# AIS-Bonn/lattice_net

Hardware: AMD Instinct MI355X
Metric: Mpoints/sec splat+conv+slice fwd+bwd on 120k-pt SemanticKITTI scan (higher is better)
Workload: dtype f32 (convolution products bf16x3-emulated)

## Files before the change

include/latticenet_hip.h:

```cpp
#ifndef LATTICENET_HIP_H
#define LATTICENET_HIP_H

#include <stddef.h>

#ifdef __cplusplus
extern "C" {
#endif

#define LN_OK 0
#define LN_ERR_ARG (-1)
#define LN_ERR_UNSUPPORTED (-2)
#define LN_ERR_LAUNCH (-3)
#define LN_ERR_WORKSPACE (-4)

#define LN_STATUS_TABLE_FULL 1
#define LN_STATUS_KEY_RANGE 2
#define LN_STATUS_BUCKET_OVERFLOW 4
#define LN_STATUS_CLOUD_BAND 8
#define LN_STATUS_CLOUD_STARTS 16

#define LN_MAX_POS_DIM 6
#define LN_SLOT_MAP_INTS 32
#define LN_KEYS_RAW 0
#define LN_KEYS_LATTICE 1
#define LN_NOT_VISITED (-2)

typedef struct LnTable {
    int capacity;
    int pos_dim;
    unsigned long long* slot_keys;
    unsigned int* slot_tok;
    int* slot_cnt;
    int* entries;
    int* keys;
    int* nr_filled;
    int* status;
    int* host_counters;
    int host_seq;
    int key_format;
    int row_limit;
    const int* slot_map;
    int bucket_slots_max;
    int batch_points;
    int batch_key_step;
    int* row_regions;
} LnTable;

#define LN_BATCH_POINT_STARTS (-1)
typedef struct LnTableClouds {
    LnTable table;
    const int* batch_point_starts;
    int batch_clouds;
} LnTableClouds;

#define LN_XCD_GROUPS 8
typedef struct LnCsr {
    int* grp_start;
    int* csr_tok;
    int* seg_desc;
    int* seg_count;
    long long seg_region;
    const int* planes;
    int dense;
} LnCsr;

const char* ln_last_error_string(void);
const char* ln_version(void);
const char* ln_abi_hash(void);

const char* ln_kernel_names(void);
int ln_profile_begin(const char* kernel_names, int max_samples);
int ln_profile_end(double* total_ms, int* launches);
int ln_profile_end_table(char* out, int out_bytes);

int ln_table_clear(const LnTable* t, float* values, long long values_elems, void* stream);

int ln_arena_init(int* arena, long long words, long long minus_begin, long long minus_end, void* stream);

int ln_table_bucket_count(int capacity);

size_t ln_build_workspace_bytes(long long tokens, int capacity);

#define LN_BUILD_WRITE_IDX 1
#define LN_BUILD_CLEAR_FIRST 2
#define LN_BUILD_ATOMIC_PATH 4
#define LN_BUILD_CANONICAL_ROWS 8
#define LN_BUILD_SORTED_CSR 16
#define LN_BUILD_OVERLAPPED 32
int ln_build_splat(const LnTable* t, const float* positions_raw, const float* sigmas_host, int n, int* idx, float* w,
                   int flags, const LnCsr* csr, void* workspace, size_t workspace_bytes, float* clear_values,
                   long long clear_values_elems, void* stream);

int ln_canonicalize(const LnTable* t, int* idx, long long tokens, const LnCsr* csr, void* workspace, size_t workspace_bytes, void* stream);

int ln_rehash(const LnTable* t, void* stream);

int ln_splat_accumulate(float* table_values, const float* vals, const int* idx, const float* w, int n, int pos_dim,
                        int val_dim, void* stream);

long long ln_csr_max_segments(long long tokens, int groups_upper);
size_t ln_csr_workspace_bytes(long long tokens, int groups_upper);
int ln_csr_build(const int* idx, long long tokens, int groups_upper, const LnCsr* csr, void* workspace, size_t workspace_bytes,
                 void* stream);
int ln_csr_reduce_rows(const LnCsr* csr, const int* grp_row, long long max_segments, const float* src, const float* w, int val_dim,
                       int src_div, int src_stride, float* dst, void* stream);
int ln_csr_sort(const LnCsr* csr, int groups_upper, void* workspace, size_t workspace_bytes, long long tokens, void* stream);

int ln_splat_accumulate_and_neighbours(const LnCsr* csr, const int* grp_row, long long max_segments, const float* src, const float* w,
                                       int val_dim, int src_div, int src_stride, float* dst, const LnTable* table, int query_rows_upper,
                                       int* nbr, void* stream);

int ln_csr_segment_max(const LnCsr* csr, const int* grp_row, long long max_segments, const float* src, int channels, int rows,
                       void* packed_ws, float* out_max, int* out_arg, void* stream);
int ln_csr_group_sizes(const LnCsr* csr, const int* grp_row, int groups_upper, int rows, int* counts, void* stream);

int ln_distribute(const LnTable* t, const float* positions_raw, const float* sigmas_host, const float* vals, int n,
                  int val_dim, int* idx, float* w, float* distributed, int flags, const LnCsr* csr, void* workspace,
                  size_t workspace_bytes, float* clear_values, long long clear_values_elems, void* stream);

int ln_coarsen(const LnTable* fine, int fine_rows_upper, const LnTable* coarse, const LnCsr* csr, void* workspace,
               size_t workspace_bytes, void* stream);

int ln_neighbours(const LnTable* query, int query_rows_upper, const LnTable* neigh, int lvl_query, int lvl_neigh,
                  int dilation, int flip, int* nbr, void* stream);

int ln_im2row(const int* nbr, const float* values_neigh, int m, int filter_extent, int val_dim, float* out, void* stream);
int ln_im2rowindices(const int* nbr, int m, int filter_extent, int val_dim, int* out, void* stream);
int ln_row2im(const int* nbr, const float* rowified, int m, int filter_extent, int val_dim, float* out, void* stream);

#define LN_CONV_FLIP_NEIGHBOURS 1
#define LN_CONV_TRANSPOSED_FILTER 2
#define LN_CONV_BANK_READY 4
int ln_conv_forward(const int* nbr, const float* values_neigh, const float* filter, int m, int filter_extent, int val_dim,
                    int nr_filters, int flags, float* out, void* stream);
size_t ln_conv_bank_workspace_bytes(int m, int filter_extent, int val_dim, int nr_filters);
size_t ln_conv_forward_workspace_bytes(int m, int filter_extent, int val_dim, int nr_filters);
int ln_conv_forward_ws(const int* nbr, const float* values_neigh, const float* filter, int m, int filter_extent, int val_dim,
                       int nr_filters, int flags, float* out, void* workspace, size_t workspace_bytes, const int* row_partition, void* stream);
size_t ln_conv_grad_filter_workspace_bytes(int m, int filter_extent, int val_dim, int nr_filters);
int ln_conv_grad_filter(const int* nbr, const float* values_neigh, const float* grad_out, int m, int filter_extent,
                        int val_dim, int nr_filters, float* grad_filter, void* workspace, size_t workspace_bytes,
                        void* stream);

int ln_slice_forward(const float* values, const int* idx, const float* w, int n, int pos_dim, int val_dim, float* out,
                     void* stream);
int ln_slice_forward_prepare_backward(const float* values, const int* idx, const float* w, int n, int pos_dim, int val_dim, float* out,
                                      float* grad_accumulator, long long grad_accumulator_elems, void* stream);
int ln_slice_forward_ordered(const LnTable* t, const LnCsr* csr, const float* values, const int* idx, const float* w, int n, int val_dim,
                             float* out, float* grad_accumulator, long long grad_accumulator_elems, void* stream);

int ln_slice_no_precomputation(const LnTable* t, const float* values, const float* positions_raw, const float* sigmas_host,
                               int n, int val_dim, float* out, int* idx, float* w, void* stream);
int ln_slice_backward(const float* grad_sliced, const int* idx, const float* w, int n, int pos_dim, int val_dim,
                      float* grad_values, void* stream);

int ln_gather_forward(const float* values, const int* idx, const float* w, int n, int pos_dim, int val_dim, float* out,
                      void* stream);
int ln_gather_backward(const float* grad_gathered, const int* idx, const float* w, int n, int pos_dim, int val_dim,
                       float* grad_values, void* stream);

int ln_slice_classify_forward(const float* values, const float* delta_w, const float* lin_w, const float* lin_b,
                              const int* idx, const float* w, int n, int pos_dim, int val_dim, int nr_classes,
                              float* logits, void* stream);
size_t ln_slice_classify_backward_workspace_bytes(int n, int pos_dim, int val_dim, int nr_classes);
int ln_slice_classify_backward(const float* grad_logits, const float* values, const float* delta_w, const float* lin_w,
                               const int* idx, const float* w, int n, int pos_dim, int val_dim, int nr_classes,
                               float* g_values, float* g_delta_w, float* g_lin_w, float* g_lin_b, float* grad_sliced,
                               float* w_eff, void* workspace, size_t workspace_bytes, void* stream);

size_t ln_conv_backward_workspace_bytes(int mq, int mn, int filter_extent, int val_dim, int nr_filters);
int ln_conv_backward(const int* nbr_q, const int* nbr_n, const float* values_neigh, const float* grad_out, const float* filter, int mq, int mn,
                     int filter_extent, int val_dim, int nr_filters, float* grad_values, float* grad_filter, void* workspace,
                     size_t workspace_bytes, const int* row_partition, void* stream);

int ln_csr_reduce_rows_f16(const LnCsr* csr, const int* grp_row, long long max_segments, const void* src_f16, const float* w, int val_dim,
                           int src_div, int src_stride, float* dst, void* stream);
int ln_splat_accumulate_and_neighbours_f16(const LnCsr* csr, const int* grp_row, long long max_segments, const void* src_f16, const float* w,
                                           int val_dim, int src_div, int src_stride, float* dst, const LnTable* table, int query_rows_upper,
                                           int* nbr, void* stream);
int ln_slice_forward_f16(const void* values_f16, const int* idx, const float* w, int n, int pos_dim, int val_dim, void* out_f16, void* stream);
int ln_slice_forward_f16_prepare_backward(const void* values_f16, const int* idx, const float* w, int n, int pos_dim, int val_dim, void* out_f16,
                                          float* grad_accumulator, long long grad_accumulator_elems, void* stream);

int ln_conv_forward_f16(const int* nbr, const void* values_neigh, const void* filter, int m, int filter_extent, int val_dim,
                        int nr_filters, int flags, void* out, void* stream);
size_t ln_conv_grad_filter_f16_workspace_bytes(int m, int filter_extent, int val_dim, int nr_filters);
int ln_conv_grad_filter_f16(const int* nbr, const void* values_neigh, const void* grad_out, int m, int filter_extent, int val_dim,
                            int nr_filters, float* grad_filter, void* workspace, size_t workspace_bytes, void* stream);

int ln_linear_act_forward(const float* x, const float* w, const float* b, long long rows, int cin, int cout, float slope, float* y,
                          void* stream);
size_t ln_linear_act_backward_workspace_bytes(int cin, int cout);
int ln_linear_act_backward(const float* x, const float* w, const float* y, const float* grad_y, long long rows, int cin, int cout,
                           float slope, float* grad_x, float* grad_w, float* grad_b, void* workspace, size_t workspace_bytes, void* stream);

size_t ln_group_norm_workspace_bytes(int channels);
int ln_group_norm_forward(const float* x, const float* gamma, const float* beta, int m, int channels, int groups, float eps, int relu,
                          float* y, float* mean_rstd, float* scale_shift, void* workspace, size_t workspace_bytes, void* next_workspace,
                          size_t next_workspace_bytes, void* stream);
int ln_group_norm_backward(const float* x, const float* grad_y, const float* gamma, const float* mean_rstd, const float* scale_shift, int m,
                           int channels, int groups, int relu, float* grad_x, float* grad_gamma, float* grad_beta, void* workspace,
                           size_t workspace_bytes, void* next_workspace, size_t next_workspace_bytes, void* stream);
int ln_group_norm_forward_rows(const float* x, const float* gamma, const float* beta, int m, int channels, int groups, float eps, int relu,
                               float* y, float* mean_rstd, float* scale_shift, void* workspace, size_t workspace_bytes, void* next_workspace,
                               size_t next_workspace_bytes, const int* rows_device, void* stream);
int ln_group_norm_backward_rows(const float* x, const float* grad_y, const float* gamma, const float* mean_rstd, const float* scale_shift, int m,
                                int channels, int groups, int relu, float* grad_x, float* grad_gamma, float* grad_beta, void* workspace,
                                size_t workspace_bytes, void* next_workspace, size_t next_workspace_bytes, const int* rows_device, void* stream);

int ln_cloud_row_starts(const LnTable* t, int rows_upper, int clouds, int* row_starts, int* order_flag, void* stream);
int ln_cloud_row_starts_many(const LnTable* t, int rows_upper, int clouds, int* row_starts, int* order_flag, void* stream);
size_t ln_group_norm_segments_workspace_bytes(int channels, int segments);
int ln_group_norm_forward_segments(const float* x, const float* gamma, const float* beta, int m, int channels, int groups, float eps, int relu,
                                   float* y, float* mean_rstd, float* scale_shift, void* workspace, size_t workspace_bytes, void* next_workspace,
                                   size_t next_workspace_bytes, const int* rows_device, const int* row_starts, int segments, void* stream);
int ln_group_norm_backward_segments(const float* x, const float* grad_y, const float* gamma, const float* mean_rstd, const float* scale_shift,
                                    int m, int channels, int groups, int relu, float* grad_x, float* grad_gamma, float* grad_beta, void* workspace,
                                    size_t workspace_bytes, void* next_workspace, size_t next_workspace_bytes, const int* rows_device,
                                    const int* row_starts, int segments, void* stream);
int ln_group_norm_forward_many_segments(const float* x, const float* gamma, const float* beta, int m, int channels, int groups, float eps,
                                        int relu, float* y, float* mean_rstd, float* scale_shift, void* workspace, size_t workspace_bytes,
                                        void* next_workspace, size_t next_workspace_bytes, const int* rows_device, const int* row_starts,
                                        int segments, void* stream);
int ln_group_norm_backward_many_segments(const float* x, const float* grad_y, const float* gamma, const float* mean_rstd,
                                         const float* scale_shift, int m, int channels, int groups, int relu, float* grad_x, float* grad_gamma,
                                         float* grad_beta, void* workspace, size_t workspace_bytes, void* next_workspace,
                                         size_t next_workspace_bytes, const int* rows_device, const int* row_starts, int segments, void* stream);

int ln_group_norm_forward_segments_f16(const void* x, const float* gamma, const float* beta, int m, int channels, int groups, float eps, int relu,
                                       void* y, float* mean_rstd, float* scale_shift, void* workspace, size_t workspace_bytes,
                                       void* next_workspace, size_t next_workspace_bytes, const int* rows_device, const int* row_starts,
                                       int segments, void* stream);
int ln_group_norm_backward_segments_f16(const void* x, const void* grad_y, const float* gamma, const float* mean_rstd, const float* scale_shift,
                                        int m, int channels, int groups, int relu, void* grad_x, float* grad_gamma, float* grad_beta,
                                        void* workspace, size_t workspace_bytes, void* next_workspace, size_t next_workspace_bytes,
                                        const int* rows_device, const int* row_starts, int segments, void* stream);

size_t ln_batch_norm_workspace_bytes(int channels);
int ln_batch_norm_forward(const float* x, const float* gamma, const float* beta, float* running_mean, float* running_var, int m, int channels,
                          float eps, double momentum, int training, int relu, float* y, float* mean_rstd, float* scale_shift, void* workspace,
                          size_t workspace_bytes, void* next_workspace, size_t next_workspace_bytes, const int* rows_device, void* stream);
int ln_batch_norm_backward(const float* x, const float* grad_y, const float* gamma, const float* mean_rstd, const float* scale_shift, int m,
                           int channels, int training, int relu, float* grad_x, float* grad_gamma, float* grad_beta, void* workspace,
                           size_t workspace_bytes, void* next_workspace, size_t next_workspace_bytes, const int* rows_device, void* stream);

int ln_max_centre_forward(const float* x, const float* gamma, const float* beta, long long n, int k, int c, float* out,
                          float* max_vals, unsigned char* arg_max, void* stream);
size_t ln_max_centre_backward_workspace_bytes(long long n, int k, int c);
int ln_max_centre_backward(const float* grad_out, const float* max_vals, const unsigned char* arg_max, const float* gamma,
                           long long n, int k, int c, float* grad_x, float* grad_gamma_beta, void* workspace,
                           size_t workspace_bytes, void* stream);

size_t ln_linear_backward_workspace_bytes(int rows, int cin, int cout);
int ln_linear_backward(const int* ident, const float* x, const float* grad_y, const float* w, int rows, int cin, int cout, float* grad_x,
                       float* grad_w, void* workspace, size_t workspace_bytes, void* stream);

int ln_weight_norm_forward(const float* v, const float* g, int rows, int cols, int g_dim, float* w, float* norm, void* stream);
int ln_weight_norm_backward(const float* v, const float* g, const float* grad_w, const float* norm, int rows, int cols, int g_dim,
                            float* grad_v, float* grad_g, void* stream);

int ln_distribute_centre(const float* distributed, const int* splat_idx, const float* position_sums, const int* counts, long long tokens,
                         int width, int pos_dim, float* out, void* stream);
int ln_distribute_centre_clouds(const float* distributed, const int* splat_idx, const float* position_sums, const int* counts,
                                long long tokens, int width, int pos_dim, long long tokens_per_cloud, const int* row_starts, int clouds,
                                float* out, void* stream);
int ln_distribute_centre_cloud_starts(const float* distributed, const int* splat_idx, const float* position_sums, const int* counts,
                                      long long tokens, int width, int pos_dim, int tokens_per_point, const int* point_starts,
                                      const int* row_starts, int clouds, float* out, void* stream);
int ln_distribute_centre_many_clouds(const float* distributed, const int* splat_idx, const float* position_sums, const int* counts,
                                     long long tokens, int width, int pos_dim, long long tokens_per_cloud, const int* row_starts, int clouds,
                                     float* out, void* stream);
int ln_distribute_centre_many_cloud_starts(const float* distributed, const int* splat_idx, const float* position_sums, const int* counts,
                                           long long tokens, int width, int pos_dim, int tokens_per_point, const int* point_starts,
                                           const int* row_starts, int clouds, float* out, void* stream);

size_t ln_pointnet_reduce_workspace_bytes(int rows, int channels);
int ln_pointnet_reduce_forward(const LnCsr* csr, const int* grp_row, long long max_segments, const float* src, int channels,
                               const float* bary, int bary_stride, int rows, int min_points, void* workspace, size_t workspace_bytes,
                               float* out, int* out_arg, void* stream);
int ln_pointnet_reduce_forward_clouds(const LnCsr* csr, const int* grp_row, long long max_segments, const float* src, int channels,
                                      const float* bary, int bary_stride, int rows, int min_points, void* workspace, size_t workspace_bytes,
                                      float* out, int* out_arg, const int* row_starts, int clouds, void* stream);
int ln_pointnet_reduce_forward_many_clouds(const LnCsr* csr, const int* grp_row, long long max_segments, const float* src, int channels,
                                           const float* bary, int bary_stride, int rows, int min_points, void* workspace,
                                           size_t workspace_bytes, float* out, int* out_arg, const int* row_starts, int clouds, void* stream);
int ln_pointnet_reduce_backward(const float* grad_out, int grad_stride, const int* out_arg, const int* splat_idx, long long tokens,
                                int channels, float* grad_src, void* stream);

size_t ln_nll_workspace_bytes(void);
int ln_nll_forward(const float* log_probs, const long long* target, long long n, int classes, long long ignore_index, void* workspace,
                   size_t workspace_bytes, float* loss_count, void* stream);
int ln_nll_backward(const long long* target, const float* grad_loss, const float* loss_count, long long n, int classes,
                    long long ignore_index, float* grad_log_probs, void* stream);

size_t ln_lovasz_workspace_bytes(long long n, int classes);
int ln_lovasz_forward(const float* log_probs, const long long* target, long long n, int classes, long long ignore_index, int reduction,
                      void* workspace, size_t workspace_bytes, float* loss, float* per_class, float* dloss_dlogp, void* stream);
int ln_lovasz_backward(const float* dloss_dlogp, const float* grad_loss, long long n, int classes, float* grad_log_probs, void* stream);

size_t ln_lovasz_clouds_workspace_bytes(long long n, long long points_per_cloud, int classes);
int ln_lovasz_forward_clouds(const float* log_probs, const long long* target, long long n, long long points_per_cloud, int classes,
                             long long ignore_index, int reduction, void* workspace, size_t workspace_bytes, float* loss, float* per_cloud,
                             float* per_class, float* dloss_dlogp, void* stream);

size_t ln_iou_counts_clouds_workspace_bytes(long long n, long long points_per_cloud, int classes);
int ln_iou_counts_clouds(const float* scores, const long long* target, long long n, long long points_per_cloud, int classes,
                         long long unlabeled_index, void* workspace, size_t workspace_bytes, long long* intersection, long long* union_,
                         void* stream);

size_t ln_dice_workspace_bytes(long long n, long long points_per_cloud, int classes);
int ln_dice_forward(const float* log_probs, const long long* target, long long n, long long points_per_cloud, int classes,
                    long long ignore_index, void* workspace, size_t workspace_bytes, float* loss, float* per_cloud, float* stats, float* coef,
                    void* stream);
int ln_dice_backward(const float* log_probs, const long long* target, const float* coef, const float* grad_loss, long long n,
                     long long points_per_cloud, int classes, float* grad_log_probs, void* stream);

size_t ln_nll_clouds_workspace_bytes(long long n, long long points_per_cloud);
int ln_nll_forward_clouds(const float* log_probs, const long long* target, long long n, long long points_per_cloud, int classes,
                          long long ignore_index, const float* class_weight, void* workspace, size_t workspace_bytes, float* loss,
                          float* per_cloud, float* weight_sum, void* stream);
int ln_nll_backward_clouds(const long long* target, const float* grad_loss, const float* weight_sum, long long n, long long points_per_cloud,
                           int classes, long long ignore_index, const float* class_weight, float* grad_log_probs, void* stream);

size_t ln_nll_ranges_workspace_bytes(long long n, int clouds, long long longest);
int ln_nll_forward_ranges(const float* log_probs, const long long* target, long long n, const int* point_starts, int clouds, long long longest,
                          int classes, long long ignore_index, const float* class_weight, void* workspace, size_t workspace_bytes, float* loss,
                          float* per_cloud, float* weight_sum, void* stream);
int ln_nll_backward_ranges(const long long* target, const float* grad_loss, const float* weight_sum, long long n, const int* point_starts,
                           int clouds, long long longest, int classes, long long ignore_index, const float* class_weight,
                           float* grad_log_probs, void* stream);
size_t ln_dice_ranges_workspace_bytes(long long n, int clouds, long long longest, int classes);
int ln_dice_forward_ranges(const float* log_probs, const long long* target, long long n, const int* point_starts, int clouds, long long longest,
                           int classes, long long ignore_index, void* workspace, size_t workspace_bytes, float* loss, float* per_cloud,
                           float* stats, float* coef, void* stream);
int ln_dice_backward_ranges(const float* log_probs, const long long* target, const float* coef, const float* grad_loss, long long n,
                            const int* point_starts, int clouds, long long longest, int classes, float* grad_log_probs, void* stream);
size_t ln_lovasz_ranges_workspace_bytes(long long n, int clouds, long long longest, int classes);
int ln_lovasz_forward_ranges(const float* log_probs, const long long* target, long long n, const int* point_starts, int clouds,
                             long long longest, int classes, long long ignore_index, int reduction, void* workspace, size_t workspace_bytes,
                             float* loss, float* per_cloud, float* per_class, float* dloss_dlogp, void* stream);

int ln_cloud_key_extents(const LnTable* t, const float* positions_raw, const float* sigmas_host, int n, int guard, int* extents,
                         int* first_bad, void* stream);
int ln_cloud_point_starts_check(const int* starts, int clouds, int n, int* status, void* stream);

#ifdef __cplusplus
}
#endif
#endif
```

lattice_net_amd/_lib.py:

```python
from __future__ import annotations

import ctypes as C
import os

import torch

_PKG = os.path.dirname(os.path.abspath(__file__))
LIB_PATH = os.environ.get("LATTICE_NET_LIB") or os.path.join(_PKG, "liblatticenet_hip.so")

LN_STATUS_TABLE_FULL = 1
LN_STATUS_KEY_RANGE = 2
LN_STATUS_BUCKET_OVERFLOW = 4
LN_STATUS_CLOUD_BAND = 8
LN_STATUS_CLOUD_STARTS = 16
LN_BUILD_WRITE_IDX = 1
LN_BUILD_CLEAR_FIRST = 2
LN_BUILD_ATOMIC_PATH = 4
LN_BUILD_CANONICAL_ROWS = 8
LN_BUILD_SORTED_CSR = 16
LN_BUILD_OVERLAPPED = 32
LN_NOT_VISITED = -2
LN_CONV_FLIP_NEIGHBOURS = 1
LN_CONV_TRANSPOSED_FILTER = 2
LN_CONV_BANK_READY = 4
LN_MAX_POS_DIM = 6
LN_KEYS_RAW = 0
LN_KEYS_LATTICE = 1
LN_XCD_GROUPS = 8
LN_SLOT_MAP_INTS = 32


class LnTable(C.Structure):

    _fields_ = [
        ("capacity", C.c_int),
        ("pos_dim", C.c_int),
        ("slot_keys", C.c_void_p),
        ("slot_tok", C.c_void_p),
        ("slot_cnt", C.c_void_p),
        ("entries", C.c_void_p),
        ("keys", C.c_void_p),
        ("nr_filled", C.c_void_p),
        ("status", C.c_void_p),
        ("host_counters", C.c_void_p),
        ("host_seq", C.c_int),
        ("key_format", C.c_int),
        ("row_limit", C.c_int),
        ("slot_map", C.c_void_p),
        ("bucket_slots_max", C.c_int),
        ("batch_points", C.c_int),
        ("batch_key_step", C.c_int),
        ("row_regions", C.c_void_p),
    ]


LN_BATCH_POINT_STARTS = -1


class LnTableClouds(C.Structure):

    _fields_ = [
        ("table", LnTable),
        ("batch_point_starts", C.c_void_p),
        ("batch_clouds", C.c_int),
    ]

    def __init__(self, table_fields=(), batch_point_starts=None, batch_clouds=0):
        super().__init__(LnTable(*table_fields), batch_point_starts, batch_clouds)
        self.table.batch_points = LN_BATCH_POINT_STARTS


class LnCsr(C.Structure):

    _fields_ = [
        ("grp_start", C.c_void_p),
        ("csr_tok", C.c_void_p),
        ("seg_desc", C.c_void_p),
        ("seg_count", C.c_void_p),
        ("seg_region", C.c_longlong),
        ("planes", C.c_void_p),
        ("dense", C.c_int),
    ]


class LatticeNetHipError(RuntimeError):
    pass


_vp, _i, _ll, _sz = C.c_void_p, C.c_int, C.c_longlong, C.c_size_t
_T = C.POINTER(LnTable)
_CSR = C.POINTER(LnCsr)

SIGNATURES = {
    "ln_last_error_string": (C.c_char_p, []),
    "ln_version": (C.c_char_p, []),
    "ln_abi_hash": (C.c_char_p, []),
    "ln_kernel_names": (C.c_char_p, []),
    "ln_profile_begin": (_i, [C.c_char_p, _i]),
    "ln_profile_end": (_i, [C.POINTER(C.c_double), C.POINTER(_i)]),
    "ln_profile_end_table": (_i, [C.c_char_p, _i]),
    "ln_table_clear": (_i, [_T, _vp, _ll, _vp]),
    "ln_build_workspace_bytes": (_sz, [_ll, _i]),
    "ln_table_bucket_count": (_i, [_i]),
    "ln_build_splat": (_i, [_T, _vp, _vp, _i, _vp, _vp, _i, _CSR, _vp, _sz, _vp, _ll, _vp]),
    "ln_rehash": (_i, [_T, _vp]),
    "ln_canonicalize": (_i, [_T, _vp, _ll, _CSR, _vp, _sz, _vp]),
    "ln_splat_accumulate": (_i, [_vp, _vp, _vp, _vp, _i, _i, _i, _vp]),
    "ln_csr_workspace_bytes": (_sz, [_ll, _i]),
    "ln_csr_max_segments": (_ll, [_ll, _i]),
    "ln_csr_build": (_i, [_vp, _ll, _i, _CSR, _vp, _sz, _vp]),
    "ln_csr_reduce_rows": (_i, [_CSR, _vp, _ll, _vp, _vp, _i, _i, _i, _vp, _vp]),
    "ln_csr_sort": (_i, [_CSR, _i, _vp, _sz, _ll, _vp]),
    "ln_splat_accumulate_and_neighbours": (_i, [_CSR, _vp, _ll, _vp, _vp, _i, _i, _i, _vp, _T, _i, _vp, _vp]),
    "ln_csr_segment_max": (_i, [_CSR, _vp, _ll, _vp, _i, _i, _vp, _vp, _vp, _vp]),
    "ln_csr_group_sizes": (_i, [_CSR, _vp, _i, _i, _vp, _vp]),
    "ln_distribute": (_i, [_T, _vp, _vp, _vp, _i, _i, _vp, _vp, _vp, _i, _CSR, _vp, _sz, _vp, _ll, _vp]),
    "ln_coarsen": (_i, [_T, _i, _T, _CSR, _vp, _sz, _vp]),
    "ln_neighbours": (_i, [_T, _i, _T, _i, _i, _i, _i, _vp, _vp]),
    "ln_im2row": (_i, [_vp, _vp, _i, _i, _i, _vp, _vp]),
    "ln_im2rowindices": (_i, [_vp, _i, _i, _i, _vp, _vp]),
    "ln_row2im": (_i, [_vp, _vp, _i, _i, _i, _vp, _vp]),
    "ln_conv_forward": (_i, [_vp, _vp, _vp, _i, _i, _i, _i, _i, _vp, _vp]),
    "ln_conv_forward_workspace_bytes": (_sz, [_i, _i, _i, _i]),
    "ln_conv_bank_workspace_bytes": (_sz, [_i, _i, _i, _i]),
    "ln_conv_forward_ws": (_i, [_vp, _vp, _vp, _i, _i, _i, _i, _i, _vp, _vp, _sz, _vp, _vp]),
    "ln_conv_grad_filter_workspace_bytes": (_sz, [_i, _i, _i, _i]),
    "ln_conv_grad_filter": (_i, [_vp, _vp, _vp, _i, _i, _i, _i, _vp, _vp, _sz, _vp]),
    "ln_slice_forward": (_i, [_vp, _vp, _vp, _i, _i, _i, _vp, _vp]),
    "ln_slice_forward_prepare_backward": (_i, [_vp, _vp, _vp, _i, _i, _i, _vp, _vp, _ll, _vp]),
    "ln_slice_forward_ordered": (_i, [_T, _CSR, _vp, _vp, _vp, _i, _i, _vp, _vp, _ll, _vp]),
    "ln_slice_no_precomputation": (_i, [_T, _vp, _vp, _vp, _i, _i, _vp, _vp, _vp, _vp]),
    "ln_slice_backward": (_i, [_vp, _vp, _vp, _i, _i, _i, _vp, _vp]),
    "ln_gather_forward": (_i, [_vp, _vp, _vp, _i, _i, _i, _vp, _vp]),
    "ln_gather_backward": (_i, [_vp, _vp, _vp, _i, _i, _i, _vp, _vp]),
    "ln_slice_classify_forward": (_i, [_vp, _vp, _vp, _vp, _vp, _vp, _i, _i, _i, _i, _vp, _vp]),
    "ln_csr_reduce_rows_f16": (_i, [_CSR, _vp, _ll, _vp, _vp, _i, _i, _i, _vp, _vp]),
    "ln_splat_accumulate_and_neighbours_f16": (_i, [_CSR, _vp, _ll, _vp, _vp, _i, _i, _i, _vp, _T, _i, _vp, _vp]),
    "ln_slice_forward_f16": (_i, [_vp, _vp, _vp, _i, _i, _i, _vp, _vp]),
    "ln_slice_forward_f16_prepare_backward": (_i, [_vp, _vp, _vp, _i, _i, _i, _vp, _vp, _ll, _vp]),
    "ln_conv_backward_workspace_bytes": (_sz, [_i, _i, _i, _i, _i]),
    "ln_conv_backward": (_i, [_vp, _vp, _vp, _vp, _vp, _i, _i, _i, _i, _i, _vp, _vp, _vp, _sz, _vp, _vp]),
    "ln_conv_forward_f16": (_i, [_vp, _vp, _vp, _i, _i, _i, _i, _i, _vp, _vp]),
    "ln_conv_grad_filter_f16_workspace_bytes": (_sz, [_i, _i, _i, _i]),
    "ln_conv_grad_filter_f16": (_i, [_vp, _vp, _vp, _i, _i, _i, _i, _vp, _vp, _sz, _vp]),
    "ln_linear_act_forward": (_i, [_vp, _vp, _vp, _ll, _i, _i, C.c_float, _vp, _vp]),
    "ln_linear_act_backward_workspace_bytes": (_sz, [_i, _i]),
    "ln_linear_act_backward": (_i, [_vp, _vp, _vp, _vp, _ll, _i, _i, C.c_float, _vp, _vp, _vp, _vp, _sz, _vp]),
    "ln_arena_init": (_i, [_vp, _ll, _ll, _ll, _vp]),
    "ln_weight_norm_forward": (_i, [_vp, _vp, _i, _i, _i, _vp, _vp, _vp]),
    "ln_weight_norm_backward": (_i, [_vp, _vp, _vp, _vp, _i, _i, _i, _vp, _vp, _vp]),
    "ln_distribute_centre": (_i, [_vp, _vp, _vp, _vp, _ll, _i, _i, _vp, _vp]),
    "ln_distribute_centre_clouds": (_i, [_vp, _vp, _vp, _vp, _ll, _i, _i, _ll, _vp, _i, _vp, _vp]),
    "ln_distribute_centre_many_clouds": (_i, [_vp, _vp, _vp, _vp, _ll, _i, _i, _ll, _vp, _i, _vp, _vp]),
    "ln_distribute_centre_cloud_starts": (_i, [_vp, _vp, _vp, _vp, _ll, _i, _i, _i, _vp, _vp, _i, _vp, _vp]),
    "ln_distribute_centre_many_cloud_starts": (_i, [_vp, _vp, _vp, _vp, _ll, _i, _i, _i, _vp, _vp, _i, _vp, _vp]),
    "ln_pointnet_reduce_workspace_bytes": (_sz, [_i, _i]),
    "ln_pointnet_reduce_forward": (_i, [_CSR, _vp, _ll, _vp, _i, _vp, _i, _i, _i, _vp, _sz, _vp, _vp, _vp]),
    "ln_pointnet_reduce_forward_clouds": (_i, [_CSR, _vp, _ll, _vp, _i, _vp, _i, _i, _i, _vp, _sz, _vp, _vp, _vp, _i, _vp]),
    "ln_pointnet_reduce_forward_many_clouds": (_i, [_CSR, _vp, _ll, _vp, _i, _vp, _i, _i, _i, _vp, _sz, _vp, _vp, _vp, _i, _vp]),
    "ln_pointnet_reduce_backward": (_i, [_vp, _i, _vp, _vp, _ll, _i, _vp, _vp]),
    "ln_linear_backward_workspace_bytes": (_sz, [_i, _i, _i]),
    "ln_linear_backward": (_i, [_vp, _vp, _vp, _vp, _i, _i, _i, _vp, _vp, _vp, _sz, _vp]),
    "ln_nll_workspace_bytes": (_sz, []),
    "ln_nll_forward": (_i, [_vp, _vp, _ll, _i, _ll, _vp, _sz, _vp, _vp]),
    "ln_nll_backward": (_i, [_vp, _vp, _vp, _ll, _i, _ll, _vp, _vp]),
    "ln_nll_clouds_workspace_bytes": (_sz, [_ll, _ll]),
    "ln_nll_forward_clouds": (_i, [_vp, _vp, _ll, _ll, _i, _ll, _vp, _vp, _sz, _vp, _vp, _vp, _vp]),
    "ln_nll_backward_clouds": (_i, [_vp, _vp, _vp, _ll, _ll, _i, _ll, _vp, _vp, _vp]),
    "ln_lovasz_workspace_bytes": (_sz, [_ll, _i]),
    "ln_lovasz_forward": (_i, [_vp, _vp, _ll, _i, _ll, _i, _vp, _sz, _vp, _vp, _vp, _vp]),
    "ln_lovasz_backward": (_i, [_vp, _vp, _ll, _i, _vp, _vp]),
    "ln_lovasz_clouds_workspace_bytes": (_sz, [_ll, _ll, _i]),
    "ln_lovasz_forward_clouds": (_i, [_vp, _vp, _ll, _ll, _i, _ll, _i, _vp, _sz, _vp, _vp, _vp, _vp, _vp]),
    "ln_iou_counts_clouds_workspace_bytes": (_sz, [_ll, _ll, _i]),
    "ln_iou_counts_clouds": (_i, [_vp, _vp, _ll, _ll, _i, _ll, _vp, _sz, _vp, _vp, _vp]),
    "ln_dice_workspace_bytes": (_sz, [_ll, _ll, _i]),
    "ln_dice_forward": (_i, [_vp, _vp, _ll, _ll, _i, _ll, _vp, _sz, _vp, _vp, _vp, _vp, _vp]),
    "ln_dice_backward": (_i, [_vp, _vp, _vp, _vp, _ll, _ll, _i, _vp, _vp]),
    "ln_nll_ranges_workspace_bytes": (_sz, [_ll, _i, _ll]),
    "ln_nll_forward_ranges": (_i, [_vp, _vp, _ll, _vp, _i, _ll, _i, _ll, _vp, _vp, _sz, _vp, _vp, _vp, _vp]),
    "ln_nll_backward_ranges": (_i, [_vp, _vp, _vp, _ll, _vp, _i, _ll, _i, _ll, _vp, _vp, _vp]),
    "ln_dice_ranges_workspace_bytes": (_sz, [_ll, _i, _ll, _i]),
    "ln_dice_forward_ranges": (_i, [_vp, _vp, _ll, _vp, _i, _ll, _i, _ll, _vp, _sz, _vp, _vp, _vp, _vp, _vp]),
    "ln_dice_backward_ranges": (_i, [_vp, _vp, _vp, _vp, _ll, _vp, _i, _ll, _i, _vp, _vp]),
    "ln_lovasz_ranges_workspace_bytes": (_sz, [_ll, _i, _ll, _i]),
    "ln_lovasz_forward_ranges": (_i, [_vp, _vp, _ll, _vp, _i, _ll, _i, _ll, _i, _vp, _sz, _vp, _vp, _vp, _vp, _vp]),
    "ln_max_centre_forward": (_i, [_vp, _vp, _vp, _ll, _i, _i, _vp, _vp, _vp, _vp]),
    "ln_max_centre_backward_workspace_bytes": (_sz, [_ll, _i, _i]),
    "ln_max_centre_backward": (_i, [_vp, _vp, _vp, _vp, _ll, _i, _i, _vp, _vp, _vp, _sz, _vp]),
    "ln_group_norm_workspace_bytes": (_sz, [_i]),
    "ln_group_norm_forward": (_i, [_vp, _vp, _vp, _i, _i, _i, C.c_float, _i, _vp, _vp, _vp, _vp, _sz, _vp, _sz, _vp]),
    "ln_group_norm_backward": (_i, [_vp, _vp, _vp, _vp, _vp, _i, _i, _i, _i, _vp, _vp, _vp, _vp, _sz, _vp, _sz, _vp]),
    "ln_group_norm_forward_rows": (_i, [_vp, _vp, _vp, _i, _i, _i, C.c_float, _i, _vp, _vp, _vp, _vp, _sz, _vp, _sz, _vp, _vp]),
    "ln_group_norm_backward_rows": (_i, [_vp, _vp, _vp, _vp, _vp, _i, _i, _i, _i, _vp, _vp, _vp, _vp, _sz, _vp, _sz, _vp, _vp]),
    "ln_cloud_row_starts": (_i, [_T, _i, _i, _vp, _vp, _vp]),
    "ln_cloud_row_starts_many": (_i, [_T, _i, _i, _vp, _vp, _vp]),
    "ln_group_norm_segments_workspace_bytes": (_sz, [_i, _i]),
    "ln_group_norm_forward_segments": (_i, [_vp, _vp, _vp, _i, _i, _i, C.c_float, _i, _vp, _vp, _vp, _vp, _sz, _vp, _sz, _vp, _vp, _i, _vp]),
    "ln_group_norm_forward_many_segments": (_i, [_vp, _vp, _vp, _i, _i, _i, C.c_float, _i, _vp, _vp, _vp, _vp, _sz, _vp, _sz, _vp, _vp, _i, _vp]),
    "ln_group_norm_backward_segments": (_i, [_vp, _vp, _vp, _vp, _vp, _i, _i, _i, _i, _vp, _vp, _vp, _vp, _sz, _vp, _sz, _vp, _vp, _i, _vp]),
    "ln_group_norm_backward_many_segments": (_i, [_vp, _vp, _vp, _vp, _vp, _i, _i, _i, _i, _vp, _vp, _vp, _vp, _sz, _vp, _sz, _vp, _vp, _i, _vp]),
    "ln_group_norm_forward_segments_f16": (_i, [_vp, _vp, _vp, _i, _i, _i, C.c_float, _i, _vp, _vp, _vp, _vp, _sz, _vp, _sz, _vp, _vp, _i, _vp]),
    "ln_group_norm_backward_segments_f16": (_i, [_vp, _vp, _vp, _vp, _vp, _i, _i, _i, _i, _vp, _vp, _vp, _vp, _sz, _vp, _sz, _vp, _vp, _i, _vp]),
    "ln_batch_norm_workspace_bytes": (_sz, [_i]),
    "ln_batch_norm_forward": (_i, [_vp, _vp, _vp, _vp, _vp, _i, _i, C.c_float, C.c_double, _i, _i, _vp, _vp, _vp, _vp, _sz, _vp, _sz, _vp, _vp]),
    "ln_batch_norm_backward": (_i, [_vp, _vp, _vp, _vp, _vp, _i, _i, _i, _i, _vp, _vp, _vp, _vp, _sz, _vp, _sz, _vp, _vp]),
    "ln_cloud_key_extents": (_i, [_T, _vp, _vp, _i, _i, _vp, _vp, _vp]),
    "ln_cloud_point_starts_check": (_i, [_vp, _i, _i, _vp, _vp]),
    "ln_slice_classify_backward_workspace_bytes": (_sz, [_i, _i, _i, _i]),
    "ln_slice_classify_backward": (_i, [_vp, _vp, _vp, _vp, _vp, _vp, _i, _i, _i, _i, _vp, _vp, _vp, _vp, _vp, _vp, _vp, _sz, _vp]),
}

_lib = None


def load():
    global _lib
    if _lib is not None:
        return _lib
    if not os.path.exists(LIB_PATH):
        raise LatticeNetHipError(
            f"{LIB_PATH} is missing: the HIP extension is not built. Run `python -c 'import __graft_entry__ as g; g.build()'` "
            "(or `python lattice_net_amd/build_ext.py`). There is no CPU fallback."
        )
    lib = C.CDLL(LIB_PATH)
    for name, (res, args) in SIGNATURES.items():
        fn = getattr(lib, name)
        fn.restype = res
        fn.argtypes = args
    from . import build_ext
    try:
        want = build_ext.abi_hash()
    except OSError:
        want = None
    have = lib.ln_abi_hash().decode()
    if want is not None and have != want:
        raise LatticeNetHipError(f"{LIB_PATH} was built from a different include/latticenet_hip.h (library {have}, header {want}): "
                                 "rebuild it with `python lattice_net_amd/build_ext.py`")
    _lib = lib
    return lib


def check(rc: int, what: str = ""):
    if rc != 0:
        msg = load().ln_last_error_string().decode("utf-8", "replace")
        raise LatticeNetHipError(f"{what or 'latticenet_hip'} failed (code {rc}): {msg}")


def ptr(t):
    return None if t is None else t.data_ptr()


def stream_ptr(device) -> int:
    cur = torch.cuda.current_device()
    idx = device.index if device.index is not None else cur
    if idx != cur:
        raise LatticeNetHipError(f"lattice tensors live on cuda:{idx} but the current device is cuda:{cur}; wrap the call in "
                                 f"`with torch.cuda.device({idx}):` (or torch.cuda.set_device) — one process drives one GPU")
    return torch._C._cuda_getCurrentRawStream(idx)


def host_floats(values):
    arr = (C.c_float * len(values))(*[float(v) for v in values])
    return arr
```

lattice_net_amd/csrc/ln_conv.hip:

```cpp
#include "ln_common.h"
#include <stdlib.h>

#include "ln_bf16x3.h"

#include "ln_conv_plan.h"
#include <type_traits>

#ifdef LN_STAMPS
__device__ unsigned long long* g_ln_stamps_conv = nullptr;
extern "C" int ln_debug_set_stamps_conv(void* buffer) {
    unsigned long long* p = static_cast<unsigned long long*>(buffer);
    return hipMemcpyToSymbol(HIP_SYMBOL(g_ln_stamps_conv), &p, sizeof(p)) == hipSuccess ? 0 : -1;
}
#define LN_CSTAMP(slot)                                                                                                  \
    do {                                                                                                                 \
        if (g_ln_stamps_conv && threadIdx.x == 0) g_ln_stamps_conv[(size_t)blockIdx.x * 8 + (slot)] = wall_clock64(); \
    } while (0)
#else
#define LN_CSTAMP(slot) do { } while (0)
#endif

template <int KQ>
__device__ __forceinline__ void ln_load_quarter(const float* __restrict__ src, float* a) {
    if constexpr (KQ % 4 == 0) {
// ... 784 lines not shown
        advance(it);
    };
    for (int it = 0; it < total; it += 2) {
        iteration(it, ap, ap_b);
        if (it + 1 < total) iteration(it + 1, ap_b, ap);
    }
    asm volatile("s_waitcnt vmcnt(0)" ::: "memory");
    __builtin_amdgcn_s_barrier();
    floatx4* park = reinterpret_cast<floatx4*>(s_pool) + (size_t)rt * NT * 4 * 64 + lane;
    if (kh == 1) {
#pragma unroll
        for (int nt = 0; nt < NT; ++nt)
#pragma unroll
            for (int qd = 0; qd < 4; ++qd)
                park[(nt * 4 + qd) * 64] = floatx4{acc[nt][4 * qd], acc[nt][4 * qd + 1], acc[nt][4 * qd + 2], acc[nt][4 * qd + 3]};
    }
    __syncthreads();
    if (kh == 0) {
#pragma unroll
        for (int nt = 0; nt < NT; ++nt) {
#pragma unroll
            for (int qd = 0; qd < 4; ++qd) {
                const floatx4 o = park[(nt * 4 + qd) * 64];
#pragma unroll
                for (int r4 = 0; r4 < 4; ++r4) {
                    const int row = m0 + 8 * qd + 4 * h + r4;
                    if (row < m) out[(size_t)row * f_total + f_off + nt * 32 + i] = acc[nt][4 * qd + r4] + o[r4];
                }
            }
        }
    }
}

template <int V, int NT, int E, bool FLIP, bool WT>
__global__ void __launch_bounds__(256)
    k_conv_mfma_full(const int* __restrict__ nbr, const float* __restrict__ values, const float* __restrict__ filter, int m,
                     float* __restrict__ out, int conv_blocks, const float* __restrict__ slab_partial, int nslabs, int slab_total,
                     float* __restrict__ slab_out) {
    if (slab_out != nullptr && (int)blockIdx.x >= conv_blocks) {
        ln_sum_slabs_body<false>(blockIdx.x - conv_blocks, slab_partial, nslabs, slab_total, slab_total, slab_out);
        return;
    }
    constexpr int F = 16 * NT;
    constexpr int KQ = V / 4;
    static_assert(E * V * F * 4 <= 64 * 1024, "filter bank must fit 64 KiB of LDS");
    __shared__ __attribute__((aligned(16))) float s_b[E * V * F];
    const int tid = threadIdx.x;
    const int lane = tid & 63;
    const int wave = tid >> 6;
    const int i = lane & 15;
    const int q = lane >> 4;
    const int m0 = blockIdx.x * 64 + wave * 16;
    const int my_row = m0 + i;

    LN_CSTAMP(0);
    constexpr int N4 = E * V * F / 4;
    constexpr int NST = (N4 + 255) / 256;
    float4 wv[NST];
#pragma unroll
    for (int s = 0; s < NST; ++s) {
        const int x4 = tid + s * 256;
        wv[s] = (x4 < N4) ? reinterpret_cast<const float4*>(filter)[x4] : make_float4(0.f, 0.f, 0.f, 0.f);
    }
    int nb[E];
#pragma unroll
    for (int e = 0; e < E; ++e) nb[e] = (my_row < m) ? nbr[(size_t)my_row * E + ((FLIP && e < E - 1) ? (e ^ 1) : e)] : -1;
    float a[E][KQ];
#pragma unroll
    for (int e = 0; e < E; ++e) ln_load_quarter<KQ>(values + (size_t)(nb[e] >= 0 ? nb[e] : 0) * V + q * KQ, a[e]);
#pragma unroll
    for (int s = 0; s < NST; ++s) {
        const int x4 = tid + s * 256;
        if (x4 < N4) {
            const int x = x4 * 4;
            if constexpr (!WT) {
                const int ek = x / F;
                const int f = x - ek * F;
                const int e = ek / V;
                const int k = ek - e * V;
                const int qq = k / KQ;
                const int kk = k - qq * KQ;
                float* dst = s_b + (((e * KQ + kk) * NT + (f >> 4)) * 64 + qq * 16 + (f & 15));
                *reinterpret_cast<float4*>(dst) = wv[s];
            } else {
                const int ef = x / V;
                const int k0 = x - ef * V;
                const int e = ef / F;
                const int f = ef - e * F;
                const float vals4[4] = {wv[s].x, wv[s].y, wv[s].z, wv[s].w};
#pragma unroll
                for (int j = 0; j < 4; ++j) {
                    const int k = k0 + j;
                    const int qq = k / KQ;
                    const int kk = k - qq * KQ;
                    s_b[((e * KQ + kk) * NT + (f >> 4)) * 64 + qq * 16 + (f & 15)] = vals4[j];
                }
            }
        }
    }
    __syncthreads();
    LN_CSTAMP(1);
    floatx4 acc[NT];
#pragma unroll
    for (int nt = 0; nt < NT; ++nt) acc[nt] = floatx4{0.f, 0.f, 0.f, 0.f};
#pragma unroll
    for (int e = 0; e < E; ++e) {
#pragma unroll
        for (int kk = 0; kk < KQ; ++kk) {
            const float av = nb[e] >= 0 ? a[e][kk] : 0.f;
#pragma unroll
            for (int nt = 0; nt < NT; ++nt) {
                const float b = s_b[((e * KQ + kk) * NT + nt) * 64 + lane];
                acc[nt] = __builtin_amdgcn_mfma_f32_16x16x4f32(av, b, acc[nt], 0, 0, 0);
            }
        }
    }
    LN_CSTAMP(2);
#pragma unroll
    for (int nt = 0; nt < NT; ++nt) {
#pragma unroll
        for (int r = 0; r < 4; ++r) {
            const int row = m0 + q * 4 + r;
            if (row < m) out[(size_t)row * F + nt * 16 + i] = acc[nt][r];
        }
    }
    LN_CSTAMP(3);
}

__global__ void __launch_bounds__(256)
    k_conv_generic(const int* __restrict__ nbr, const float* __restrict__ values, const float* __restrict__ filter, long long work,
                   int E, int V, int F, int flip, int wt, float* __restrict__ out) {
    const long long g = (long long)blockIdx.x * blockDim.x + threadIdx.x;
    if (g >= work) return;
    const long long mrow = g / F;
    const int f = int(g - mrow * F);
    float acc = 0.0f;
    for (int e = 0; e < E; ++e) {
        const int nb = nbr[mrow * E + ((flip && e < E - 1) ? (e ^ 1) : e)];
        if (nb < 0) continue;
        const float* vr = values + (size_t)nb * V;
        if (wt) {
            const float* wr = filter + ((size_t)e * F + f) * V;
            for (int v = 0; v < V; ++v) acc = fmaf(vr[v], wr[v], acc);
        } else {
            const float* wr = filter + (size_t)e * V * F + f;
            for (int v = 0; v < V; ++v) acc = fmaf(vr[v], wr[(size_t)v * F], acc);
        }
    }
    out[g] = acc;
}

__global__ void __launch_bounds__(256) ln_k_sum_partials(const float* __restrict__ partial, int nslabs, long long total4, float* __restrict__ out) {
    const long long i = (long long)blockIdx.x * 256 + threadIdx.x;
    if (i >= total4) return;
    float4 acc = reinterpret_cast<const float4*>(partial)[i];
    for (int sl = 1; sl < nslabs; ++sl) {
        const float4 v = reinterpret_cast<const float4*>(partial)[(long long)sl * total4 + i];
        acc.x += v.x; acc.y += v.y; acc.z += v.z; acc.w += v.w;
    }
    reinterpret_cast<float4*>(out)[i] = acc;
}

static bool ln_conv_b3_enabled() {
    static int v = -1;
    if (v < 0) {
        const char* e = getenv("LN_CONV_EXACT_F32");
        v = (e && e[0] == '1') ? 0 : 1;
    }
    return v == 1;
}
static bool ln_aligned16(const void* p) { return (reinterpret_cast<uintptr_t>(p) & 15) == 0; }

extern "C" size_t ln_conv_bank_workspace_bytes(int m, int filter_extent, int val_dim, int nr_filters) {
    return ln_conv_bank_query(m, filter_extent, val_dim, nr_filters, ln_conv_b3_enabled());
}

extern "C" size_t ln_conv_forward_workspace_bytes(int m, int filter_extent, int val_dim, int nr_filters) {
    return ln_conv_forward_query(m, filter_extent, val_dim, nr_filters, ln_conv_b3_enabled());
}

template <int T>
__global__ void __launch_bounds__(256 * T) __attribute__((amdgpu_waves_per_eu(T, T)))
    k_conv_forward_b3(const int* __restrict__ nbr, const float* __restrict__ values, const float* __restrict__ filter, int m,
                      float* __restrict__ out, const int* __restrict__ row_part) {
    constexpr int V = 32, F = 32, E = 9, KQ = 8, NT = 2;
    constexpr int THREADS = 256 * T;
    constexpr int FRAG16 = E * NT * 3 * 64;
    __shared__ __attribute__((aligned(16))) unsigned char s_raw[FRAG16 * 16];
    const u32x4* s_frag = reinterpret_cast<const u32x4*>(s_raw);
    __shared__ __attribute__((aligned(16))) floatx4 s_x[4 * T][16 * 8];
    __shared__ int s_nbr[64 * T * E];
    const int tid = threadIdx.x;
    const int lane = tid & 63;
    const int i = lane & 15;
    const int q = lane >> 4;
    const int bx = ln_partition_tile(blockIdx.x, gridDim.x, row_part, 64 * T);
    const int m0 = bx * (64 * T) + (tid >> 6) * 16;
    const int my_row = m0 + i;
    constexpr int ITEMS = E * (V / 8) * F;
    constexpr int NIT = (ITEMS + THREADS - 1) / THREADS;
    float wv[NIT][8];
#pragma unroll
    for (int s = 0; s < NIT; ++s) {
        const int x = min(tid + s * THREADS, ITEMS - 1);
        const int f = x % F;
        const int ev8 = x / F;
#pragma unroll
        for (int j = 0; j < 8; ++j) wv[s][j] = filter[(ev8 * 8 + j) * F + f];
    }
    {
        const size_t g0 = (size_t)bx * (64 * T) * E, g_end = (size_t)m * E;
        for (int x = tid; x < 64 * T * E; x += THREADS) s_nbr[x] = (g0 + x < g_end) ? nbr[g0 + x] : -1;
    }
    {
        bool any = false;
        for (int x = tid; x < 64 * T * E; x += THREADS) any |= s_nbr[x] >= 0;
        if (!__syncthreads_or(any)) {
            for (int x = tid; x < 64 * T * (F / 4); x += THREADS) {
                const int row = bx * (64 * T) + x / (F / 4);
                if (row < m) *reinterpret_cast<float4*>(out + (size_t)row * F + (x % (F / 4)) * 4) = make_float4(0.f, 0.f, 0.f, 0.f);
            }
            return;
        }
    }
    const int wv_ = tid >> 6;
    const int lr = lane >> 3;
    int nb[2][E];
#pragma unroll
    for (int j = 0; j < 2; ++j)
#pragma unroll
        for (int e = 0; e < E; ++e) nb[j][e] = s_nbr[(wv_ * 16 + 8 * j + lr) * E + e];
    auto fsw = [](int r) -> int { return ((r >> 1) & 7) ^ (((r >> 2) & 1) << 1); };
    floatx4* xw[2];
#pragma unroll
    for (int j = 0; j < 2; ++j) xw[j] = &s_x[wv_][(8 * j + lr) * 8 + ((lane & 7) ^ fsw(8 * j + lr))];
    const floatx4* xr0 = &s_x[wv_][i * 8 + ((2 * q) ^ fsw(i))];
    const floatx4* xr1 = &s_x[wv_][i * 8 + ((2 * q + 1) ^ fsw(i))];
#ifndef LN_FWD_DEPTH
#define LN_FWD_DEPTH 4
#endif
    constexpr int DEPTH = LN_FWD_DEPTH;
    floatx4 a[DEPTH][2];
    auto gather = [&](int e, floatx4 (&dst)[2]) {
#pragma unroll
        for (int j = 0; j < 2; ++j)
            dst[j] = *reinterpret_cast<const floatx4*>(values + (size_t)(nb[j][e] >= 0 ? nb[j][e] : 0) * V + (lane & 7) * 4);
    };
#pragma unroll
    for (int k = 0; k < DEPTH - 1 && k < E; ++k) gather(k, a[k]);
    u32x4* s_frag_w = reinterpret_cast<u32x4*>(s_raw);
#pragma unroll
    for (int s = 0; s < NIT; ++s) {
        const int x = tid + s * THREADS;
        if (x < ITEMS) {
            const int f = x % F;
            const int ev8 = x / F;
            const int e = ev8 / (V / 8);
            const int vo = ev8 - e * (V / 8);
            unsigned int h[8], md[8], lo[8];
#pragma unroll
            for (int j = 0; j < 8; ++j) ln_split3_bits(wv[s][j], h[j], md[j], lo[j]);
            const int unit = ((e * NT + (f >> 4)) * 3) * 64 + vo * 16 + (f & 15);
            s_frag_w[unit] = u32x4{ln_pack_hi(h[0], h[1]), ln_pack_hi(h[2], h[3]), ln_pack_hi(h[4], h[5]), ln_pack_hi(h[6], h[7])};
            s_frag_w[unit + 64] = u32x4{ln_pack_hi(md[0], md[1]), ln_pack_hi(md[2], md[3]), ln_pack_hi(md[4], md[5]), ln_pack_hi(md[6], md[7])};
            s_frag_w[unit + 128] = u32x4{ln_pack_hi(lo[0], lo[1]), ln_pack_hi(lo[2], lo[3]), ln_pack_hi(lo[4], lo[5]), ln_pack_hi(lo[6], lo[7])};
        }
    }
    floatx4 acc[NT];
#pragma unroll
    for (int nt = 0; nt < NT; ++nt) acc[nt] = floatx4{0.f, 0.f, 0.f, 0.f};
    __syncthreads();
#pragma unroll
    for (int e = 0; e < E; ++e) {
        if (e + DEPTH - 1 < E) gather(e + DEPTH - 1, a[(e + DEPTH - 1) % DEPTH]);
#pragma unroll
        for (int j = 0; j < 2; ++j) *xw[j] = (nb[j][e] >= 0) ? a[e % DEPTH][j] : floatx4{0.f, 0.f, 0.f, 0.f};
        __builtin_amdgcn_fence(__ATOMIC_RELEASE, "wavefront");
        __builtin_amdgcn_wave_barrier();
        __builtin_amdgcn_fence(__ATOMIC_ACQUIRE, "wavefront");
        const floatx4 lo4 = *xr0, hi4 = *xr1;
        __builtin_amdgcn_fence(__ATOMIC_RELEASE, "wavefront");
        __builtin_amdgcn_wave_barrier();
        __builtin_amdgcn_fence(__ATOMIC_ACQUIRE, "wavefront");
        const float ae[KQ] = {lo4[0], lo4[1], lo4[2], lo4[3], hi4[0], hi4[1], hi4[2], hi4[3]};
        u32x4 p[3];
        ln_split3_pack8(ae, 0, p);
        const bf16x8 ap[3] = {__builtin_bit_cast(bf16x8, p[0]), __builtin_bit_cast(bf16x8, p[1]), __builtin_bit_cast(bf16x8, p[2])};
#pragma unroll
        for (int nt = 0; nt < NT; ++nt) {
            const u32x4* pb = s_frag + ((e * NT + nt) * 3) * 64 + lane;
            const bf16x8 bp[3] = {__builtin_bit_cast(bf16x8, pb[0]), __builtin_bit_cast(bf16x8, pb[64]), __builtin_bit_cast(bf16x8, pb[128])};
            ln_b3_mfma16(ap, bp, acc[nt]);
        }
    }
#pragma unroll
    for (int nt = 0; nt < NT; ++nt)
#pragma unroll
        for (int r = 0; r < 4; ++r) {
            const int row = m0 + q * 4 + r;
            if (row < m) out[(size_t)row * F + nt * 16 + i] = acc[nt][r];
        }
}

template <bool FLIP, bool WT>
struct LnConvCall {
    const int* nbr;
    const float *values, *filter;
    int m, E, V, F;
    float* out;
    unsigned short* bank;
    float* dst;
    int e_per;
    LnSlabSum sum;
    const int* row_partition;
    hipStream_t st;
};

template <bool FLIP, bool WT>
static void ln_conv_launch_full(int V, int NT, dim3 grid, hipStream_t st, const int* nbr, const float* values, const float* filter, int m,
                                float* out, int conv_blocks, const float* partial, int chunks, int total, float* grad_filter) {
    auto go = [&](auto v, auto nt) {
        constexpr int VV = decltype(v)::value, NN = decltype(nt)::value;
        static_assert(ln_conv_full_shape(VV, 16 * NN), "not a small-filter shape");
        LN_LAUNCH("k_conv_mfma", (k_conv_mfma_full<VV, NN, 9, FLIP, WT>), grid, dim3(256), 0, st, nbr, values, filter, m, out, conv_blocks, partial,
                  chunks, total, grad_filter);
    };
    using std::integral_constant;
    switch (V * 16 + NT) {
        case 32 * 16 + 2: go(integral_constant<int, 32>{}, integral_constant<int, 2>{}); break;
        case 32 * 16 + 1: go(integral_constant<int, 32>{}, integral_constant<int, 1>{}); break;
        case 16 * 16 + 1: go(integral_constant<int, 16>{}, integral_constant<int, 1>{}); break;
        case 16 * 16 + 2: go(integral_constant<int, 16>{}, integral_constant<int, 2>{}); break;
        case 16 * 16 + 4: go(integral_constant<int, 16>{}, integral_constant<int, 4>{}); break;
        case 8 * 16 + 1: go(integral_constant<int, 8>{}, integral_constant<int, 1>{}); break;
        case 8 * 16 + 2: go(integral_constant<int, 8>{}, integral_constant<int, 2>{}); break;
        case 8 * 16 + 4: go(integral_constant<int, 8>{}, integral_constant<int, 4>{}); break;
        case 8 * 16 + 8: go(integral_constant<int, 8>{}, integral_constant<int, 8>{}); break;
        default: break;
    }
}

template <bool FLIP, bool WT>
struct LnConvEntry {
    const LnConvLaunch& l;
    const LnConvCall<FLIP, WT>& c;
    dim3 grid() const { return dim3(l.grid[0], l.grid[1], l.grid[2]); }
    unsigned short* bank() const { return c.bank + l.bank_off; }
    const u32x4* frags() const { return reinterpret_cast<const u32x4*>(bank()); }
    LnSlabSum ride() const { return l.carries_sum ? c.sum : LnSlabSum{nullptr, 0, 0, nullptr}; }
};
template <int V, int NT, bool FLIP, bool WT>
static void ln_conv_run_wide(const LnConvEntry<FLIP, WT>& e) {
    const LnConvLaunch& l = e.l;
    const LnConvCall<FLIP, WT>& c = e.c;
    if constexpr (ln_conv_wide_built(V, NT)) {
        if (l.kernel == LN_K_SPLIT_BANK32) {
            LN_LAUNCH("k_conv_split_bank", (k_conv_split_bank32<V, NT, WT>), e.grid(), dim3(l.block), 0, c.st, c.filter, c.F, l.f_off, e.bank(), l.split_x,
                      e.ride());
            return;
        }
        if constexpr (NT == 3) {
            if (l.kernel == LN_K_ROWS32SK) {
                LN_LAUNCH("k_conv_mfma", (k_conv_rows32sk_b3<V, NT, LN_CONV_R32SK_RT, FLIP>), e.grid(), dim3(l.block), 0, c.st, c.nbr, c.values, e.frags(),
                          c.m, c.E, c.dst, c.F, l.f_off, c.e_per);
                return;
            }
        }
        LN_LAUNCH("k_conv_mfma", (k_conv_rows32_b3<V, ln_conv_r32_ntw(NT), ln_conv_r32_ch(NT), ln_conv_r32_rt(NT), FLIP>), e.grid(), dim3(l.block), 0, c.st,
                  c.nbr, c.values, e.frags(), c.m, c.E, c.dst, c.F, l.f_off, c.e_per);
    }
}
template <int V, int NT, bool FLIP, bool WT>
static void ln_conv_run_chunk(const LnConvEntry<FLIP, WT>& e) {
    const LnConvLaunch& l = e.l;
    const LnConvCall<FLIP, WT>& c = e.c;
    if constexpr (ln_conv_chunk_fits(V, NT)) {
        if constexpr (ln_conv_chunk_b3(V, NT)) {
            if (l.kernel == LN_K_SPLIT_BANK) {
                LN_LAUNCH("k_conv_split_bank", (k_conv_split_bank<V, NT, WT>), e.grid(), dim3(l.block), 0, c.st, c.filter, c.F, l.f_off, e.bank(), l.split_x,
                          e.ride());
                return;
            }
            if (l.kernel == LN_K_MFMA_B3) {
                if (l.t == 3) {
                    if constexpr (ln_conv_b3_three_subtiles(V))
                        LN_LAUNCH("k_conv_mfma", (k_conv_mfma_b3<V, NT, FLIP, 3>), e.grid(), dim3(l.block), 0, c.st, c.nbr, c.values, e.frags(), c.m, c.E,
                                  c.dst, c.F, l.f_off, c.e_per);
                } else {
                    LN_LAUNCH("k_conv_mfma", (k_conv_mfma_b3<V, NT, FLIP, 1>), e.grid(), dim3(l.block), 0, c.st, c.nbr, c.values, e.frags(), c.m, c.E, c.dst,
                              c.F, l.f_off, c.e_per);
                }
                return;
            }
        }
        LN_LAUNCH("k_conv_mfma", (k_conv_mfma<V, NT, FLIP, WT>), e.grid(), dim3(l.block), 0, c.st, c.nbr, c.values, c.filter, c.m, c.E, c.dst, c.F, l.f_off,
                  c.e_per);
    }
}

template <int V, bool FLIP, bool WT>
static void ln_conv_run_v(const LnConvLaunch& l, const LnConvCall<FLIP, WT>& c) {
    const LnConvEntry<FLIP, WT> e = {l, c};
    if (l.kernel == LN_K_SPLIT_BANK32 || l.kernel == LN_K_ROWS32 || l.kernel == LN_K_ROWS32SK) {
        switch (l.nt) {
            case 4: ln_conv_run_wide<V, 4>(e); break;
            case 3: ln_conv_run_wide<V, 3>(e); break;
            case 2: ln_conv_run_wide<V, 2>(e); break;
            case 1: ln_conv_run_wide<V, 1>(e); break;
            default: break;
        }
    } else {
        switch (l.nt) {
            case 8: ln_conv_run_chunk<V, 8>(e); break;
            case 4: ln_conv_run_chunk<V, 4>(e); break;
            case 2: ln_conv_run_chunk<V, 2>(e); break;
            case 1: ln_conv_run_chunk<V, 1>(e); break;
            default: break;
        }
    }
}

template <bool FLIP, bool WT>
static void ln_conv_run(const LnConvPlan& p, const LnConvCall<FLIP, WT>& c) {
    for (int k = 0; k < p.n; ++k) {
        const LnConvLaunch& l = p.launch[k];
        const dim3 grid(l.grid[0], l.grid[1], l.grid[2]), block(l.block);
        switch (l.kernel) {
            case LN_K_FORWARD_B3:
                if constexpr (!FLIP && !WT) {
                    if (l.t == 1) LN_LAUNCH("k_conv_mfma", (k_conv_forward_b3<1>), grid, block, 0, c.st, c.nbr, c.values, c.filter, c.m, c.out, c.row_partition);
                    else if (l.t == 2) LN_LAUNCH("k_conv_mfma", (k_conv_forward_b3<2>), grid, block, 0, c.st, c.nbr, c.values, c.filter, c.m, c.out, c.row_partition);
                    else LN_LAUNCH("k_conv_mfma", (k_conv_forward_b3<3>), grid, block, 0, c.st, c.nbr, c.values, c.filter, c.m, c.out, c.row_partition);
                }
                break;
            case LN_K_FULL:
                ln_conv_launch_full<FLIP, WT>(c.V, l.nt, grid, c.st, c.nbr, c.values, c.filter, c.m, c.out, l.grid[0], nullptr, 0, 0, nullptr);
                break;
            case LN_K_SUM_PARTIALS:
                LN_LAUNCH("k_conv_sum_partials", ln_k_sum_partials, grid, block, 0, c.st, (const float*)c.dst, p.nsplit, (long long)c.m * c.F / 4, c.out);
                break;
            case LN_K_GENERIC:
                LN_LAUNCH("k_conv_generic", k_conv_generic, grid, block, 0, c.st, c.nbr, c.values, c.filter, (long long)c.m * c.F, c.E, c.V, c.F,
                          FLIP ? 1 : 0, WT ? 1 : 0, c.out);
                break;
            default:
                switch (c.V) {
                    case 8: ln_conv_run_v<8>(l, c); break;
                    case 16: ln_conv_run_v<16>(l, c); break;
                    case 32: ln_conv_run_v<32>(l, c); break;
                    case 48: ln_conv_run_v<48>(l, c); break;
                    case 64: ln_conv_run_v<64>(l, c); break;
                    case 96: ln_conv_run_v<96>(l, c); break;
                    case 128: ln_conv_run_v<128>(l, c); break;
                    case 192: ln_conv_run_v<192>(l, c); break;
                    case 256: ln_conv_run_v<256>(l, c); break;
                    default: break;
                }
        }
    }
}

template <bool FLIP, bool WT>
static void ln_conv_plan_and_run(LnConvPlanIn in, const int* nbr, const float* values, const float* filter, float* out, void* ws,
                                 const LnSlabSum& sum, bool* sum_left, const int* row_partition, hipStream_t st) {
    in.flip = FLIP;
    in.wt = WT;
    const LnConvPlan p = ln_conv_plan(in);
    char* slabs = static_cast<char*>(ws) + p.bank_bytes;
    ln_conv_run<FLIP, WT>(p, LnConvCall<FLIP, WT>{nbr, values, filter, in.m, in.E, in.V, in.F, out, static_cast<unsigned short*>(ws),
                                                 p.nsplit > 1 ? reinterpret_cast<float*>(slabs) : out, p.e_per, sum, row_partition, st});
    *sum_left = p.sum_left;
}

static int ln_conv_forward_riding(const int* nbr, const float* values_neigh, const float* filter, int m, int filter_extent, int val_dim,
                                  int nr_filters, int flags, float* out, void* workspace, size_t workspace_bytes, const int* row_partition,
                                  void* stream, const LnSlabSum& sum) {
    hipStream_t st = (hipStream_t)stream;
    bool sum_left = sum.partial != nullptr;
    const int rc = [&]() -> int {
        LN_REQUIRE(m >= 0 && filter_extent >= 1 && val_dim >= 1 && nr_filters >= 1, LN_ERR_ARG, "ln_conv_forward: bad sizes");
        LN_REQUIRE(m == 0 || (nbr && values_neigh && filter && out), LN_ERR_ARG, "ln_conv_forward: null buffer");
        LN_REQUIRE((flags & ~7) == 0, LN_ERR_ARG, "ln_conv_forward: unknown flags %d", flags);
        if (m == 0) return LN_OK;
        LnConvPlanIn in = {};
        in.m = m, in.E = filter_extent, in.V = val_dim, in.F = nr_filters;
        in.b3_enabled = ln_conv_b3_enabled();
        in.values_aligned = ln_aligned16(values_neigh);
        in.filter_aligned = ln_aligned16(filter);
        in.ws_aligned = workspace && (reinterpret_cast<uintptr_t>(workspace) & 255) == 0;
        in.ws_bytes = workspace_bytes;
        in.bank_ready = (flags & LN_CONV_BANK_READY) != 0 && workspace != nullptr;
        in.riding_total = sum.partial ? sum.total : 0;
        switch (flags & 3) {
            case 0: ln_conv_plan_and_run<false, false>(in, nbr, values_neigh, filter, out, workspace, sum, &sum_left, row_partition, st); break;
            case LN_CONV_FLIP_NEIGHBOURS: ln_conv_plan_and_run<true, false>(in, nbr, values_neigh, filter, out, workspace, sum, &sum_left, row_partition, st); break;
            case LN_CONV_TRANSPOSED_FILTER: ln_conv_plan_and_run<false, true>(in, nbr, values_neigh, filter, out, workspace, sum, &sum_left, row_partition, st); break;
            default: ln_conv_plan_and_run<true, true>(in, nbr, values_neigh, filter, out, workspace, sum, &sum_left, row_partition, st); break;
        }
        return ln_check_launch("ln_conv_forward");
    }();
    if (sum_left) (void)ln_reduce_slabs_async(sum.partial, sum.nslabs, sum.total, sum.out, st);
    return rc;
}

extern "C" int ln_conv_forward_ws(const int* nbr, const float* values_neigh, const float* filter, int m, int filter_extent, int val_dim,
                                  int nr_filters, int flags, float* out, void* workspace, size_t workspace_bytes, const int* row_partition,
                                  void* stream) {
    return ln_conv_forward_riding(nbr, values_neigh, filter, m, filter_extent, val_dim, nr_filters, flags, out, workspace, workspace_bytes,
                                  row_partition, stream, LnSlabSum{nullptr, 0, 0, nullptr});
}

extern "C" int ln_conv_forward(const int* nbr, const float* values_neigh, const float* filter, int m, int filter_extent,
                               int val_dim, int nr_filters, int flags, float* out, void* stream) {
    return ln_conv_forward_ws(nbr, values_neigh, filter, m, filter_extent, val_dim, nr_filters, flags, out, nullptr, 0, nullptr, stream);
}

#define LN_GF_SUB 64

template <int VT, int FT>
__global__ void __launch_bounds__(256)
    k_grad_filter_mfma(const int* __restrict__ nbr, const float* __restrict__ values, const float* __restrict__ grad_out, int m,
                       int E, float* __restrict__ partial, int v_total, int v_off, int f_total, int f_off) {
    if (gridDim.z > 1) {
        const int col_tiles = f_total / (16 * FT);
        v_off = (blockIdx.z / col_tiles) * 16 * VT;
        f_off = (blockIdx.z % col_tiles) * 16 * FT;
    }
    constexpr int V = VT * 16;
    constexpr int F = FT * 16;
    constexpr int SA = V + 16;
    constexpr int SG = F + 16;
    constexpr int TILES = VT * FT;
    constexpr int TPW = (TILES + 3) / 4;
    constexpr int A4 = LN_GF_SUB * V / 4 / 256;
    constexpr int G4 = LN_GF_SUB * F / 4 / 256;
    static_assert(A4 >= 1 && G4 >= 1, "tile too small for 256 staging threads");
    __shared__ __attribute__((aligned(16))) float s_a[LN_GF_SUB * SA];
    __shared__ __attribute__((aligned(16))) float s_g[LN_GF_SUB * SG];
    const int tid = threadIdx.x;
    const int lane = tid & 63;
    const int wave = tid >> 6;
    const int i = lane & 15;
    const int q = lane >> 4;
    const int e = blockIdx.y;
    const int chunk_begin = blockIdx.x * LN_GF_ROWS;
    const int chunk_end = min(chunk_begin + LN_GF_ROWS, m);

    floatx4 acc[TPW][2];
#pragma unroll
    for (int t = 0; t < TPW; ++t) {
        acc[t][0] = floatx4{0.f, 0.f, 0.f, 0.f};
        acc[t][1] = floatx4{0.f, 0.f, 0.f, 0.f};
    }
    float4 ra[A4], rg[G4];
    auto issue_loads = [&](int sub_begin) {
#pragma unroll
        for (int s = 0; s < A4; ++s) {
            const int x4 = tid + s * 256;
            const int r = x4 / (V / 4);
            const int c = x4 - r * (V / 4);
            const int row = sub_begin + r;
            const int nb = (row < chunk_end) ? nbr[(size_t)row * E + e] : -1;
            ra[s] = *reinterpret_cast<const float4*>(values + (size_t)(nb >= 0 ? nb : 0) * v_total + v_off + c * 4);
            if (nb < 0) ra[s] = make_float4(0.f, 0.f, 0.f, 0.f);
        }
#pragma unroll
        for (int s = 0; s < G4; ++s) {
            const int x4 = tid + s * 256;
            const int r = x4 / (F / 4);
            const int c = x4 - r * (F / 4);
            const int row = sub_begin + r;
            rg[s] = (row < chunk_end) ? *reinterpret_cast<const float4*>(grad_out + (size_t)row * f_total + f_off + c * 4)
                                      : make_float4(0.f, 0.f, 0.f, 0.f);
        }
    };
    if (chunk_begin < chunk_end) issue_loads(chunk_begin);
    for (int sub = chunk_begin; sub < chunk_end; sub += LN_GF_SUB) {
        __syncthreads();
#pragma unroll
        for (int s = 0; s < A4; ++s) {
            const int x4 = tid + s * 256;
            const int r = x4 / (V / 4);
            const int c = x4 - r * (V / 4);
            *reinterpret_cast<float4*>(s_a + r * SA + c * 4) = ra[s];
        }
#pragma unroll
        for (int s = 0; s < G4; ++s) {
            const int x4 = tid + s * 256;
            const int r = x4 / (F / 4);
            const int c = x4 - r * (F / 4);
            *reinterpret_cast<float4*>(s_g + r * SG + c * 4) = rg[s];
        }
        __syncthreads();
        if (sub + LN_GF_SUB < chunk_end) issue_loads(sub + LN_GF_SUB);
#pragma unroll
        for (int t = 0; t < TPW; ++t) {
            const int tile = wave + 4 * t;
            if (tile < TILES) {
                const int vt = tile / FT;
                const int ft = tile - vt * FT;
                const float* pa = s_a + q * SA + vt * 16 + i;
                const float* pg = s_g + q * SG + ft * 16 + i;
#pragma unroll 8
                for (int k = 0; k < LN_GF_SUB / 4; k += 2) {
                    acc[t][0] = __builtin_amdgcn_mfma_f32_16x16x4f32(pa[(k * 4) * SA], pg[(k * 4) * SG], acc[t][0], 0, 0, 0);
                    acc[t][1] = __builtin_amdgcn_mfma_f32_16x16x4f32(pa[(k * 4 + 4) * SA], pg[(k * 4 + 4) * SG], acc[t][1], 0, 0, 0);
                }
            }
        }
    }
    float* dst = partial + ((size_t)blockIdx.x * E + e) * ((size_t)v_total * f_total) + (size_t)v_off * f_total + f_off;
#pragma unroll
    for (int t = 0; t < TPW; ++t) {
        const int tile = wave + 4 * t;
        if (tile < TILES) {
            const int vt = tile / FT;
            const int ft = tile - vt * FT;
#pragma unroll
            for (int r = 0; r < 4; ++r) dst[(size_t)(vt * 16 + q * 4 + r) * f_total + ft * 16 + i] = acc[t][0][r] + acc[t][1][r];
        }
    }
}

__global__ void __launch_bounds__(256)
    k_grad_filter_generic(const int* __restrict__ nbr, const float* __restrict__ values, const float* __restrict__ grad_out, int m,
                          int E, int V, int F, float* __restrict__ grad_filter) {
    const int g = blockIdx.x * blockDim.x + threadIdx.x;
    if (g >= E * V * F) return;
    const int f = g % F;
    const int ev = g / F;
    const int v = ev % V;
    const int e = ev / V;
    float acc = 0.0f;
    for (int row = 0; row < m; ++row) {
        const int nb = nbr[(size_t)row * E + e];
        if (nb >= 0) acc = fmaf(values[(size_t)nb * V + v], grad_out[(size_t)row * F + f], acc);
    }
    grad_filter[g] = acc;
}

__global__ void __launch_bounds__(256) k_reduce_slabs4(const float* __restrict__ partial, int nslabs, int total, float* __restrict__ out) {
    ln_reduce_slabs4_block(blockIdx.x, partial, nslabs, total, out);
}

int ln_reduce_slabs_async(const float* partial, int nslabs, int total, float* out, hipStream_t st) {
    if (total % 64 == 0 && ((reinterpret_cast<uintptr_t>(out) | reinterpret_cast<uintptr_t>(partial)) & 15) == 0)
        LN_LAUNCH("k_reduce_slabs", k_reduce_slabs4, dim3(total / 64), dim3(256), 0, st, partial, nslabs, total, out);
    else
        LN_LAUNCH("k_reduce_slabs", ln_k_sum_slabs<false>, dim3(ln_div_up(total, 16)), dim3(256), 0, st, partial, nslabs, (long long)total, total, out);
    return LN_OK;
}

typedef short gf_short4 __attribute__((ext_vector_type(4)));
#ifndef LN_GFB_WAVES
#define LN_GFB_WAVES 2
#endif
template <int VT, int FT, int E, int WV, int WF>
__global__ void __launch_bounds__(64 * WV * WF, (WV * WF) > 8 ? 1 : LN_GFB_WAVES)
    k_grad_filter_b3(const int* __restrict__ nbr, const float* __restrict__ values, const float* __restrict__ grad_out, int m, int rows_per_wg,
                     float* __restrict__ partial, int v_total, int f_total) {
    constexpr int V = VT * 16, F = FT * 16;
    constexpr int EG = LN_GFB_EG;
    static_assert(E % EG == 0, "slot groups");
    constexpr int TPV = VT / WV, TPF = FT / WF;
    constexpr int THREADS = 64 * WV * WF;
    constexpr int RSA = V + 16, RSG = F + 16;
    constexpr int PA = LN_GFB_SUB * RSA, PG = LN_GFB_SUB * RSG;
    constexpr int A4 = LN_GFB_SUB * V / 4 / THREADS, G4 = LN_GFB_SUB * F / 4 / THREADS;
    static_assert(A4 >= 1 && G4 >= 1 && VT % WV == 0 && FT % WF == 0 && (LN_GFB_SUB * V / 4) % THREADS == 0 && (LN_GFB_SUB * F / 4) % THREADS == 0,
                  "block shape");
    extern __shared__ __attribute__((aligned(16))) unsigned short s_gfb[];
    unsigned short* s_a = s_gfb;
    unsigned short* s_g = s_gfb + 3 * PA;
    const int tid = threadIdx.x, lane = tid & 63, wave = tid >> 6;
    const int i = lane & 15, q = lane >> 4;
    const int col_blocks = f_total / F;
    const int v_off = (blockIdx.z / col_blocks) * V, f_off = (blockIdx.z % col_blocks) * F;
    const int e0 = blockIdx.y * EG;
    const int chunk_begin = blockIdx.x * rows_per_wg;
    const int chunk_end = min(chunk_begin + rows_per_wg, m);
    const int wv = wave / WF, wf = wave % WF;

    floatx4 acc[EG][TPV][TPF];
#pragma unroll
    for (int e = 0; e < EG; ++e)
#pragma unroll
        for (int a = 0; a < TPV; ++a)
#pragma unroll
            for (int b = 0; b < TPF; ++b) acc[e][a][b] = floatx4{0.f, 0.f, 0.f, 0.f};
    float4 ra[A4], rg[G4];
    int ids[EG][A4];
    auto fetch_ids = [&](int sub) {
#pragma unroll
        for (int e = 0; e < EG; ++e)
#pragma unroll
            for (int k = 0; k < A4; ++k) {
                const int row = sub + (tid + THREADS * k) / (V / 4);
                ids[e][k] = row < chunk_end ? nbr[(size_t)row * E + e0 + e] : -1;
            }
    };
    auto fetch_a = [&](const int (&nb)[A4]) {
#pragma unroll
        for (int k = 0; k < A4; ++k) {
            const int x4 = tid + THREADS * k;
            const int c4 = x4 % (V / 4);
            ra[k] = make_float4(0.f, 0.f, 0.f, 0.f);
            if (nb[k] >= 0) ra[k] = *reinterpret_cast<const float4*>(values + (size_t)nb[k] * v_total + v_off + c4 * 4);
        }
    };
    auto fetch_g = [&](int sub) {
#pragma unroll
        for (int k = 0; k < G4; ++k) {
            const int x4 = tid + THREADS * k;
            const int r = x4 / (F / 4), c4 = x4 - r * (F / 4);
            const int row = sub + r;
            rg[k] = make_float4(0.f, 0.f, 0.f, 0.f);
            if (row < chunk_end) rg[k] = *reinterpret_cast<const float4*>(grad_out + (size_t)row * f_total + f_off + c4 * 4);
        }
    };
    auto stage = [&](const float4& x, unsigned short* dst, int plane) {
        unsigned int h[4], md[4], lo[4];
        ln_split3_bits(x.x, h[0], md[0], lo[0]);
        ln_split3_bits(x.y, h[1], md[1], lo[1]);
        ln_split3_bits(x.z, h[2], md[2], lo[2]);
        ln_split3_bits(x.w, h[3], md[3], lo[3]);
        *reinterpret_cast<uint2*>(dst) = make_uint2(ln_pack_hi(h[0], h[1]), ln_pack_hi(h[2], h[3]));
        *reinterpret_cast<uint2*>(dst + plane) = make_uint2(ln_pack_hi(md[0], md[1]), ln_pack_hi(md[2], md[3]));
        *reinterpret_cast<uint2*>(dst + 2 * plane) = make_uint2(ln_pack_hi(lo[0], lo[1]), ln_pack_hi(lo[2], lo[3]));
    };
    auto frag = [&](const unsigned short* base, int rs) {
        const gf_short4 lo4 = __builtin_amdgcn_ds_read_tr16_b64_v4i16((gf_short4 __attribute__((address_space(3)))*)(base));
        const gf_short4 hi4 = __builtin_amdgcn_ds_read_tr16_b64_v4i16((gf_short4 __attribute__((address_space(3)))*)(base + 16 * rs));
        u32x4 p;
        p[0] = (unsigned int)(unsigned short)lo4[0] | ((unsigned int)(unsigned short)lo4[1] << 16);
        p[1] = (unsigned int)(unsigned short)lo4[2] | ((unsigned int)(unsigned short)lo4[3] << 16);
        p[2] = (unsigned int)(unsigned short)hi4[0] | ((unsigned int)(unsigned short)hi4[1] << 16);
        p[3] = (unsigned int)(unsigned short)hi4[2] | ((unsigned int)(unsigned short)hi4[3] << 16);
        return __builtin_bit_cast(bf16x8, p);
    };
    if (chunk_begin < chunk_end) {
        fetch_ids(chunk_begin);
        fetch_g(chunk_begin);
        fetch_a(ids[0]);
    }
    for (int sub = chunk_begin; sub < chunk_end; sub += LN_GFB_SUB) {
        int nxt[A4];
#pragma unroll
        for (int k = 0; k < A4; ++k) {
            const int row = sub + LN_GFB_SUB + (tid + THREADS * k) / (V / 4);
            nxt[k] = row < chunk_end ? nbr[(size_t)row * E + e0] : -1;
        }
#pragma unroll
        for (int e = 0; e < EG; ++e) {
            __syncthreads();
            if (e == 0) {
#pragma unroll
                for (int k = 0; k < G4; ++k) {
                    const int x4 = tid + THREADS * k;
                    const int r = x4 / (F / 4), c4 = x4 - r * (F / 4);
                    stage(rg[k], s_g + r * RSG + c4 * 4, PG);
                }
            }
#pragma unroll
            for (int k = 0; k < A4; ++k) {
                const int x4 = tid + THREADS * k;
                const int r = x4 / (V / 4), c4 = x4 - r * (V / 4);
                stage(ra[k], s_a + r * RSA + c4 * 4, PA);
            }
            __syncthreads();
            if (e + 1 < EG) {
                fetch_a(ids[e + 1]);
            } else if (sub + LN_GFB_SUB < chunk_end) {
                fetch_g(sub + LN_GFB_SUB);
                fetch_a(nxt);
                fetch_ids(sub + LN_GFB_SUB);
            }
#pragma unroll
            for (int st = 0; st < LN_GFB_SUB / 32; ++st) {
                const int row0 = 32 * st + 4 * q + (i >> 2);
                bf16x8 fa[TPV][3], fb[TPF][3];
#pragma unroll
                for (int a = 0; a < TPV; ++a)
#pragma unroll
                    for (int part = 0; part < 3; ++part) fa[a][part] = frag(s_a + part * PA + row0 * RSA + (wv * TPV + a) * 16 + (i & 3) * 4, RSA);
#pragma unroll
                for (int b = 0; b < TPF; ++b)
#pragma unroll
                    for (int part = 0; part < 3; ++part) fb[b][part] = frag(s_g + part * PG + row0 * RSG + (wf * TPF + b) * 16 + (i & 3) * 4, RSG);
#pragma unroll
                for (int a = 0; a < TPV; ++a)
#pragma unroll
                    for (int b = 0; b < TPF; ++b) ln_b3_mfma16(fa[a], fb[b], acc[e][a][b]);
            }
        }
    }
// ... 146 lines not shown
        const int x4 = tid + s * THREADS;
        if (x4 < N4) {
            const int x = x4 * 4;
            const int ev = x / F;
            const int k0 = x - ev * F;
            const int e = ev / V;
            const int v = ev - e * V;
            const float vals4[4] = {wv[s].x, wv[s].y, wv[s].z, wv[s].w};
#pragma unroll
            for (int j = 0; j < 4; ++j) {
                const int k = k0 + j;
                const int qq = k / KQ;
                const int kk = k - qq * KQ;
                s_b[((e * KQ + kk) * NT + (v >> 4)) * 64 + qq * 16 + (v & 15)] = vals4[j];
            }
        }
    }
    floatx4 acc_v[NT];
#pragma unroll
    for (int nt = 0; nt < NT; ++nt) acc_v[nt] = floatx4{0.f, 0.f, 0.f, 0.f};
    floatx4 acc_w[E];
#pragma unroll
    for (int e = 0; e < E; ++e) acc_w[e] = floatx4{0.f, 0.f, 0.f, 0.f};
#pragma unroll
    for (int k = 0; k < E; ++k) {
        const int e = slot_of(k);
        float* sg = s_all + BANK + sub * STAGE + (k & 1) * (64 * SG);
        float (&ae)[KQ] = a[k % (DEPTH + 1)];
        if (k + DEPTH < E)
            ln_load_quarter<KQ>(grad_out + (size_t)(nb[slot_of(k + DEPTH)] >= 0 ? nb[slot_of(k + DEPTH)] : 0) * F + q * KQ, a[(k + DEPTH) % (DEPTH + 1)]);
        {
            float* dst = sg + (wave * 16 + i) * SG + q * KQ;
#pragma unroll
            for (int c = 0; c < KQ; c += 4)
                *reinterpret_cast<float4*>(dst + c) = nb[e] >= 0 ? make_float4(ae[c], ae[c + 1], ae[c + 2], ae[c + 3]) : make_float4(0.f, 0.f, 0.f, 0.f);
        }
        __syncthreads();
        if (k == 0) LN_CSTAMP(1);
        if (k == 1) LN_CSTAMP(4);
        if (k == 8) LN_CSTAMP(5);
#pragma unroll
        for (int kk = 0; kk < KQ; ++kk) {
            const float av = nb[e] >= 0 ? ae[kk] : 0.f;
#pragma unroll
            for (int nt = 0; nt < NT; ++nt)
                acc_v[nt] = __builtin_amdgcn_mfma_f32_16x16x4f32(av, s_b[((e * KQ + kk) * NT + nt) * 64 + lane], acc_v[nt], 0, 0, 0);
        }
        const float* pg = sg + q * SG + ft * 16 + i;
        floatx4 w0 = floatx4{0.f, 0.f, 0.f, 0.f}, w1 = floatx4{0.f, 0.f, 0.f, 0.f};
#pragma unroll
        for (int st = 0; st < 16; st += 2) {
            w0 = __builtin_amdgcn_mfma_f32_16x16x4f32(vT[st], pg[(4 * st) * SG], w0, 0, 0, 0);
            w1 = __builtin_amdgcn_mfma_f32_16x16x4f32(vT[st + 1], pg[(4 * st + 4) * SG], w1, 0, 0, 0);
        }
        acc_w[e] = w0 + w1;
    }
    LN_CSTAMP(2);
#pragma unroll
    for (int nt = 0; nt < NT; ++nt) {
#pragma unroll
        for (int r = 0; r < 4; ++r) {
            const int row = m0 + q * 4 + r;
            if (row < m) grad_values[(size_t)row * V + nt * 16 + i] = acc_v[nt][r];
        }
    }
    __syncthreads();
    if (sub > 0) {
        float* park = s_all + (size_t)(sub - 1) * BANK;
#pragma unroll
        for (int e = 0; e < E; ++e)
#pragma unroll
            for (int r = 0; r < 4; ++r) park[(e * V + vt * 16 + q * 4 + r) * F + ft * 16 + i] = acc_w[e][r];
    }
    if constexpr (T > 1) __syncthreads();
    if (sub == 0) {
        float* dst = slabs + (size_t)blockIdx.x * BANK;
#pragma unroll
        for (int e = 0; e < E; ++e)
#pragma unroll
            for (int r = 0; r < 4; ++r) {
                const int o = (e * V + vt * 16 + q * 4 + r) * F + ft * 16 + i;
                float sum = acc_w[e][r];
#pragma unroll
                for (int k = 1; k < T; ++k) sum += s_all[(size_t)(k - 1) * BANK + o];
                dst[o] = sum;
            }
    }
    LN_CSTAMP(3);
}

typedef short short4v __attribute__((ext_vector_type(4)));
template <int T>
__global__ void __launch_bounds__(256 * T) __attribute__((amdgpu_waves_per_eu(T, T)))
    k_conv_backward_fused_b3(const int* __restrict__ nbr, const float* __restrict__ values, const float* __restrict__ grad_out,
                             const float* __restrict__ filter, int m, float* __restrict__ grad_values, float* __restrict__ slabs,
                             const int* __restrict__ row_part) {
    constexpr int V = 32, F = 32, E = 9, KQ = 8, NT = 2, FT = 2;
    constexpr int THREADS = 256 * T;
    constexpr int BANK = E * V * F;
    constexpr int FRAG16 = E * NT * 3 * 64;
    constexpr int RS = 32;
    auto swz = [](int r) { return (0x78 >> (2 * ((r >> 2) & 3))) & 3; };
    constexpr int PART = 64 * RS;
    constexpr int STAGE = 2 * 3 * PART;
    constexpr int LDS_BYTES_A = FRAG16 * 16 + T * STAGE * 2;
    constexpr int LDS_BYTES_B = (T - 1) * BANK * 4;
    constexpr int LDS_BYTES = LDS_BYTES_A > LDS_BYTES_B ? LDS_BYTES_A : LDS_BYTES_B;
    __shared__ __attribute__((aligned(16))) unsigned char s_raw[LDS_BYTES];
    u32x4* s_frag = reinterpret_cast<u32x4*>(s_raw);
    unsigned short* s_fh = reinterpret_cast<unsigned short*>(s_raw);
    unsigned short* s_stage = reinterpret_cast<unsigned short*>(s_raw + FRAG16 * 16);
    const int tid = threadIdx.x;
    const int sub = tid >> 8;
    const int t256 = tid & 255;
    const int lane = tid & 63;
    const int wave = t256 >> 6;
    const int i = lane & 15;
    const int q = lane >> 4;
    const int bx = ln_partition_tile(blockIdx.x, gridDim.x, row_part, 64 * T);
    const int sub0 = bx * (64 * T) + sub * 64;
    const int m0 = sub0 + wave * 16;
    const int my_row = m0 + i;

    constexpr int N4 = E * V * F / 4;
    constexpr int NST = (N4 + THREADS - 1) / THREADS;
    float4 wv[NST];
#pragma unroll
    for (int s = 0; s < NST; ++s) {
        const int x4 = tid + s * THREADS;
        wv[s] = (N4 % THREADS == 0 || x4 < N4) ? reinterpret_cast<const float4*>(filter)[x4] : make_float4(0.f, 0.f, 0.f, 0.f);
    }
    const int vt = wave / FT, ft = wave % FT;
    u32x4 va[2][3];
#pragma unroll
    for (int st = 0; st < 2; ++st) {
        float x[8];
#pragma unroll
        for (int j = 0; j < 8; ++j) {
            const int row = sub0 + 32 * st + 8 * q + j;
            const float xv = values[(size_t)min(row, m - 1) * V + vt * 16 + i];
            x[j] = (row < m) ? xv : 0.f;
        }
#pragma unroll
        for (int j = 0; j < 4; ++j) {
            unsigned int h0, m0_, l0, h1, m1_, l1;
            ln_split3_bits(x[2 * j], h0, m0_, l0);
            ln_split3_bits(x[2 * j + 1], h1, m1_, l1);
            va[st][0][j] = ln_pack_hi(h0, h1);
            va[st][1][j] = ln_pack_hi(m0_, m1_);
            va[st][2][j] = ln_pack_hi(l0, l1);
        }
    }
#ifndef LN_BWD_DEPTH
#define LN_BWD_DEPTH 2
#endif
    constexpr int DEPTH = LN_BWD_DEPTH;
    auto slot_of = [](int k) { return k == 0 ? E - 1 : k - 1; };
    const int lr = lane >> 3, c8 = lane & 7;
    int nb2[2][E];
#pragma unroll
    for (int j = 0; j < 2; ++j)
#pragma unroll
        for (int e = 0; e < E; ++e) {
            const int id = nbr[(size_t)min(m0 + 8 * j + lr, m - 1) * E + (e < E - 1 ? (e ^ 1) : e)];
            nb2[j][e] = (m0 + 8 * j + lr < m) ? id : -1;
        }
    floatx4 a[DEPTH + 1][2];
    auto gather = [&](int e, floatx4 (&dst)[2]) {
#pragma unroll
        for (int j = 0; j < 2; ++j) dst[j] = *reinterpret_cast<const floatx4*>(grad_out + (size_t)(nb2[j][e] >= 0 ? nb2[j][e] : 0) * F + c8 * 4);
    };
#pragma unroll
    for (int j = 0; j < 2; ++j)
        a[0][j] = *reinterpret_cast<const floatx4*>(grad_out + (size_t)(m0 + 8 * j + lr < m ? m0 + 8 * j + lr : 0) * F + c8 * 4);
#pragma unroll
    for (int k = 1; k < DEPTH && k < E; ++k) gather(slot_of(k), a[k % (DEPTH + 1)]);
#pragma unroll
    for (int s = 0; s < NST; ++s) {
        const int x4 = tid + s * THREADS;
        if (N4 % THREADS == 0 || x4 < N4) {
            const int x = x4 * 4;
            const int ev = x / F;
            const int f0 = x - ev * F;
            const int e = ev / V;
            const int v = ev - e * V;
            const float v4[4] = {wv[s].x, wv[s].y, wv[s].z, wv[s].w};
            unsigned int h[4], md[4], lo[4];
#pragma unroll
            for (int j = 0; j < 4; ++j) ln_split3_bits(v4[j], h[j], md[j], lo[j]);
            const int fr = (((e * NT + (v >> 4)) * 3) * 64 + (f0 >> 3) * 16 + ((v & 15) ^ (2 * (f0 >> 3)))) * 8 + (f0 & 7);
            *reinterpret_cast<uint2*>(s_fh + fr) = make_uint2(ln_pack_hi(h[0], h[1]), ln_pack_hi(h[2], h[3]));
            *reinterpret_cast<uint2*>(s_fh + fr + 64 * 8) = make_uint2(ln_pack_hi(md[0], md[1]), ln_pack_hi(md[2], md[3]));
            *reinterpret_cast<uint2*>(s_fh + fr + 2 * 64 * 8) = make_uint2(ln_pack_hi(lo[0], lo[1]), ln_pack_hi(lo[2], lo[3]));
        }
    }
    floatx4 acc_v[NT];
#pragma unroll
    for (int nt = 0; nt < NT; ++nt) acc_v[nt] = floatx4{0.f, 0.f, 0.f, 0.f};
    floatx4 acc_w[E];
#pragma unroll
    for (int e = 0; e < E; ++e) acc_w[e] = floatx4{0.f, 0.f, 0.f, 0.f};
#pragma unroll
    for (int k = 0; k < E; ++k) {
        const int e = slot_of(k);
        unsigned short* sg = s_stage + (size_t)sub * STAGE + (k & 1) * (3 * PART);
        if (k + DEPTH < E) gather(slot_of(k + DEPTH), a[(k + DEPTH) % (DEPTH + 1)]);
#pragma unroll
        for (int j = 0; j < 2; ++j) {
            const floatx4 x = a[k % (DEPTH + 1)][j];
            const bool there = nb2[j][e] >= 0;
            unsigned int h[4], md[4], lo[4];
#pragma unroll
            for (int c = 0; c < 4; ++c) ln_split3_bits(there ? x[c] : 0.f, h[c], md[c], lo[c]);
            const int row = wave * 16 + 8 * j + lr;
            unsigned short* dst = sg + row * RS + (((c8 >> 1) ^ swz(row)) * 8 + (c8 & 1) * 4);
            *reinterpret_cast<uint2*>(dst) = make_uint2(ln_pack_hi(h[0], h[1]), ln_pack_hi(h[2], h[3]));
            *reinterpret_cast<uint2*>(dst + PART) = make_uint2(ln_pack_hi(md[0], md[1]), ln_pack_hi(md[2], md[3]));
            *reinterpret_cast<uint2*>(dst + 2 * PART) = make_uint2(ln_pack_hi(lo[0], lo[1]), ln_pack_hi(lo[2], lo[3]));
        }
        __syncthreads();
        u32x4 p1, p2, p3;
        {
            const unsigned short* src = sg + (wave * 16 + i) * RS + ((q ^ swz(wave * 16 + i)) * KQ);
            p1 = *reinterpret_cast<const u32x4*>(src);
            p2 = *reinterpret_cast<const u32x4*>(src + PART);
            p3 = *reinterpret_cast<const u32x4*>(src + 2 * PART);
        }
        const bf16x8 a1 = __builtin_bit_cast(bf16x8, p1), a2 = __builtin_bit_cast(bf16x8, p2), a3 = __builtin_bit_cast(bf16x8, p3);
#pragma unroll
        for (int nt = 0; nt < NT; ++nt) {
            const u32x4* pb = s_frag + ((e * NT + nt) * 3) * 64 + q * 16 + (i ^ (2 * q));
            const bf16x8 b1 = __builtin_bit_cast(bf16x8, pb[0]), b2 = __builtin_bit_cast(bf16x8, pb[64]), b3 = __builtin_bit_cast(bf16x8, pb[128]);
            acc_v[nt] = __builtin_amdgcn_mfma_f32_16x16x32_bf16(a3, b1, acc_v[nt], 0, 0, 0);
            acc_v[nt] = __builtin_amdgcn_mfma_f32_16x16x32_bf16(a1, b3, acc_v[nt], 0, 0, 0);
            acc_v[nt] = __builtin_amdgcn_mfma_f32_16x16x32_bf16(a2, b2, acc_v[nt], 0, 0, 0);
            acc_v[nt] = __builtin_amdgcn_mfma_f32_16x16x32_bf16(a2, b1, acc_v[nt], 0, 0, 0);
            acc_v[nt] = __builtin_amdgcn_mfma_f32_16x16x32_bf16(a1, b2, acc_v[nt], 0, 0, 0);
            acc_v[nt] = __builtin_amdgcn_mfma_f32_16x16x32_bf16(a1, b1, acc_v[nt], 0, 0, 0);
        }
        floatx4 w0 = floatx4{0.f, 0.f, 0.f, 0.f}, w1 = floatx4{0.f, 0.f, 0.f, 0.f};
#pragma unroll
        for (int st = 0; st < 2; ++st) {
            bf16x8 b[3];
#pragma unroll
            for (int part = 0; part < 3; ++part) {
                const int r_lo = 32 * st + 8 * q + (i >> 2), r_hi = r_lo + 4;
                const int piece = ft * 2 + ((i & 3) >> 1), inner = (i & 1) * 4;
                const unsigned short* base = sg + part * PART + r_lo * RS + (piece ^ swz(r_lo)) * 8 + inner;
                const unsigned short* base_hi = sg + part * PART + r_hi * RS + (piece ^ swz(r_hi)) * 8 + inner;
                const short4v lo4 = __builtin_amdgcn_ds_read_tr16_b64_v4i16((short4v __attribute__((address_space(3)))*)(base));
                const short4v hi4 = __builtin_amdgcn_ds_read_tr16_b64_v4i16((short4v __attribute__((address_space(3)))*)(base_hi));
                u32x4 packed;
                packed[0] = (unsigned int)(unsigned short)lo4[0] | ((unsigned int)(unsigned short)lo4[1] << 16);
                packed[1] = (unsigned int)(unsigned short)lo4[2] | ((unsigned int)(unsigned short)lo4[3] << 16);
                packed[2] = (unsigned int)(unsigned short)hi4[0] | ((unsigned int)(unsigned short)hi4[1] << 16);
                packed[3] = (unsigned int)(unsigned short)hi4[2] | ((unsigned int)(unsigned short)hi4[3] << 16);
                b[part] = __builtin_bit_cast(bf16x8, packed);
            }
            const bf16x8 v1 = __builtin_bit_cast(bf16x8, va[st][0]), v2 = __builtin_bit_cast(bf16x8, va[st][1]), v3 = __builtin_bit_cast(bf16x8, va[st][2]);
            floatx4& acc = st ? w1 : w0;
            acc = __builtin_amdgcn_mfma_f32_16x16x32_bf16(v3, b[0], acc, 0, 0, 0);
            acc = __builtin_amdgcn_mfma_f32_16x16x32_bf16(v1, b[2], acc, 0, 0, 0);
            acc = __builtin_amdgcn_mfma_f32_16x16x32_bf16(v2, b[1], acc, 0, 0, 0);
            acc = __builtin_amdgcn_mfma_f32_16x16x32_bf16(v2, b[0], acc, 0, 0, 0);
            acc = __builtin_amdgcn_mfma_f32_16x16x32_bf16(v1, b[1], acc, 0, 0, 0);
            acc = __builtin_amdgcn_mfma_f32_16x16x32_bf16(v1, b[0], acc, 0, 0, 0);
        }
        acc_w[e] = w0 + w1;
    }
#pragma unroll
    for (int nt = 0; nt < NT; ++nt) {
#pragma unroll
        for (int r = 0; r < 4; ++r) {
            const int row = m0 + q * 4 + r;
            if (row < m) grad_values[(size_t)row * V + nt * 16 + i] = acc_v[nt][r];
        }
    }
    __syncthreads();
    float* park_all = reinterpret_cast<float*>(s_raw);
    const int colp = (ft * 16 + i) ^ ((q & 1) << 4);
    if (sub > 0) {
        float* park = park_all + (size_t)(sub - 1) * BANK;
#pragma unroll
        for (int e = 0; e < E; ++e)
#pragma unroll
            for (int r = 0; r < 4; ++r) park[(e * V + vt * 16 + q * 4 + r) * F + colp] = acc_w[e][r];
    }
    if constexpr (T > 1) __syncthreads();
    if (sub == 0) {
        float* dst = slabs + (size_t)blockIdx.x * BANK;
#pragma unroll
        for (int e = 0; e < E; ++e)
#pragma unroll
            for (int r = 0; r < 4; ++r) {
                const int o = (e * V + vt * 16 + q * 4 + r) * F + ft * 16 + i;
                float sum = acc_w[e][r];
#pragma unroll
                for (int k2 = 1; k2 < T; ++k2) sum += park_all[(k2 - 1) * BANK + (e * V + vt * 16 + q * 4 + r) * F + colp];
                dst[o] = sum;
            }
    }
}

template <int T>
static void ln_bwd_launch_fused(const LnBwdPlan& p, const int* nbr, const float* values, const float* grad_out, const float* filter, int m,
                                float* grad_values, float* partial, const int* row_partition, hipStream_t st) {
    if constexpr (T <= LN_BWD_B3_MAX_T) {
        if (p.form == LN_BWD_FUSED_B3) {
            LN_LAUNCH("k_conv_backward_fused", (k_conv_backward_fused_b3<T>), dim3(p.grid), dim3(p.block), 0, st, nbr, values, grad_out, filter, m,
                      grad_values, partial, row_partition);
            return;
        }
    }
    LN_LAUNCH("k_conv_backward_fused", (k_conv_backward_fused<32, 32, 9, T>), dim3(p.grid), dim3(p.block), 0, st, nbr, values, grad_out, filter, m,
              grad_values, partial);
}

extern "C" size_t ln_conv_backward_workspace_bytes(int mq, int mn, int filter_extent, int val_dim, int nr_filters) {
    return ln_conv_backward_query(mq, mn, filter_extent, val_dim, nr_filters, ln_conv_b3_enabled());
}

extern "C" int ln_conv_backward(const int* nbr_q, const int* nbr_n, const float* values_neigh, const float* grad_out, const float* filter, int mq,
                                int mn, int filter_extent, int val_dim, int nr_filters, float* grad_values, float* grad_filter,
                                void* workspace, size_t workspace_bytes, const int* row_partition, void* stream) {
    hipStream_t st = (hipStream_t)stream;
    const LnBwdPlan p = ln_conv_backward_plan(LnBwdPlanIn{
        mq, mn, filter_extent, val_dim, nr_filters, nbr_q == nbr_n,
        nbr_q && nbr_n && values_neigh && grad_out && filter && grad_values && grad_filter, workspace ? workspace_bytes : 0,
        ln_aligned16(values_neigh) && ln_aligned16(grad_out) && ln_aligned16(filter), ln_conv_b3_enabled()});
    float* partial = static_cast<float*>(workspace);
    const int total = filter_extent * val_dim * nr_filters;
    if (p.form == LN_BWD_FUSED_B3 || p.form == LN_BWD_FUSED_F32) {
        switch (p.t) {
            case 1: ln_bwd_launch_fused<1>(p, nbr_n, values_neigh, grad_out, filter, mn, grad_values, partial, row_partition, st); break;
            case 2: ln_bwd_launch_fused<2>(p, nbr_n, values_neigh, grad_out, filter, mn, grad_values, partial, row_partition, st); break;
            case 3: ln_bwd_launch_fused<3>(p, nbr_n, values_neigh, grad_out, filter, mn, grad_values, partial, row_partition, st); break;
            default: ln_bwd_launch_fused<4>(p, nbr_n, values_neigh, grad_out, filter, mn, grad_values, partial, row_partition, st); break;
        }
        (void)ln_reduce_slabs_async(partial, p.grid, total, grad_filter, st);
        return ln_check_launch("ln_conv_backward");
    }
    if (p.form == LN_BWD_FULL_SUM) {
        const LnGfPlan gf = ln_gf_plan(mq, filter_extent, val_dim, nr_filters, ln_conv_b3_enabled());
        ln_gf_launch_partials(gf, nbr_q, values_neigh, grad_out, mq, filter_extent, val_dim, nr_filters, partial, st);
        ln_conv_launch_full<true, true>(nr_filters, val_dim / 16, dim3(p.grid), st, nbr_n, grad_out, filter, mn, grad_values, p.conv_blocks,
                                        (const float*)partial, gf.chunks, total, grad_filter);
        return ln_check_launch("ln_conv_backward");
    }
    LnSlabSum sum = {nullptr, 0, 0, nullptr};
    int rc = ln_conv_grad_filter_impl(nbr_q, values_neigh, grad_out, mq, filter_extent, val_dim, nr_filters, grad_filter, workspace, workspace_bytes,
                                      stream, &sum);
    if (rc) return rc;
    const size_t gf_bytes = ln_bwd_gf_bytes(mq, filter_extent, val_dim, nr_filters, ln_conv_b3_enabled());
    char* conv_ws = (workspace && workspace_bytes > gf_bytes) ? static_cast<char*>(workspace) + gf_bytes : nullptr;
    rc = ln_conv_forward_riding(nbr_n, grad_out, filter, mn, filter_extent, nr_filters, val_dim, LN_CONV_FLIP_NEIGHBOURS | LN_CONV_TRANSPOSED_FILTER,
                                grad_values, conv_ws, conv_ws ? workspace_bytes - gf_bytes : 0, row_partition, stream, sum);
    return rc ? rc : ln_check_launch("ln_conv_backward");
}

extern "C" size_t ln_linear_backward_workspace_bytes(int rows, int cin, int cout) {
    return ln_linear_backward_query(rows, cin, cout, ln_conv_b3_enabled());
}

extern "C" int ln_linear_backward(const int* ident, const float* x, const float* grad_y, const float* w, int rows, int cin, int cout,
                                  float* grad_x, float* grad_w, void* workspace, size_t workspace_bytes, void* stream) {
    LN_REQUIRE(rows >= 0 && cin >= 1 && cout >= 1 && grad_w, LN_ERR_ARG, "ln_linear_backward: bad sizes / null output");
    LN_REQUIRE(workspace && workspace_bytes >= ln_linear_backward_workspace_bytes(rows, cin, cout), LN_ERR_WORKSPACE,
               "ln_linear_backward: workspace too small");
    const size_t gf_bytes = ln_bwd_gf_bytes(rows, 1, cout, cin, ln_conv_b3_enabled());
    const bool conv = grad_x && rows > 0;
    LnSlabSum sum = {nullptr, 0, 0, nullptr};
    int rc = ln_conv_grad_filter_impl(ident, grad_y, x, rows, 1, cout, cin, grad_w, workspace, gf_bytes, stream, conv ? &sum : nullptr);
    if (rc) return rc;
    if (conv)
        rc = ln_conv_forward_riding(ident, grad_y, w, rows, 1, cout, cin, 0, grad_x, static_cast<char*>(workspace) + gf_bytes,
                                    workspace_bytes - gf_bytes, nullptr, stream, sum);
    return rc ? rc : ln_check_launch("ln_linear_backward");
}
```

lattice_net_amd/csrc/ln_conv_plan.h:

```cpp
#pragma once
#include <stddef.h>
#include <stdint.h>

#define LN_BWD_MAX_SUBTILES 4
#define LN_BWD_CUS 256
#ifndef LN_BWD_B3_MAX_T
#define LN_BWD_B3_MAX_T 3
#endif
#ifndef LN_CONV_LDS_E
#define LN_CONV_LDS_E 16
#endif
#define LN_CONV_B3_WAVES(V) ((V) <= 128 ? 3 : 2)
#ifndef LN_CONV_SPLIT_TILES
#define LN_CONV_SPLIT_TILES 512
#endif
#ifndef LN_CONV_WIDE_SPLIT_MIN_V
#define LN_CONV_WIDE_SPLIT_MIN_V 128
#endif
#ifndef LN_CONV_B3_MIN_ROWS
#define LN_CONV_B3_MIN_ROWS 4096
#endif
#ifndef LN_GF_ROWS
#define LN_GF_ROWS 320
#endif
#ifndef LN_GFB_SUB
#define LN_GFB_SUB 64
#endif
#ifndef LN_GFB_EG
#define LN_GFB_EG 3
#endif
#ifndef LN_GFB_W128F
#define LN_GFB_W128F 2
#endif
#define LN_GFB_SLAB_BYTES (24ll << 20)

constexpr int ln_cdiv(long long a, long long b) { return int((a + b - 1) / b); }

constexpr bool ln_conv_per_slot_v(int V) {
    return V == 8 || V == 16 || V == 32 || V == 48 || V == 64 || V == 96 || V == 128 || V == 192 || V == 256;
}
constexpr int ln_conv_nt_max(int V) { return (V * 16 * 8 * 4 <= 32 * 1024) ? 8 : ((V * 16 * 4 * 4 <= 48 * 1024) ? 4 : 2); }
constexpr bool ln_conv_chunk_fits(int V, int NT) { return (NT == 8 || NT == 4 || NT == 2 || NT == 1) && NT <= ln_conv_nt_max(V); }
constexpr bool ln_conv_chunk_b3_spills(int V, int NT) { return V >= 256 && NT > 1; }
constexpr bool ln_conv_chunk_b3(int V, int NT) { return V % 32 == 0 && V * 16 * NT * 6 <= 64 * 1024 && !ln_conv_chunk_b3_spills(V, NT); }
constexpr bool ln_conv_b3_three_subtiles(int V) { return LN_CONV_B3_WAVES(V) == 3; }
constexpr int ln_conv_b3_subtiles(int V, int m, int chunks) {
    return ln_conv_b3_three_subtiles(V) && (long long)ln_cdiv(m, 192) * chunks >= LN_BWD_CUS * 3 / 4 ? 3 : 1;
}
constexpr bool ln_conv_wide_built(int V, int NT) { return V % 32 == 0 && NT >= 1 && NT <= 4; }
constexpr bool ln_conv_wide_shape(int V, int F) { return V % 32 == 0 && V >= 96 && F % 32 == 0; }
constexpr int ln_conv_r32_ntw(int NT) { return NT == 4 ? 2 : (NT == 3 ? 3 : 1); }
constexpr int ln_conv_r32_ch(int NT) { return NT % 2 == 0 ? 2 : 1; }
constexpr int ln_conv_r32_rt(int NT) { return NT % 2 == 0 ? 6 : 4; }
constexpr int LN_CONV_R32SK_RT = 6;
constexpr bool ln_conv_full_shape(int V, int F) {
    return (V == 8 || V == 16 || V == 32) && (F == 16 || F == 32 || F == 64 || F == 128) && V * F <= 1024;
}
constexpr bool ln_conv_small_filter(int E, int V, int F) { return E == 9 && (size_t)E * V * F * 4 <= 64 * 1024 && V <= 32; }
constexpr bool ln_bwd_fused_shape(int E, int V, int F) { return E == 9 && V == 32 && F == 32; }

constexpr int ln_bwd_subtiles(int m, bool b3_enabled) {
    const int max_t = b3_enabled ? LN_BWD_B3_MAX_T : LN_BWD_MAX_SUBTILES;
    const int s = (m + 63) / 64;
    int best = 1, best_cost = 1 << 30;
    for (int t = 1; t <= max_t; ++t) {
        const int wgs = (s + t - 1) / t;
        const int cost = ((wgs + LN_BWD_CUS - 1) / LN_BWD_CUS) * (t + 1);
        if (cost <= best_cost) {
            best = t;
            best_cost = cost;
        }
    }
    return best;
}
constexpr int ln_bwd_workgroups(int m, bool b3_enabled) { return ln_cdiv(m, 64 * ln_bwd_subtiles(m, b3_enabled)); }

constexpr size_t ln_conv_bank_bytes(int m, int E, int V, int F, bool b3_enabled) {
    if (V % 32 != 0 || F % 16 != 0 || m < LN_CONV_B3_MIN_ROWS || E > LN_CONV_LDS_E || !b3_enabled) return 0;
    return (((size_t)E * V * F * 3 * sizeof(unsigned short)) + 255) & ~size_t(255);
}
constexpr int ln_conv_slots_per_split(int V, int m, int E, int F) {
    if (!ln_conv_per_slot_v(V)) return E;
    const long long tiles = (long long)ln_cdiv(m, 64) * ln_cdiv(F, 16 * ln_conv_nt_max(V));
    if (tiles * 2 > LN_CONV_SPLIT_TILES || E < 2) return E;
    int nsplit = int((LN_CONV_SPLIT_TILES + tiles - 1) / tiles);
    if (nsplit > E) nsplit = E;
    return (E + nsplit - 1) / nsplit;
}
constexpr bool ln_conv_wide_fills_chip(int m, int F) { return (long long)ln_cdiv(m, 192) * ln_cdiv(F, 128) >= LN_BWD_CUS / 2; }
constexpr int ln_conv_wide_split(int V, int m, int E, int F, bool have_bank) {
    if (!have_bank || !ln_conv_per_slot_v(V) || V % 32 != 0 || V < LN_CONV_WIDE_SPLIT_MIN_V || F % 32 != 0 || E < 3 || m < LN_CONV_B3_MIN_ROWS)
        return 0;
    if (ln_conv_wide_fills_chip(m, F)) return 0;
    const long long wgs = (long long)ln_cdiv(m, 192) * (F >= 128 ? F / 128 : 1);
    int best = 1;
    long long best_cost = 1ll << 60;
    for (int n = 2; n <= E; ++n) {
        const long long cost = ((wgs * n + LN_BWD_CUS - 1) / LN_BWD_CUS) * ((E + n - 1) / n);
        if (cost < best_cost) {
            best = n;
            best_cost = cost;
        }
    }
    return best;
}
struct LnConvLayout {
    size_t bank_bytes;
    int wide_split;
    int nsplit, e_per;
};
constexpr LnConvLayout ln_conv_layout(int m, int E, int V, int F, bool b3_enabled, bool have_bank) {
    LnConvLayout l = {ln_conv_bank_bytes(m, E, V, F, b3_enabled), 0, 1, ln_conv_slots_per_split(V, m, E, F)};
    l.wide_split = ln_conv_wide_split(V, m, E, F, l.bank_bytes > 0 && have_bank);
    if (l.wide_split > 1) l.e_per = (E + l.wide_split - 1) / l.wide_split;
    l.nsplit = (E + l.e_per - 1) / l.e_per;
    return l;
}
constexpr size_t ln_conv_slab_bytes(int nsplit, int m, int F) { return nsplit > 1 ? (size_t)nsplit * m * F * sizeof(float) : 0; }
constexpr size_t ln_conv_bank_query(int m, int E, int V, int F, bool b3_enabled) {
    if (m <= 0 || F % 16 != 0 || ln_conv_small_filter(E, V, F)) return 0;
    return ln_conv_bank_bytes(m, E, V, F, b3_enabled);
}
constexpr size_t ln_conv_forward_query(int m, int E, int V, int F, bool b3_enabled) {
    if (m <= 0 || F % 16 != 0) return 256;
    return ln_conv_bank_query(m, E, V, F, b3_enabled) + ln_conv_slab_bytes(ln_conv_layout(m, E, V, F, b3_enabled, true).nsplit, m, F) + 256;
}

enum LnConvKernel : uint8_t {
    LN_K_FORWARD_B3,
    LN_K_FULL,
    LN_K_SPLIT_BANK32,
    LN_K_ROWS32,
    LN_K_ROWS32SK,
    LN_K_SPLIT_BANK,
    LN_K_MFMA_B3,
    LN_K_MFMA,
    LN_K_SUM_PARTIALS,
    LN_K_GENERIC,
};
struct LnConvLaunch {
    uint8_t kernel;
    uint8_t nt, t;
    bool carries_sum;
    int grid[3], block;
    int f_off, cols;
    int split_x;
    size_t bank_off;
    size_t bank_elems;
};
#define LN_CONV_MAX_LAUNCHES 10
struct LnConvPlanIn {
    int m, E, V, F;
    bool flip, wt;
    bool b3_enabled;
    bool values_aligned, filter_aligned;
    bool ws_aligned;
    size_t ws_bytes;
    bool bank_ready;
    int riding_total;
};
struct LnConvPlan {
    size_t bank_bytes, slab_bytes;
    int nsplit, e_per;
    bool sum_left;
    int n;
    LnConvLaunch launch[LN_CONV_MAX_LAUNCHES];
};

inline LnConvLaunch* ln_plan_add(LnConvPlan& p, LnConvKernel k, int nt, int t, int gx, int gy, int gz, int block, int f_off, int cols) {
    LnConvLaunch& l = p.launch[p.n++];
    l = LnConvLaunch{uint8_t(k), uint8_t(nt), uint8_t(t), false, {gx, gy, gz}, block, f_off, cols, 0, 0, 0};
    return &l;
}

inline LnConvPlan ln_conv_plan(const LnConvPlanIn& in) {
    const int m = in.m, E = in.E, V = in.V, F = in.F;
    LnConvPlan p = {};
    p.nsplit = 1;
    p.e_per = E;
    p.sum_left = in.riding_total > 0;
    if (E == 9 && in.filter_aligned) {
        if (!in.flip && !in.wt && V == 32 && F == 32 && m >= LN_CONV_B3_MIN_ROWS && in.b3_enabled && in.values_aligned) {
            const int bt = ln_bwd_subtiles(m, true), t = bt < 3 ? bt : 3;
            ln_plan_add(p, LN_K_FORWARD_B3, 2, t, ln_cdiv(m, 64 * t), 1, 1, 256 * t, 0, F);
            return p;
        }
        if (ln_conv_full_shape(V, F)) {
            ln_plan_add(p, LN_K_FULL, F / 16, 1, ln_cdiv(m, 64), 1, 1, 256, 0, F);
            return p;
        }
    }
    if (!(F % 16 == 0 && in.values_aligned && in.filter_aligned && ln_conv_per_slot_v(V))) {
        ln_plan_add(p, LN_K_GENERIC, 0, 0, ln_cdiv((long long)m * F, 256), 1, 1, 256, 0, F);
        return p;
    }
    const size_t bank_bytes = ln_conv_bank_bytes(m, E, V, F, in.b3_enabled);
    const bool b3 = bank_bytes > 0 && in.ws_aligned && in.ws_bytes >= bank_bytes;
    const LnConvLayout lay = ln_conv_layout(m, E, V, F, in.b3_enabled, b3);
    p.bank_bytes = b3 ? bank_bytes : 0;
    p.nsplit = lay.nsplit;
    p.e_per = lay.e_per;
    if (p.nsplit > 1 && (!in.ws_aligned || in.ws_bytes - p.bank_bytes < ln_conv_slab_bytes(p.nsplit, m, F))) {
        p.e_per = E;
        p.nsplit = 1;
    }
    p.slab_bytes = ln_conv_slab_bytes(p.nsplit, m, F);
    const int nsplit = p.nsplit;
    int f_off = 0;
    size_t bank_off = 0;
    auto split = [&](LnConvKernel k, int nt, int cnt, int cols_per_chunk) {
        if (in.bank_ready) return;
        const int sx = ln_cdiv(V * cols_per_chunk, 256);
        LnConvLaunch* l = ln_plan_add(p, k, nt, 1, sx, E, cnt, 256, f_off, cnt * cols_per_chunk);
        l->split_x = sx;
        l->bank_off = bank_off;
        l->bank_elems = (size_t)E * cnt * V * cols_per_chunk * 3;
        if (p.sum_left) {
            l->carries_sum = true;
            l->grid[0] += ln_cdiv(in.riding_total / 64, E * cnt);
            p.sum_left = false;
        }
    };
    auto conv = [&](LnConvKernel k, int nt, int t, int rows, int block, int cnt, int cols_per_chunk, bool banked) {
        LnConvLaunch* l = ln_plan_add(p, k, nt, t, ln_cdiv(m, rows), cnt, nsplit, block, f_off, cnt * cols_per_chunk);
        if (banked) {
            l->bank_off = bank_off;
            l->bank_elems = (size_t)E * cnt * V * cols_per_chunk * 3;
            bank_off += l->bank_elems;
        }
        f_off += cnt * cols_per_chunk;
    };
    if (b3 && ln_conv_wide_shape(V, F) && ((lay.wide_split > 1 && nsplit > 1) || (nsplit == 1 && ln_conv_wide_fills_chip(m, F)))) {
        const bool rest_sk = F % 128 == 96;
        for (int nt = 4; nt >= 1; --nt) {
            const int cnt = (F - f_off) / (32 * nt);
            if (cnt == 0) continue;
            const bool sk = rest_sk && nt == 3;
            const int rt = sk ? LN_CONV_R32SK_RT : ln_conv_r32_rt(nt);
            split(LN_K_SPLIT_BANK32, nt, cnt, 32 * nt);
            conv(sk ? LN_K_ROWS32SK : LN_K_ROWS32, nt, 1, 32 * rt, sk ? 128 * rt : 64 * rt * ln_conv_r32_ch(nt), cnt, 32 * nt, true);
        }
    }
    for (int nt = 8; nt >= 1; nt >>= 1) {
        if (!ln_conv_chunk_fits(V, nt) || (b3 && ln_conv_chunk_b3_spills(V, nt))) continue;
        const int cnt = (F - f_off) / (16 * nt);
        if (cnt == 0) continue;
        if (b3 && ln_conv_chunk_b3(V, nt)) {
            split(LN_K_SPLIT_BANK, nt, cnt, 16 * nt);
            const int t = ln_conv_b3_subtiles(V, m, cnt * nsplit);
            conv(LN_K_MFMA_B3, nt, t, 64 * t, 256 * t, cnt, 16 * nt, true);
        } else {
            conv(LN_K_MFMA, nt, 1, 64, 256, cnt, 16 * nt, false);
        }
    }
    if (nsplit > 1) ln_plan_add(p, LN_K_SUM_PARTIALS, 0, 0, ln_cdiv((long long)m * F / 4, 256), 1, 1, 256, 0, F);
    return p;
}

constexpr bool ln_gf_mfma_supported(int V, int F) { return V % 16 == 0 && F % 16 == 0; }
struct LnGfBlock {
    int vs, fs;
};
constexpr LnGfBlock ln_gfb_block(int V, int F) {
    constexpr int cand[7][2] = {{128, 128}, {64, 64}, {32, 96}, {96, 32}, {64, 32}, {32, 64}, {32, 32}};
    for (int k = 0; k < 7; ++k)
        if (V % cand[k][0] == 0 && F % cand[k][1] == 0) return LnGfBlock{cand[k][0], cand[k][1]};
    return LnGfBlock{0, 0};
}
constexpr int ln_gfb_wv(int vs, int fs) { return vs == 128 && fs == 128 ? 4 : 2; }
constexpr int ln_gfb_wf(int vs, int fs) { return vs == 128 && fs == 128 ? LN_GFB_W128F : 2; }
constexpr int ln_gfb_rows(int m, int E, int V, int F) {
    const LnGfBlock b = ln_gfb_block(V, F);
    if (E != 9 || b.vs == 0) return 0;
    const long long z = (long long)(V / b.vs) * (F / b.fs) * (E / LN_GFB_EG);
    const long long slab = (long long)E * V * F * 4;
    const bool one_per_cu = b.vs * b.fs > 64 * 96;
    long long chunks = ((one_per_cu ? 256 : 512) + z - 1) / z;
    const long long budget = one_per_cu ? 2 * LN_GFB_SLAB_BYTES : LN_GFB_SLAB_BYTES;
    const long long cap = budget / slab > 0 ? budget / slab : 1;
    if (chunks > cap) chunks = cap;
    long long rows = ((m + chunks - 1) / chunks + LN_GFB_SUB - 1) / LN_GFB_SUB * LN_GFB_SUB;
    if (rows < LN_GFB_SUB) rows = LN_GFB_SUB;
    return int(rows);
}
constexpr size_t ln_gf_query(int m, int E, int V, int F, bool b3_enabled) {
    if (!ln_gf_mfma_supported(V, F) || m <= 0) return 256;
    int chunks = ln_cdiv(m, LN_GF_ROWS);
    if (ln_bwd_fused_shape(E, V, F) && ln_bwd_workgroups(m, b3_enabled) > chunks) chunks = ln_bwd_workgroups(m, b3_enabled);
    const int rows_b3 = ln_gfb_rows(m, E, V, F);
    if (rows_b3 > 0 && ln_cdiv(m, rows_b3) > chunks) chunks = ln_cdiv(m, rows_b3);
    return (size_t)chunks * E * V * F * sizeof(float) + 256;
}
constexpr size_t ln_round256(size_t b) { return (b + 255) & ~size_t(255); }
constexpr size_t ln_bwd_gf_bytes(int m, int E, int V, int F, bool b3_enabled) { return ln_round256(ln_gf_query(m, E, V, F, b3_enabled)); }
constexpr size_t ln_linear_backward_query(int rows, int cin, int cout, bool b3_enabled) {
    return ln_bwd_gf_bytes(rows, 1, cout, cin, b3_enabled) + ln_conv_forward_query(rows, 1, cout, cin, b3_enabled) + 256;
}
constexpr size_t ln_conv_backward_query(int mq, int mn, int E, int V, int F, bool b3_enabled) {
    const size_t conv = ln_conv_forward_query(mn, E, F, V, b3_enabled);
    return conv > 256 ? ln_bwd_gf_bytes(mq, E, V, F, b3_enabled) + conv : ln_gf_query(mq, E, V, F, b3_enabled);
}

enum LnGfForm : uint8_t {
    LN_GF_GENERIC,
    LN_GF_B3,
    LN_GF_F32,
};
struct LnGfPlan {
    uint8_t form;
    int vs, fs, wv, wf;
    int tile;
    int rows, chunks;
    int grid[3], block;
    size_t lds;
};
constexpr LnGfPlan ln_gf_plan(int m, int E, int V, int F, bool b3_enabled) {
    LnGfPlan p = {};
    p.block = 256;
    if (!ln_gf_mfma_supported(V, F)) {
        p.form = LN_GF_GENERIC;
        p.grid[0] = ln_cdiv((long long)E * V * F, 256);
        p.grid[1] = p.grid[2] = 1;
        return p;
    }
    const LnGfBlock b = ln_gfb_block(V, F);
    if (E == 9 && m >= LN_CONV_B3_MIN_ROWS && b3_enabled && b.vs > 0) {
        p.form = LN_GF_B3;
        p.vs = b.vs, p.fs = b.fs, p.wv = ln_gfb_wv(b.vs, b.fs), p.wf = ln_gfb_wf(b.vs, b.fs);
        p.rows = ln_gfb_rows(m, E, V, F);
        p.chunks = ln_cdiv(m, p.rows);
        p.grid[0] = p.chunks, p.grid[1] = E / LN_GFB_EG, p.grid[2] = (V / b.vs) * (F / b.fs);
        p.block = 64 * p.wv * p.wf;
        p.lds = (size_t)3 * LN_GFB_SUB * ((b.vs + 16) + (b.fs + 16)) * sizeof(unsigned short);
        return p;
    }
    p.form = LN_GF_F32;
    p.tile = (V % 64 == 0 && F % 64 == 0) ? 4 : ((V % 32 == 0 && F % 32 == 0) ? 2 : 1);
    p.rows = LN_GF_ROWS;
    p.chunks = ln_cdiv(m, LN_GF_ROWS);
    p.grid[0] = p.chunks, p.grid[1] = E, p.grid[2] = (V / (16 * p.tile)) * (F / (16 * p.tile));
    return p;
}

enum LnBwdForm : uint8_t {
    LN_BWD_FUSED_B3,
    LN_BWD_FUSED_F32,
    LN_BWD_FULL_SUM,
    LN_BWD_TWO_CALLS,
};
struct LnBwdPlanIn {
    int mq, mn, E, val_dim, nr_filters;
    bool same_list;
    bool buffers;
    size_t ws_bytes;
    bool aligned;
    bool b3_enabled;
};
struct LnBwdPlan {
    uint8_t form;
    int t;
    int grid, block;
    int conv_blocks;
};
constexpr LnBwdPlan ln_conv_backward_plan(const LnBwdPlanIn& in) {
    LnBwdPlan p = {LN_BWD_TWO_CALLS, 0, 0, 256, 0};
    if (!(in.E == 9 && in.mq > 0 && in.mn > 0 && ln_gf_mfma_supported(in.val_dim, in.nr_filters) && in.buffers && in.ws_bytes > 0 &&
          in.ws_bytes >= ln_gf_query(in.mq, in.E, in.val_dim, in.nr_filters, in.b3_enabled) && in.aligned))
        return p;
    if (in.same_list && in.mq == in.mn && ln_bwd_fused_shape(in.E, in.val_dim, in.nr_filters)) {
        p.t = ln_bwd_subtiles(in.mn, in.b3_enabled);
        p.form = in.b3_enabled && p.t <= LN_BWD_B3_MAX_T ? LN_BWD_FUSED_B3 : LN_BWD_FUSED_F32;
        p.grid = ln_cdiv(in.mn, 64 * p.t);
        p.block = 256 * p.t;
    } else if (ln_conv_full_shape(in.nr_filters, in.val_dim)) {
        p.form = LN_BWD_FULL_SUM;
        p.conv_blocks = ln_cdiv(in.mn, 64);
        p.grid = p.conv_blocks + ln_cdiv((long long)in.E * in.val_dim * in.nr_filters, 16);
    }
    return p;
}
```

lattice_net_amd/lattice.py:

```python
from __future__ import annotations

import ctypes as C
import itertools
import os
import re
import weakref
from typing import Optional, Sequence

import torch
import torch.utils.weak

from . import _lib

__all__ = ["Lattice", "HashTable", "set_row_order", "get_row_order", "set_hash_capacity_policy", "set_slot_order", "set_bank_cache", "set_deterministic"]


_SIZE_CACHE = {}
_FORCE_ATOMIC_BUILD = os.environ.get("LATTICE_BUILD_PATH", "") == "atomic"

_ROW_ORDER = [os.environ.get("LATTICE_ROW_ORDER", "slot")]


_HASH_POLICY = [os.environ.get("LATTICE_HASH_CAPACITY", "tokens")]
_STATIC_SLOTS_PER_ROW = float(os.environ.get("LATTICE_STATIC_SLOTS_PER_ROW", "2.3"))
# ... 764 lines not shown
        _lib.check(_lib.load().ln_cloud_key_extents(C.byref(t), _lib.ptr(positions_raw), self._sigmas_host(), n, band.guard, buf.data_ptr(),
                                                    buf.data_ptr() + 8 * clouds, stream), "ln_cloud_key_extents")
        ht._band_last = (buf, clouds)
        ht._band_pending = True
        _BAND_REPORTS[ht._pinned.data_ptr()] = (buf, clouds, band.guard, step, d)

    def cloud_key_extents(self) -> torch.Tensor:
        last = self.m_hash_table._band_last
        if last is None:
            raise _lib.LatticeNetHipError("cloud_key_extents: no checked build has happened on this lattice (set_cloud_batch(check_band=True))")
        buf, clouds = last
        return buf[: 2 * clouds].view(clouds, 2)

    @staticmethod
    def band_violation_message(report) -> str:
        info = _BAND_REPORTS.get(int(report.ctypes.data)) if report is not None else None
        if info is None:
            return "a cloud of the batch leaves its key band (Lattice.set_cloud_batch)"
        buf, clouds, guard, step, d = info
        vals = buf.tolist()
        half, bad = step >> 1, vals[2 * clouds]
        where = (f"cloud {bad} has first key coordinates [{vals[2 * bad]}, {vals[2 * bad + 1]}]" if 0 <= bad < clouds
                 else "no cloud of the LAST checked build on this stream offends (the extents buffer was reused since)")
        return (f"a cloud of the batch leaves its key band: {where}, the band is [{-half + guard}, {half - guard}) "
                f"(half a key step of {step} = quotient_step {step // (d + 1)} x {d + 1}, less a guard of {guard}); its vertices merge with "
                "the next cloud's and per-cloud results are wrong.  Raise quotient_step (lattice_net_amd.suggest_quotient_step), use larger "
                "sigmas or centre the clouds")

    def canonicalize_rows(self, idx: torch.Tensor):
        ht = self.m_hash_table
        st = ht._storage
        lib = _lib.load()
        tokens = int(idx.numel())
        hit = st.csr_cache.get((idx.data_ptr(), idx._version, idx.numel()))
        ws = self._workspace(_build_sizes(tokens, st.hashed())[0])
        t = ht.c_table()
        _lib.check(lib.ln_canonicalize(C.byref(t), _lib.ptr(idx), tokens, C.byref(hit[1]) if hit is not None else None, _lib.ptr(ws), ws.numel(),
                                       self._stream()), "ln_canonicalize")
        keep = {k: v for k, v in st.csr_cache.items() if hit is not None and v is hit}
        st.touch()
        st.csr_cache.update(keep)

    def _csr(self, idx: torch.Tensor):
        st = self.m_hash_table._storage
        key = (idx.data_ptr(), idx._version, idx.numel())
        hit = st.csr_cache.get(key)
        if hit is not None:
            return hit
        lib = _lib.load()
        tokens = idx.numel()
        rows_upper = self.m_hash_table.capacity()
        csr_buf, csr, max_seg = self._alloc_csr(tokens, rows_upper)
        ws = self._workspace(_build_sizes(tokens, rows_upper)[1])
        _lib.check(lib.ln_csr_build(_lib.ptr(idx), tokens, rows_upper, C.byref(csr), _lib.ptr(ws), ws.numel(), self._stream()), "ln_csr_build")
        if _DETERMINISTIC[0]:
            _lib.check(lib.ln_csr_sort(C.byref(csr), rows_upper, _lib.ptr(ws), ws.numel(), tokens, self._stream()), "ln_csr_sort")
        if len(st.csr_cache) >= 4:
            st.csr_cache.pop(next(iter(st.csr_cache)))
        entry = (csr_buf, csr, max_seg, None, idx)
        st.csr_cache[key] = entry
        return entry

    def _dense_hint(self, tokens: int) -> int:
        ht = self.m_hash_table
        m = ht._static_rows if ht._static_rows is not None else ht.m_nr_filled
        return (1 if (m is not None and m > 0 and tokens >= _DENSE_TOKENS_PER_VERTEX * m) else 0) | (2 if _DETERMINISTIC[0] else 0)

    def _scatter_rows(self, src: torch.Tensor, idx: torch.Tensor, w: torch.Tensor, dst: torch.Tensor, val_dim: int, src_div: int,
                      src_stride: int):
        if idx.numel() == 0:
            return
        _, csr, max_seg, grp_row, _ = self._csr(idx)
        csr.dense = self._dense_hint(idx.numel())
        lib = _lib.load()
        fn, what = (lib.ln_csr_reduce_rows_f16, "ln_csr_reduce_rows_f16") if src.dtype == torch.float16 else \
            (lib.ln_csr_reduce_rows, "ln_csr_reduce_rows")
        _lib.check(fn(C.byref(csr), _lib.ptr(grp_row), max_seg, _lib.ptr(src), _lib.ptr(w), val_dim, src_div, src_stride, _lib.ptr(dst),
                      self._stream()), what)

    def scatter_max(self, src: torch.Tensor, idx: torch.Tensor):
        if src.dim() != 2 or src.dtype != torch.float32 or not src.is_contiguous() or src.shape[0] != idx.numel():
            raise ValueError("src must be a contiguous float [nr_tokens, C] tensor matching the splat indices")
        _require_cuda(src, "src")
        m = self.nr_lattice_vertices()
        c = int(src.shape[1])
        _, csr, max_seg, grp_row, _ = self._csr(idx)
        dev = self._dev()
        out_max = torch.empty((m, c), dtype=torch.float32, device=dev)
        out_arg = torch.empty((m, c), dtype=torch.int32, device=dev)
        packed = torch.empty((m * c,), dtype=torch.int64, device=dev)
        lib = _lib.load()
        _lib.check(lib.ln_csr_segment_max(C.byref(csr), _lib.ptr(grp_row), max_seg, _lib.ptr(src), c, m, _lib.ptr(packed), _lib.ptr(out_max),
                                          _lib.ptr(out_arg), self._stream()), "ln_csr_segment_max")
        return out_max, out_arg

    def vertex_point_counts(self, idx: torch.Tensor) -> torch.Tensor:
        m = self.nr_lattice_vertices()
        _, csr, _, grp_row, _ = self._csr(idx)
        counts = torch.empty((m,), dtype=torch.int32, device=self._dev())
        lib = _lib.load()
        groups_upper = self.m_hash_table._storage.hashed() if grp_row is not None else self.m_hash_table.capacity()
        _lib.check(lib.ln_csr_group_sizes(C.byref(csr), _lib.ptr(grp_row), groups_upper, m, _lib.ptr(counts), self._stream()),
                   "ln_csr_group_sizes")
        return counts

    def begin_splat(self, reset_hashmap: bool = True):
        if reset_hashmap:
            self.m_hash_table.clear(lazy=True)
        else:
            self.m_hash_table.clear_only_values()
        self.m_hash_table.m_nr_filled_is_dirty = True

    def splat_standalone(self, positions_raw: torch.Tensor, values: torch.Tensor):
        self._check_positions_and_values(positions_raw, values)
        n, d = positions_raw.shape
        v = values.shape[1]
        self.m_positions = positions_raw
        ht = self.m_hash_table
        if not ht.is_initialized():
            ht.init(d, v, self._dev(positions_raw))
        tv = ht.m_values_tensor
        cap = ht._static_rows if ht._static_rows is not None else ht.capacity()
        if tv is None or tuple(tv.shape) != (cap, v) or tv.requires_grad or tv._base is not None or not tv.is_contiguous():
            pending = getattr(ht, "_clear_pending", False)
            ht._clear_pending = False
            if pending:
                self._choose_hash_capacity(n * (d + 1), fresh=True)
                reach = min(cap, ht._storage.hashed())
                ht.m_values_tensor = torch.empty((cap, v), dtype=torch.float32, device=self._dev(positions_raw))
                if reach < cap:
                    ht.m_values_tensor[reach:].zero_()
                ht._zero_beyond = (weakref.ref(ht.m_values_tensor), reach)
            else:
                ht.m_values_tensor = torch.zeros((cap, v), dtype=torch.float32, device=self._dev(positions_raw))
                ht._zero_beyond = (weakref.ref(ht.m_values_tensor), 0)
            ht._clear_pending = pending
        idx, w = self._build(positions_raw, True)
        tv = ht.m_values_tensor
        self._after_build(lambda: self._accumulate_and_prefetch(values, idx, w, tv, v, d + 1, n * (d + 1)))
        self._trace_level()
        return idx, w

    def just_create_verts(self, positions_raw: torch.Tensor, return_indices_and_weights: bool):
        self._check_positions(positions_raw)
        d = positions_raw.shape[1]
        self._ensure_table(d, 1, positions_raw)
        idx, w = self._build(positions_raw, bool(return_indices_and_weights))
        self._trace_level()
        return idx, w

    def distribute(self, positions_raw: torch.Tensor, values: torch.Tensor, reset_hashmap: bool = True):
        self._check_positions_and_values(positions_raw, values)
        n, d = positions_raw.shape
        v = values.shape[1]
        dev = self._dev(positions_raw)
        self.m_positions = positions_raw
        oh = self.m_hash_table
        if not oh.is_initialized():
            if reset_hashmap:
                oh._pos_dim_hint, oh._val_dim_hint = d, v
            else:
                oh.init(d, v, dev)
        distributed = torch.empty((n * (d + 1), d + v + 1), dtype=torch.float32, device=dev)
        new = Lattice._clone_of(self)
        new.m_name = "distributed_lattice"
        nh = new.m_hash_table
        if reset_hashmap:
            nh._storage = _TableStorage(oh.capacity(), d, dev)
            nh.m_values_tensor = torch.zeros((oh.capacity(), oh.val_dim() or v), dtype=torch.float32, device=dev)
            nh._zero_beyond = (weakref.ref(nh.m_values_tensor), 0)
            nh._counters = nh._storage.fresh_counters
            nh.clear(lazy=True)
        else:
            nh._storage = oh._storage.clone()
            nh.m_values_tensor = torch.zeros_like(oh.m_values_tensor)
            nh._counters = oh._counters.clone()
        idx, w = new._build(positions_raw, True, vals=values, distributed=distributed)
        new._after_build(lambda: new._prefetch_neighbours(n * (d + 1)))
        new._trace_level()
        return new, distributed, idx, w

    def expand(self, positions_raw: torch.Tensor, point_multiplier: int, noise_stddev: float, expand_values: bool):
        self._check_positions(positions_raw)
        d = positions_raw.shape[1]
        self._ensure_table(d, 1, positions_raw)
        pos = positions_raw.repeat(point_multiplier, 1)
        pos = pos + torch.randn_like(pos) * noise_stddev
        new = Lattice._clone_of(self)
        new.m_name = "expanded_lattice"
        oh, nh = self.m_hash_table, new.m_hash_table
        nh._storage = oh._storage.clone()
        nh.m_values_tensor = torch.zeros((1, self.val_dim()), dtype=torch.float32, device=self._dev())
        nh._counters = oh._counters.clone()
        new.just_create_verts(pos.contiguous(), False)
        if expand_values:
            diff = new.nr_lattice_vertices() - self.nr_lattice_vertices()
            if diff < 0:
                raise _lib.LatticeNetHipError("expand produced fewer vertices than the source lattice")
            new.set_values(torch.nn.functional.pad(self.values()[: self.nr_lattice_vertices()], (0, 0, 0, diff)))
        return new

    def _accumulate_and_prefetch(self, values, idx, w, dst, val_dim, src_div, tokens):
        ht = self.m_hash_table
        st = ht._storage
        rows_upper = min(ht.capacity(), tokens)
        _, csr, max_seg, grp_row, _ = self._csr(idx)
        if rows_upper <= 0 or max_seg <= 0 or not self.prefetch_neighbours:
            return self._scatter_rows(values, idx, w, dst, val_dim, src_div, val_dim)
        lib = _lib.load()
        nbr = torch.empty((rows_upper, self.get_filter_extent(1)), dtype=torch.int32, device=self._dev())
        t = ht.c_table()
        fn, what = (lib.ln_splat_accumulate_and_neighbours_f16, "ln_splat_accumulate_and_neighbours_f16") if values.dtype == torch.float16 \
            else (lib.ln_splat_accumulate_and_neighbours, "ln_splat_accumulate_and_neighbours")
        csr.dense = self._dense_hint(tokens)
        _lib.check(fn(C.byref(csr), _lib.ptr(grp_row), max_seg, _lib.ptr(values), _lib.ptr(w), val_dim, src_div, val_dim, _lib.ptr(dst),
                      C.byref(t), rows_upper, _lib.ptr(nbr), self._stream()), what)
        st.nbr_cache[("prefetch", st.uid, st.version, self.m_lvl)] = (nbr,)

    def _prefetch_neighbours(self, tokens: int):
        ht = self.m_hash_table
        st = ht._storage
        rows_upper = min(ht.capacity(), tokens)
        if rows_upper <= 0:
            return
        lib = _lib.load()
        E = self.get_filter_extent(1)
        nbr = torch.empty((rows_upper, E), dtype=torch.int32, device=self._dev())
        t = ht.c_table()
        _lib.check(lib.ln_neighbours(C.byref(t), rows_upper, C.byref(t), self.m_lvl, self.m_lvl, 1, 0, _lib.ptr(nbr), self._stream()),
                   "ln_neighbours")
        st.nbr_cache[("prefetch", st.uid, st.version, self.m_lvl)] = (nbr,)


    def neighbours(self, lattice_neighbours: Optional["Lattice"], dilation: int, flip_neighbours: bool) -> torch.Tensor:
        nb = lattice_neighbours if lattice_neighbours is not None else self
        if abs(self.m_lvl - nb.m_lvl) > 1:
            raise ValueError(f"query lvl {self.m_lvl} and neighbours lvl {nb.m_lvl} must differ by at most 1")
        m = self.nr_lattice_vertices()
        if m == 0:
            raise _lib.LatticeNetHipError("this lattice has zero vertices")
        sq, sn = self.m_hash_table._storage, nb.m_hash_table._storage
        key = (sn.uid, sn.version, self.m_lvl, nb.m_lvl, int(dilation), bool(flip_neighbours), m)
        hit = sq.nbr_cache.get(key)
        if hit is not None:
            return hit[0]
        E = self.get_filter_extent(1)
        pre = sq.nbr_cache.get(("prefetch", sn.uid, sn.version, self.m_lvl)) if (sn is sq and not flip_neighbours and dilation == 1 and
                                                                                  nb.m_lvl == self.m_lvl) else None
        if pre is not None and pre[0].shape[0] >= m:
            nbr = pre[0][:m]
            sq.nbr_cache[key] = (nbr,)
            return nbr
        if flip_neighbours:
            base = self.neighbours(nb, dilation, False)
            perm = [e ^ 1 for e in range(E - 1)] + [E - 1]
            nbr = base[:, perm].contiguous()
        else:
            lib = _lib.load()
            nbr = torch.empty((m, E), dtype=torch.int32, device=self._dev())
            tq, tn = self.m_hash_table.c_table(), nb.m_hash_table.c_table()
            _lib.check(lib.ln_neighbours(C.byref(tq), m, C.byref(tn), self.m_lvl, nb.m_lvl, int(dilation), 0, _lib.ptr(nbr),
                                         self._stream()), "ln_neighbours")
        sq.nbr_cache[key] = (nbr,)
        return nbr

    def _row_partition(self):
        st = self.m_hash_table._storage
        if st is None or not st.rows_follow_space or st.row_regions is None:
            return None
        return st.row_regions.data_ptr()

    def _check_filter_extent(self, filter_extent: int):
        if filter_extent != self.get_filter_extent(1):
            raise ValueError(f"filter extent should be {self.get_filter_extent(1)} (1-hop neighbourhood + centre), got {filter_extent}")

    def convolve_im2row_standalone(self, filter_bank: torch.Tensor, dilation: int, lattice_neighbours: Optional["Lattice"],
                                   flip_neighbours: bool, filter_is_transposed: bool = False) -> "Lattice":
        nb = lattice_neighbours if lattice_neighbours is not None else self
        if filter_bank is None or filter_bank.dim() != 2:
            raise ValueError("filter bank should be 2-D: (filter_extent * val_dim) x nr_filters")
        filter_bank = filter_bank.contiguous()
        v = nb.val_dim()
        E = self.get_filter_extent(1)
        if filter_is_transposed:
            if filter_bank.shape[1] != v or filter_bank.shape[0] % E != 0:
                raise ValueError(f"transposed filter bank should be (filter_extent * nr_filters) x val_dim={v}, got {tuple(filter_bank.shape)}")
            nr_filters = int(filter_bank.shape[0]) // E
            filter_extent = E
        else:
            nr_filters = int(filter_bank.shape[1])
            filter_extent = filter_bank.shape[0] // v
            self._check_filter_extent(filter_extent)
            if filter_bank.shape[0] != filter_extent * v:
                raise ValueError("filter bank rows must be filter_extent * val_dim")
        nbr = self.neighbours(nb, dilation, False)
        m = nbr.shape[0]
        vals = nb.values()
        half = vals.dtype == torch.float16
        if filter_bank.dtype != vals.dtype:
            raise ValueError(f"filter bank is {filter_bank.dtype}, lattice values are {vals.dtype}")
        out = torch.empty((m, nr_filters), dtype=vals.dtype, device=self._dev())
        flags = (_lib.LN_CONV_FLIP_NEIGHBOURS if flip_neighbours else 0) | (_lib.LN_CONV_TRANSPOSED_FILTER if filter_is_transposed else 0)
        lib = _lib.load()
        if half:
            _lib.check(lib.ln_conv_forward_f16(_lib.ptr(nbr), _lib.ptr(vals), _lib.ptr(filter_bank), m, filter_extent, v, nr_filters, flags,
                                               _lib.ptr(out), self._stream()), "ln_conv_forward_f16")
        else:
            wsb = int(lib.ln_conv_forward_workspace_bytes(m, filter_extent, v, nr_filters))
            ws = None
            key = None
            bank_b = int(lib.ln_conv_bank_workspace_bytes(m, filter_extent, v, nr_filters))
            if bank_b > 0 and wsb == bank_b + 256 and _BANK_CACHE[0] and not filter_bank.requires_grad and \
                    not torch.cuda.is_current_stream_capturing():
                key = (filter_bank.data_ptr(), filter_bank._version, m, filter_extent, v, nr_filters, flags, self._stream())
                hit = _BANK_ENTRIES.get(filter_bank)
                if hit is not None and hit[0] == key:
                    ws, flags = hit[1], flags | _lib.LN_CONV_BANK_READY
            if ws is None and wsb > 256:
                ws = torch.empty((wsb,), dtype=torch.uint8, device=self._dev())
            _lib.check(lib.ln_conv_forward_ws(_lib.ptr(nbr), _lib.ptr(vals), _lib.ptr(filter_bank), m, filter_extent, v, nr_filters, flags,
                                              _lib.ptr(out), _lib.ptr(ws), 0 if ws is None else ws.numel(), self._row_partition(),
                                              self._stream()), "ln_conv_forward")
            if key is not None and not (flags & _lib.LN_CONV_BANK_READY):
                try:
                    _BANK_ENTRIES[filter_bank] = (key, ws)
                except TypeError:
                    pass
        conv = Lattice._clone_of(self)
        conv.m_name = "convolved_lattice"
        conv.m_hash_table.set_values(out)
        return conv

    def convolve_im2row_backward(self, grad_out: torch.Tensor, filter_bank: torch.Tensor, dilation: int,
                                 query: Optional["Lattice"], neighbours: Optional["Lattice"], filter_grad_fp32: bool = False):
        q = query if query is not None else self
        nb = neighbours if neighbours is not None else self
        lib = _lib.load()
        main = self._stream()
        E = q.get_filter_extent(1)
        grad_out = grad_out.contiguous()
        filter_bank = filter_bank.contiguous()
        v = nb.val_dim()
        f = int(filter_bank.shape[1])
        if filter_bank.shape[0] != E * v or grad_out.shape[1] != f:
            raise ValueError("filter bank / gradient shapes do not match the forward convolution")
        nbr_q = q.neighbours(nb, dilation, False)
        mq = nbr_q.shape[0]
        if grad_out.shape[0] != mq:
            raise ValueError(f"grad_out has {grad_out.shape[0]} rows, the query lattice has {mq} vertices")
        dev = self._dev()
        half = grad_out.dtype == torch.float16
        if filter_bank.dtype != grad_out.dtype or nb.values().dtype != grad_out.dtype:
            raise ValueError("grad_out, filter bank and lattice values must share one dtype (float32 or float16)")
        gf = torch.empty((E * v, f), dtype=torch.float32, device=dev)
        ws_bytes = int(lib.ln_conv_grad_filter_f16_workspace_bytes(mq, E, v, f) if half else
                       lib.ln_conv_backward_workspace_bytes(mq, int(nb.nr_lattice_vertices()), E, v, f))
        ws = torch.empty((max(ws_bytes, 256),), dtype=torch.uint8, device=dev)
        nbr_n = nb.neighbours(q, dilation, False)
        mn = nbr_n.shape[0]
        gvals = torch.empty((mn, v), dtype=grad_out.dtype, device=dev)
        if half:
            _lib.check(lib.ln_conv_grad_filter_f16(_lib.ptr(nbr_q), _lib.ptr(nb.values()), _lib.ptr(grad_out), mq, E, v, f, _lib.ptr(gf),
                                                   _lib.ptr(ws), ws.numel(), main), "ln_conv_grad_filter_f16")
            flags = _lib.LN_CONV_FLIP_NEIGHBOURS | _lib.LN_CONV_TRANSPOSED_FILTER
            _lib.check(lib.ln_conv_forward_f16(_lib.ptr(nbr_n), _lib.ptr(grad_out), _lib.ptr(filter_bank), mn, E, f, v, flags, _lib.ptr(gvals),
                                               main), "ln_conv_forward_f16")
            return gvals, (gf if filter_grad_fp32 else gf.to(torch.float16))
        part = nb._row_partition() if q.m_hash_table._storage is nb.m_hash_table._storage else None
        _lib.check(lib.ln_conv_backward(_lib.ptr(nbr_q), _lib.ptr(nbr_n), _lib.ptr(nb.values()), _lib.ptr(grad_out), _lib.ptr(filter_bank), mq,
                                        mn, E, v, f, _lib.ptr(gvals), _lib.ptr(gf), _lib.ptr(ws), ws.numel(), part, main), "ln_conv_backward")
        return gvals, gf

    def convolve_im2row_grad_filter(self, grad_out: torch.Tensor, dilation: int, lattice_neighbours: Optional["Lattice"],
                                    filter_extent: int) -> torch.Tensor:
        nb = lattice_neighbours if lattice_neighbours is not None else self
        self._check_filter_extent(filter_extent)
        grad_out = grad_out.contiguous()
        nbr = self.neighbours(nb, dilation, False)
        m = nbr.shape[0]
        v = nb.val_dim()
        f = int(grad_out.shape[1])
        if grad_out.shape[0] != m:
            raise ValueError(f"grad_out has {grad_out.shape[0]} rows, lattice has {m} vertices")
        lib = _lib.load()
        gf = torch.empty((filter_extent * v, f), dtype=torch.float32, device=self._dev())
        ws = self._workspace(lib.ln_conv_grad_filter_workspace_bytes(m, filter_extent, v, f))
        _lib.check(lib.ln_conv_grad_filter(_lib.ptr(nbr), _lib.ptr(nb.values()), _lib.ptr(grad_out), m, filter_extent, v, f,
                                           _lib.ptr(gf), _lib.ptr(ws), ws.numel(), self._stream()), "ln_conv_grad_filter")
        return gf

    def im2row(self, lattice_neighbours: Optional["Lattice"], filter_extent: int, dilation: int, flip_neighbours: bool):
        nb = lattice_neighbours if lattice_neighbours is not None else self
        self._check_filter_extent(filter_extent)
        nbr = self.neighbours(nb, dilation, flip_neighbours)
        m = nbr.shape[0]
        v = nb.val_dim()
        out = torch.empty((m, filter_extent * v), dtype=torch.float32, device=self._dev())
        lib = _lib.load()
        _lib.check(lib.ln_im2row(_lib.ptr(nbr), _lib.ptr(nb.values()), m, filter_extent, v, _lib.ptr(out), self._stream()), "ln_im2row")
        return out

    def im2rowindices(self, lattice_neighbours: Optional["Lattice"], filter_extent: int, dilation: int, flip_neighbours: bool):
        nb = lattice_neighbours if lattice_neighbours is not None else self
        self._check_filter_extent(filter_extent)
        nbr = self.neighbours(nb, dilation, flip_neighbours)
        m = nbr.shape[0]
        v = nb.val_dim()
        out = torch.empty((m, filter_extent * v), dtype=torch.int32, device=self._dev())
        lib = _lib.load()
        _lib.check(lib.ln_im2rowindices(_lib.ptr(nbr), m, filter_extent, v, _lib.ptr(out), self._stream()), "ln_im2rowindices")
        return out

    def row2im(self, lattice_rowified: torch.Tensor, dilation: int, filter_extent: int, nr_filters: int,
               lattice_neighbours: Optional["Lattice"]):
        nb = lattice_neighbours if lattice_neighbours is not None else self
        if not lattice_rowified.is_contiguous():
            raise ValueError("lattice rowified is not contiguous, call .contiguous() on it")
        v = lattice_rowified.shape[1] // filter_extent
        if v != self.val_dim():
            raise ValueError(f"each rowified row should be val_dim*filter_extent long: row {lattice_rowified.shape[1]}, val_dim {self.val_dim()}")
        nbr = self.neighbours(nb, dilation, False)
        m = nbr.shape[0]
        out = torch.empty((m, v), dtype=torch.float32, device=self._dev())
        lib = _lib.load()
        _lib.check(lib.ln_row2im(_lib.ptr(nbr), _lib.ptr(lattice_rowified), m, filter_extent, v, _lib.ptr(out), self._stream()), "ln_row2im")
        self.m_hash_table.m_values_tensor = out
        return out

    def _new_coarse(self) -> "Lattice":
        capacity = self.m_hash_table.capacity()
        d = self.pos_dim()
        dev = self._dev()
        coarse = Lattice._clone_of(self)
        coarse.m_name = "coarse_lattice"
        coarse.m_lvl = self.m_lvl + 1
        coarse.m_sigmas = [s * 2.0 for s in self.m_sigmas]
        coarse._sigmas_tensor = None
        ht = HashTable(capacity)
        bp, step = self.m_hash_table._batch
        ht._batch = (bp, (step // (2 * (d + 1))) * (d + 1)) if bp else (0, 0)
        ht._cloud_lengths, ht._cloud_starts = self.m_hash_table._cloud_lengths, self.m_hash_table._cloud_starts
        ht._per_cloud_norm = self.m_hash_table._per_cloud_norm
        ht._per_cloud_invalid_vertex = self.m_hash_table._per_cloud_invalid_vertex
        ht._many_clouds = self.m_hash_table._many_clouds
        ht._band = self.m_hash_table._band
        ht._storage = _TableStorage(capacity, d, dev, spare_row_width=self.val_dim())
        ht.m_values_tensor = ht._storage.fresh_row if ht._storage.fresh_row is not None else torch.zeros((1, self.val_dim()), dtype=torch.float32, device=dev)
        ht._counters = ht._storage.fresh_counters
        levels = getattr(self.m_hash_table, "_static_levels", None)
        if self.m_hash_table._static_rows is not None:
            if not levels or coarse.m_lvl not in levels:
                raise _lib.LatticeNetHipError(f"static-rows mode: no row bound for lattice level {coarse.m_lvl} "
                                              "(set_static_rows(bound, coarse_bounds=[...]))")
            ht._static_rows = min(int(levels[coarse.m_lvl]), capacity)
        ht._static_levels = levels
        coarse.m_hash_table = ht
        ht.clear(lazy=True)
        return coarse

    def create_coarse_verts(self) -> "Lattice":
        coarse = self._new_coarse()
        coarse.m_hash_table._storage.key_format = _lib.LN_KEYS_RAW
        lib = _lib.load()
        m = self.nr_lattice_vertices()
        tokens = m * (2 * (self.pos_dim() + 1) + 1)
        coarse._choose_hash_capacity(tokens, fresh=True)
        cap = coarse.m_hash_table._storage.hashed()
        ws = self._workspace(_build_sizes(tokens, cap)[0])
        csr_buf, csr, _ = self._alloc_csr(tokens, cap)
        tf, tc = self.m_hash_table.c_table(), coarse.m_hash_table.c_table()
        _lib.check(lib.ln_coarsen(C.byref(tf), m, C.byref(tc), C.byref(csr), _lib.ptr(ws), ws.numel(), self._stream()), "ln_coarsen")
        coarse.m_hash_table._storage.touch()
        coarse.m_hash_table.m_nr_filled_is_dirty = True
        nr = coarse.nr_lattice_vertices()
        coarse.m_hash_table.m_values_tensor = torch.zeros((nr, self.val_dim()), dtype=torch.float32, device=self._dev())
        coarse._trace_level()
        return coarse

    def create_coarse_verts_naive(self, positions_raw: torch.Tensor) -> "Lattice":
        self._check_positions(positions_raw)
        coarse = self._new_coarse()
        coarse.just_create_verts(positions_raw, False)
        coarse._trace_level()
        return coarse

    def _check_slice_inputs(self, positions_raw, idx, w):
        self._check_positions(positions_raw)
        if self.val_dim() <= 0:
            raise ValueError("val_dim is 0: splat something first")
        if positions_raw.shape[1] != self.pos_dim():
            raise ValueError("position dimension does not match the lattice")
        n = positions_raw.shape[0]
        expect = n * (self.pos_dim() + 1)
        if idx is None or w is None or idx.numel() != expect or w.numel() != expect:
            raise ValueError(f"indices / weights must have {expect} elements")
        return n

    def slice_standalone_with_precomputation(self, positions_raw, splatting_indices_tensor, splatting_weights_tensor,
                                             grad_accumulator: Optional[torch.Tensor] = None):
        idx, w = splatting_indices_tensor.contiguous(), splatting_weights_tensor.contiguous()
        n = self._check_slice_inputs(positions_raw, idx, w)
        vals = self.values()
        lib = _lib.load()
        if vals.dtype == torch.float16:
            out = torch.empty((n, self.val_dim()), dtype=torch.float16, device=self._dev())
            if grad_accumulator is None:
                _lib.check(lib.ln_slice_forward_f16(_lib.ptr(vals), _lib.ptr(idx), _lib.ptr(w), n, self.pos_dim(), self.val_dim(), _lib.ptr(out),
                                                    self._stream()), "ln_slice_forward_f16")
            else:
                _lib.check(lib.ln_slice_forward_f16_prepare_backward(_lib.ptr(vals), _lib.ptr(idx), _lib.ptr(w), n, self.pos_dim(), self.val_dim(),
                                                                     _lib.ptr(out), _lib.ptr(grad_accumulator), grad_accumulator.numel(),
                                                                     self._stream()), "ln_slice_forward_f16_prepare_backward")
            return out
        out = torch.empty((n, self.val_dim()), dtype=torch.float32, device=self._dev())
        st = self.m_hash_table._storage
        hit = st.csr_cache.get((idx.data_ptr(), idx._version, idx.numel())) if (st is not None and st.rows_follow_space and _ORDERED_SLICE[0]) else None
        if hit is not None and hit[3] is not None:
            t = self.m_hash_table.c_table()
            _lib.check(lib.ln_slice_forward_ordered(C.byref(t), C.byref(hit[1]), _lib.ptr(vals), _lib.ptr(idx), _lib.ptr(w), n, self.val_dim(),
                                                    _lib.ptr(out), _lib.ptr(grad_accumulator),
                                                    0 if grad_accumulator is None else grad_accumulator.numel(), self._stream()),
                       "ln_slice_forward_ordered")
            return out
        if grad_accumulator is None:
            _lib.check(lib.ln_slice_forward(_lib.ptr(vals), _lib.ptr(idx), _lib.ptr(w), n, self.pos_dim(), self.val_dim(), _lib.ptr(out),
                                            self._stream()), "ln_slice_forward")
        else:
            _lib.check(lib.ln_slice_forward_prepare_backward(_lib.ptr(vals), _lib.ptr(idx), _lib.ptr(w), n, self.pos_dim(), self.val_dim(),
                                                             _lib.ptr(out), _lib.ptr(grad_accumulator), grad_accumulator.numel(),
                                                             self._stream()), "ln_slice_forward_prepare_backward")
        return out

    def slice_standalone_no_precomputation(self, positions_raw):
        self._check_positions(positions_raw)
        if positions_raw.shape[1] != self.pos_dim():
            raise ValueError("position dimension does not match the lattice")
        n, d = positions_raw.shape
        dev = self._dev()
        out = torch.empty((n, self.val_dim()), dtype=torch.float32, device=dev)
        idx = torch.empty((n * (d + 1),), dtype=torch.int32, device=dev)
        w = torch.empty((n * (d + 1),), dtype=torch.float32, device=dev)
        lib = _lib.load()
        t = self.m_hash_table.c_table()
        _lib.check(lib.ln_slice_no_precomputation(C.byref(t), _lib.ptr(self.values()), _lib.ptr(positions_raw), self._sigmas_host(), n,
                                                  self.val_dim(), _lib.ptr(out), _lib.ptr(idx), _lib.ptr(w), self._stream()),
                   "ln_slice_no_precomputation")
        return out, idx, w

    def gather_standalone_with_precomputation(self, positions_raw, splatting_indices_tensor, splatting_weights_tensor):
        idx, w = splatting_indices_tensor.contiguous(), splatting_weights_tensor.contiguous()
        n = self._check_slice_inputs(positions_raw, idx, w)
        d, v = self.pos_dim(), self.val_dim()
        out = torch.empty((n, (d + 1) * (v + 1)), dtype=torch.float32, device=self._dev())
        lib = _lib.load()
        _lib.check(lib.ln_gather_forward(_lib.ptr(self.values()), _lib.ptr(idx), _lib.ptr(w), n, d, v, _lib.ptr(out), self._stream()),
                   "ln_gather_forward")
        return out

    def gather_standalone_no_precomputation(self, positions_raw):
        raise NotImplementedError("gather_no_precomputation is dead code in the reference (LatticeGPU.cuh:2875 names an undeclared symbol)")

    def slice_classify_no_precomputation(self, *args, **kwargs):
        raise NotImplementedError("slice_classify_no_precomputation is dead code in the reference (LatticeGPU.cuh:3356)")

    def slice_backwards_standalone_with_precomputation(self, *args, **kwargs):
        raise NotImplementedError("the homogeneous slice backward kernel is commented out in the reference (LatticeGPU.cuh:3467-3536)")

    def slice_classify_with_precomputation(self, positions_raw, delta_weights, linear_clasify_weight, linear_clasify_bias, nr_classes,
                                           splatting_indices_tensor, splatting_weights_tensor):
        idx, w = splatting_indices_tensor.contiguous(), splatting_weights_tensor.contiguous()
        n = self._check_slice_inputs(positions_raw, idx, w)
        dw, lw, lb = delta_weights.contiguous(), linear_clasify_weight.contiguous(), linear_clasify_bias.contiguous()
        logits = torch.empty((n, nr_classes), dtype=torch.float32, device=self._dev())
        lib = _lib.load()
        _lib.check(lib.ln_slice_classify_forward(_lib.ptr(self.values()), _lib.ptr(dw), _lib.ptr(lw), _lib.ptr(lb), _lib.ptr(idx),
                                                 _lib.ptr(w), n, self.pos_dim(), self.val_dim(), int(nr_classes), _lib.ptr(logits),
                                                 self._stream()), "ln_slice_classify_forward")
        return logits

    def slice_backwards_standalone_with_precomputation_no_homogeneous(self, positions_raw, grad_sliced_values, splatting_indices_tensor,
                                                                      splatting_weights_tensor, zeroed_accumulator=None):
        idx, w = splatting_indices_tensor.contiguous(), splatting_weights_tensor.contiguous()
        n = self._check_slice_inputs(positions_raw, idx, w)
        if grad_sliced_values.dim() != 2 or not grad_sliced_values.is_contiguous():
            raise ValueError("grad_sliced_values should be contiguous nr_positions x val_dim")
        v = int(grad_sliced_values.shape[1])
        m = self.nr_lattice_vertices()
        gv = zeroed_accumulator
        if gv is None or tuple(gv.shape) != (m, v) or gv.dtype != torch.float32 or not gv.is_contiguous():
            gv = torch.zeros((m, v), dtype=torch.float32, device=self._dev())
        self._scatter_rows(grad_sliced_values, idx, w, gv, v, self.pos_dim() + 1, v)
        if grad_sliced_values.dtype == torch.float16:
            gv = gv.half()
        self.m_hash_table.m_values_tensor = gv

    def slice_classify_backwards_with_precomputation(self, grad_class_logits, positions_raw, initial_values, delta_weights,
                                                     linear_clasify_weight, linear_clasify_bias, nr_classes, grad_lattice_values,
                                                     grad_delta_weights, grad_linear_clasify_weight, grad_linear_clasify_bias,
                                                     splatting_indices_tensor, splatting_weights_tensor):
        idx, w = splatting_indices_tensor.contiguous(), splatting_weights_tensor.contiguous()
        n = self._check_slice_inputs(positions_raw, idx, w)
        if grad_class_logits.dim() != 2 or not grad_class_logits.is_contiguous():
            raise ValueError("grad_class_logits should be contiguous nr_positions x nr_classes")
        for name, g in (("grad_lattice_values", grad_lattice_values), ("grad_delta_weights", grad_delta_weights),
                        ("grad_linear_clasify_weight", grad_linear_clasify_weight), ("grad_linear_clasify_bias", grad_linear_clasify_bias)):
            if not g.is_contiguous():
                raise ValueError(f"{name} must be contiguous (it is filled in place)")
        iv, dw, lw = initial_values.contiguous(), delta_weights.contiguous(), linear_clasify_weight.contiguous()
        lib = _lib.load()
        v, c, d = int(iv.shape[1]), int(nr_classes), self.pos_dim()
        dev = self._dev()
        grad_sliced = torch.empty((n, v), dtype=torch.float32, device=dev)
        w_eff = torch.empty((n * (d + 1),), dtype=torch.float32, device=dev)
        ws = self._workspace(lib.ln_slice_classify_backward_workspace_bytes(n, d, v, c))
        _lib.check(lib.ln_slice_classify_backward(_lib.ptr(grad_class_logits), _lib.ptr(iv), _lib.ptr(dw), _lib.ptr(lw), _lib.ptr(idx),
                                                  _lib.ptr(w), n, d, v, c, None, _lib.ptr(grad_delta_weights),
                                                  _lib.ptr(grad_linear_clasify_weight), _lib.ptr(grad_linear_clasify_bias),
                                                  _lib.ptr(grad_sliced), _lib.ptr(w_eff), _lib.ptr(ws), ws.numel(), self._stream()),
                   "ln_slice_classify_backward")
        self._scatter_rows(grad_sliced, idx, w_eff, grad_lattice_values, v, d + 1, v)

    def gather_backwards_standalone_with_precomputation(self, positions_raw, grad_sliced_values, splatting_indices_tensor,
                                                        splatting_weights_tensor):
        idx, w = splatting_indices_tensor.contiguous(), splatting_weights_tensor.contiguous()
        n = self._check_slice_inputs(positions_raw, idx, w)
        if grad_sliced_values.dim() != 2 or not grad_sliced_values.is_contiguous():
            raise ValueError("grad_sliced_values should be contiguous nr_positions x ((val_dim+1)*(pos_dim+1))")
        d = self.pos_dim()
        v = grad_sliced_values.shape[1] // (d + 1) - 1
        m = self.nr_lattice_vertices()
        gv = torch.zeros((m, v), dtype=torch.float32, device=self._dev())
        self._scatter_rows(grad_sliced_values, idx, w, gv, v, 1, v + 1)
        self.m_hash_table.m_values_tensor = gv

    def clone_lattice(self) -> "Lattice":
        return Lattice._clone_of(self)

    def increase_sigmas(self, stepsize: float):
        self.m_sigmas = [s + stepsize for s in self.m_sigmas]
        self._sigmas_tensor = None

    def set_sigma(self, sigma: float):
        if len(self.m_sigmas_val_and_extent) != 1:
            raise ValueError("set_sigma assumes exactly one sigma group")
        self.m_sigmas = [float(sigma)] * len(self.m_sigmas)
        self._sigmas_tensor = None

    def val_dim(self) -> int:
        return self.m_hash_table.val_dim()

    def pos_dim(self) -> int:
        d = self.m_hash_table.pos_dim()
        return d if d >= 0 else len(self.m_sigmas)

    def capacity(self) -> int:
        return self.m_hash_table.capacity()

    def name(self) -> str:
        return self.m_name

    def set_name(self, name: str):
        self.m_name = name

    def lvl(self) -> int:
        return self.m_lvl

    def rows_device(self):
        ht = self.m_hash_table
        return ht._counters[0:1] if (ht._static_rows is not None and ht._counters is not None) else None

    _level_trace = None
    _level_trace_segments = 1
    _static_build_log = None
# ... 321 lines not shown
```

Before: 1487.

## Add narrow multi-chunk conv kernels when several scans run concurrently

Adds an OVERLAPPED flag that the Python layer sets when more than one scan is in flight. With the flag set, the bf16x3 forward and fused-backward conv kernels run with a fixed narrow workgroup (T=2) that loops over C=2 row chunks. The filter fragments are staged into LDS once per workgroup and reused across both chunks. The goal is to use fewer, persistent workgroups so concurrent scans share the GPU better and filter splitting is amortised, at the cost of less parallelism per kernel and extra plan and workspace complexity.

```diff
diff --git a/include/latticenet_hip.h b/include/latticenet_hip.h
--- a/include/latticenet_hip.h
+++ b/include/latticenet_hip.h
@@ -131,6 +131,7 @@
 #define LN_CONV_FLIP_NEIGHBOURS 1
 #define LN_CONV_TRANSPOSED_FILTER 2
 #define LN_CONV_BANK_READY 4
+#define LN_CONV_OVERLAPPED 8
 int ln_conv_forward(const int* nbr, const float* values_neigh, const float* filter, int m, int filter_extent, int val_dim,
                     int nr_filters, int flags, float* out, void* stream);
 size_t ln_conv_bank_workspace_bytes(int m, int filter_extent, int val_dim, int nr_filters);
@@ -172,6 +173,9 @@
 int ln_conv_backward(const int* nbr_q, const int* nbr_n, const float* values_neigh, const float* grad_out, const float* filter, int mq, int mn,
                      int filter_extent, int val_dim, int nr_filters, float* grad_values, float* grad_filter, void* workspace,
                      size_t workspace_bytes, const int* row_partition, void* stream);
+int ln_conv_backward_flags(const int* nbr_q, const int* nbr_n, const float* values_neigh, const float* grad_out, const float* filter, int mq,
+                           int mn, int filter_extent, int val_dim, int nr_filters, int flags, float* grad_values, float* grad_filter,
+                           void* workspace, size_t workspace_bytes, const int* row_partition, void* stream);
 
 int ln_csr_reduce_rows_f16(const LnCsr* csr, const int* grp_row, long long max_segments, const void* src_f16, const float* w, int val_dim,
                            int src_div, int src_stride, float* dst, void* stream);
diff --git a/lattice_net_amd/_lib.py b/lattice_net_amd/_lib.py
--- a/lattice_net_amd/_lib.py
+++ b/lattice_net_amd/_lib.py
@@ -23,6 +23,7 @@
 LN_CONV_FLIP_NEIGHBOURS = 1
 LN_CONV_TRANSPOSED_FILTER = 2
 LN_CONV_BANK_READY = 4
+LN_CONV_OVERLAPPED = 8
 LN_MAX_POS_DIM = 6
 LN_KEYS_RAW = 0
 LN_KEYS_LATTICE = 1
@@ -140,6 +141,7 @@
     "ln_slice_forward_f16_prepare_backward": (_i, [_vp, _vp, _vp, _i, _i, _i, _vp, _vp, _ll, _vp]),
     "ln_conv_backward_workspace_bytes": (_sz, [_i, _i, _i, _i, _i]),
     "ln_conv_backward": (_i, [_vp, _vp, _vp, _vp, _vp, _i, _i, _i, _i, _i, _vp, _vp, _vp, _sz, _vp, _vp]),
+    "ln_conv_backward_flags": (_i, [_vp, _vp, _vp, _vp, _vp, _i, _i, _i, _i, _i, _i, _vp, _vp, _vp, _sz, _vp, _vp]),
     "ln_conv_forward_f16": (_i, [_vp, _vp, _vp, _i, _i, _i, _i, _i, _vp, _vp]),
     "ln_conv_grad_filter_f16_workspace_bytes": (_sz, [_i, _i, _i, _i]),
     "ln_conv_grad_filter_f16": (_i, [_vp, _vp, _vp, _i, _i, _i, _i, _vp, _vp, _sz, _vp]),
diff --git a/lattice_net_amd/csrc/ln_conv.hip b/lattice_net_amd/csrc/ln_conv.hip
--- a/lattice_net_amd/csrc/ln_conv.hip
+++ b/lattice_net_amd/csrc/ln_conv.hip
@@ -1110,6 +1110,138 @@
         }
 }
 
+template <int T, int C>
+__global__ void __launch_bounds__(256 * T) __attribute__((amdgpu_waves_per_eu(T, T)))
+    k_conv_forward_b3_rows(const int* __restrict__ nbr, const float* __restrict__ values, const float* __restrict__ filter, int m,
+                      float* __restrict__ out, const int* __restrict__ row_part) {
+    constexpr int V = 32, F = 32, E = 9, KQ = 8, NT = 2;
+    constexpr int THREADS = 256 * T;
+    constexpr int FRAG16 = E * NT * 3 * 64;
+    __shared__ __attribute__((aligned(16))) unsigned char s_raw[FRAG16 * 16];
+    const u32x4* s_frag = reinterpret_cast<const u32x4*>(s_raw);
+    __shared__ __attribute__((aligned(16))) floatx4 s_x[4 * T][16 * 8];
+    __shared__ int s_nbr[64 * T * E];
+    const int tid = threadIdx.x;
+    const int lane = tid & 63;
+    const int i = lane & 15;
+    const int q = lane >> 4;
+    const int bx0 = ln_partition_tile(blockIdx.x, gridDim.x, row_part, 64 * T * C) * C;
+    const int m00 = bx0 * (64 * T) + (tid >> 6) * 16;
+    constexpr int ITEMS = E * (V / 8) * F;
+    constexpr int NIT = (ITEMS + THREADS - 1) / THREADS;
+    float wv[NIT][8];
+#pragma unroll
+    for (int s = 0; s < NIT; ++s) {
+        const int x = min(tid + s * THREADS, ITEMS - 1);
+        const int f = x % F;
+        const int ev8 = x / F;
+#pragma unroll
+        for (int j = 0; j < 8; ++j) wv[s][j] = filter[(ev8 * 8 + j) * F + f];
+    }
+    bool staged = false;
+#pragma unroll
+    for (int c = 0; c < C; ++c) {
+    const int bx = bx0 + c;
+    const int m0 = m00 + c * (64 * T);
+    {
+        const size_t g0 = (size_t)bx * (64 * T) * E, g_end = (size_t)m * E;
+        for (int x = tid; x < 64 * T * E; x += THREADS) s_nbr[x] = (g0 + x < g_end) ? nbr[g0 + x] : -1;
+    }
+    {
+        bool any = false;
+        for (int x = tid; x < 64 * T * E; x += THREADS) any |= s_nbr[x] >= 0;
+        if (!__syncthreads_or(any)) {
+            for (int x = tid; x < 64 * T * (F / 4); x += THREADS) {
+                const int row = bx * (64 * T) + x / (F / 4);
+                if (row < m) *reinterpret_cast<float4*>(out + (size_t)row * F + (x % (F / 4)) * 4) = make_float4(0.f, 0.f, 0.f, 0.f);
+            }
+            if constexpr (C == 1) return;
+            else continue;
+        }
+    }
+    const int wv_ = tid >> 6;
+    const int lr = lane >> 3;
+    int nb[2][E];
+#pragma unroll
+    for (int j = 0; j < 2; ++j)
+#pragma unroll
+        for (int e = 0; e < E; ++e) nb[j][e] = s_nbr[(wv_ * 16 + 8 * j + lr) * E + e];
+    auto fsw = [](int r) -> int { return ((r >> 1) & 7) ^ (((r >> 2) & 1) << 1); };
+    floatx4* xw[2];
+#pragma unroll
+    for (int j = 0; j < 2; ++j) xw[j] = &s_x[wv_][(8 * j + lr) * 8 + ((lane & 7) ^ fsw(8 * j + lr))];
+    const floatx4* xr0 = &s_x[wv_][i * 8 + ((2 * q) ^ fsw(i))];
+    const floatx4* xr1 = &s_x[wv_][i * 8 + ((2 * q + 1) ^ fsw(i))];
+#ifndef LN_FWD_DEPTH
+#define LN_FWD_DEPTH 4
+#endif
+    constexpr int DEPTH = LN_FWD_DEPTH;
+    floatx4 a[DEPTH][2];
+    auto gather = [&](int e, floatx4 (&dst)[2]) {
+#pragma unroll
+        for (int j = 0; j < 2; ++j)
+            dst[j] = *reinterpret_cast<const floatx4*>(values + (size_t)(nb[j][e] >= 0 ? nb[j][e] : 0) * V + (lane & 7) * 4);
+    };
+#pragma unroll
+    for (int k = 0; k < DEPTH - 1 && k < E; ++k) gather(k, a[k]);
+    u32x4* s_frag_w = reinterpret_cast<u32x4*>(s_raw);
+    if (!staged) {
+    staged = true;
+#pragma unroll
+    for (int s = 0; s < NIT; ++s) {
+        const int x = tid + s * THREADS;
+        if (x < ITEMS) {
+            const int f = x % F;
+            const int ev8 = x / F;
+            const int e = ev8 / (V / 8);
+            const int vo = ev8 - e * (V / 8);
+            unsigned int h[8], md[8], lo[8];
+#pragma unroll
+            for (int j = 0; j < 8; ++j) ln_split3_bits(wv[s][j], h[j], md[j], lo[j]);
+            const int unit = ((e * NT + (f >> 4)) * 3) * 64 + vo * 16 + (f & 15);
+            s_frag_w[unit] = u32x4{ln_pack_hi(h[0], h[1]), ln_pack_hi(h[2], h[3]), ln_pack_hi(h[4], h[5]), ln_pack_hi(h[6], h[7])};
+            s_frag_w[unit + 64] = u32x4{ln_pack_hi(md[0], md[1]), ln_pack_hi(md[2], md[3]), ln_pack_hi(md[4], md[5]), ln_pack_hi(md[6], md[7])};
+            s_frag_w[unit + 128] = u32x4{ln_pack_hi(lo[0], lo[1]), ln_pack_hi(lo[2], lo[3]), ln_pack_hi(lo[4], lo[5]), ln_pack_hi(lo[6], lo[7])};
+        }
+    }
+    }
+    floatx4 acc[NT];
+#pragma unroll
+    for (int nt = 0; nt < NT; ++nt) acc[nt] = floatx4{0.f, 0.f, 0.f, 0.f};
+    __syncthreads();
+#pragma unroll
+    for (int e = 0; e < E; ++e) {
+        if (e + DEPTH - 1 < E) gather(e + DEPTH - 1, a[(e + DEPTH - 1) % DEPTH]);
+#pragma unroll
+        for (int j = 0; j < 2; ++j) *xw[j] = (nb[j][e] >= 0) ? a[e % DEPTH][j] : floatx4{0.f, 0.f, 0.f, 0.f};
+        __builtin_amdgcn_fence(__ATOMIC_RELEASE, "wavefront");
+        __builtin_amdgcn_wave_barrier();
+        __builtin_amdgcn_fence(__ATOMIC_ACQUIRE, "wavefront");
+        const floatx4 lo4 = *xr0, hi4 = *xr1;
+        __builtin_amdgcn_fence(__ATOMIC_RELEASE, "wavefront");
+        __builtin_amdgcn_wave_barrier();
+        __builtin_amdgcn_fence(__ATOMIC_ACQUIRE, "wavefront");
+        const float ae[KQ] = {lo4[0], lo4[1], lo4[2], lo4[3], hi4[0], hi4[1], hi4[2], hi4[3]};
+        u32x4 p[3];
+        ln_split3_pack8(ae, 0, p);
+        const bf16x8 ap[3] = {__builtin_bit_cast(bf16x8, p[0]), __builtin_bit_cast(bf16x8, p[1]), __builtin_bit_cast(bf16x8, p[2])};
+#pragma unroll
+        for (int nt = 0; nt < NT; ++nt) {
+            const u32x4* pb = s_frag + ((e * NT + nt) * 3) * 64 + lane;
+            const bf16x8 bp[3] = {__builtin_bit_cast(bf16x8, pb[0]), __builtin_bit_cast(bf16x8, pb[64]), __builtin_bit_cast(bf16x8, pb[128])};
+            ln_b3_mfma16(ap, bp, acc[nt]);
+        }
+    }
+#pragma unroll
+    for (int nt = 0; nt < NT; ++nt)
+#pragma unroll
+        for (int r = 0; r < 4; ++r) {
+            const int row = m0 + q * 4 + r;
+            if (row < m) out[(size_t)row * F + nt * 16 + i] = acc[nt][r];
+        }
+    }
+}
+
 template <bool FLIP, bool WT>
 struct LnConvCall {
     const int* nbr;
@@ -1236,7 +1368,10 @@
         switch (l.kernel) {
             case LN_K_FORWARD_B3:
                 if constexpr (!FLIP && !WT) {
-                    if (l.t == 1) LN_LAUNCH("k_conv_mfma", (k_conv_forward_b3<1>), grid, block, 0, c.st, c.nbr, c.values, c.filter, c.m, c.out, c.row_partition);
+                    if (l.c > 1)
+                        LN_LAUNCH("k_conv_mfma", (k_conv_forward_b3_rows<LN_CONV_OVL_T, LN_CONV_OVL_C>), grid, block, 0, c.st, c.nbr, c.values, c.filter, c.m, c.out,
+                                  c.row_partition);
+                    else if (l.t == 1) LN_LAUNCH("k_conv_mfma", (k_conv_forward_b3<1>), grid, block, 0, c.st, c.nbr, c.values, c.filter, c.m, c.out, c.row_partition);
                     else if (l.t == 2) LN_LAUNCH("k_conv_mfma", (k_conv_forward_b3<2>), grid, block, 0, c.st, c.nbr, c.values, c.filter, c.m, c.out, c.row_partition);
                     else LN_LAUNCH("k_conv_mfma", (k_conv_forward_b3<3>), grid, block, 0, c.st, c.nbr, c.values, c.filter, c.m, c.out, c.row_partition);
                 }
@@ -1288,7 +1423,7 @@
     const int rc = [&]() -> int {
         LN_REQUIRE(m >= 0 && filter_extent >= 1 && val_dim >= 1 && nr_filters >= 1, LN_ERR_ARG, "ln_conv_forward: bad sizes");
         LN_REQUIRE(m == 0 || (nbr && values_neigh && filter && out), LN_ERR_ARG, "ln_conv_forward: null buffer");
-        LN_REQUIRE((flags & ~7) == 0, LN_ERR_ARG, "ln_conv_forward: unknown flags %d", flags);
+        LN_REQUIRE((flags & ~15) == 0, LN_ERR_ARG, "ln_conv_forward: unknown flags %d", flags);
         if (m == 0) return LN_OK;
         LnConvPlanIn in = {};
         in.m = m, in.E = filter_extent, in.V = val_dim, in.F = nr_filters;
@@ -1299,6 +1434,7 @@
         in.ws_bytes = workspace_bytes;
         in.bank_ready = (flags & LN_CONV_BANK_READY) != 0 && workspace != nullptr;
         in.riding_total = sum.partial ? sum.total : 0;
+        in.overlapped = (flags & LN_CONV_OVERLAPPED) != 0;
         switch (flags & 3) {
             case 0: ln_conv_plan_and_run<false, false>(in, nbr, values_neigh, filter, out, workspace, sum, &sum_left, row_partition, st); break;
             case LN_CONV_FLIP_NEIGHBOURS: ln_conv_plan_and_run<true, false>(in, nbr, values_neigh, filter, out, workspace, sum, &sum_left, row_partition, st); break;
@@ -2051,11 +2187,236 @@
     }
 }
 
+template <int T, int C>
+__global__ void __launch_bounds__(256 * T) __attribute__((amdgpu_waves_per_eu(T, T)))
+    k_conv_backward_fused_b3_rows(const int* __restrict__ nbr, const float* __restrict__ values, const float* __restrict__ grad_out,
+                             const float* __restrict__ filter, int m, float* __restrict__ grad_values, float* __restrict__ slabs,
+                             const int* __restrict__ row_part) {
+    constexpr int V = 32, F = 32, E = 9, KQ = 8, NT = 2, FT = 2;
+    constexpr int THREADS = 256 * T;
+    constexpr int BANK = E * V * F;
+    constexpr int FRAG16 = E * NT * 3 * 64;
+    constexpr int RS = 32;
+    auto swz = [](int r) { return (0x78 >> (2 * ((r >> 2) & 3))) & 3; };
+    constexpr int PART = 64 * RS;
+    constexpr int STAGE = 2 * 3 * PART;
+    constexpr int LDS_BYTES_A = FRAG16 * 16 + T * STAGE * 2;
+    constexpr int LDS_BYTES_B = (T - 1) * BANK * 4;
+    constexpr int LDS_BYTES = LDS_BYTES_A > LDS_BYTES_B ? LDS_BYTES_A : LDS_BYTES_B;
+    __shared__ __attribute__((aligned(16))) unsigned char s_raw[LDS_BYTES];
+    u32x4* s_frag = reinterpret_cast<u32x4*>(s_raw);
+    unsigned short* s_fh = reinterpret_cast<unsigned short*>(s_raw);
+    unsigned short* s_stage = reinterpret_cast<unsigned short*>(s_raw + FRAG16 * 16);
+    const int tid = threadIdx.x;
+    const int sub = tid >> 8;
+    const int t256 = tid & 255;
+    const int lane = tid & 63;
+    const int wave = t256 >> 6;
+    const int i = lane & 15;
+    const int q = lane >> 4;
+    const int bx0 = ln_partition_tile(blockIdx.x, gridDim.x, row_part, 64 * T * C) * C;
+    const int sub00 = bx0 * (64 * T) + sub * 64;
+    const int m00 = sub00 + wave * 16;
+
+    constexpr int N4 = E * V * F / 4;
+    constexpr int NST = (N4 + THREADS - 1) / THREADS;
+    float4 wv[NST];
+#pragma unroll
+    for (int s = 0; s < NST; ++s) {
+        const int x4 = tid + s * THREADS;
+        wv[s] = (N4 % THREADS == 0 || x4 < N4) ? reinterpret_cast<const float4*>(filter)[x4] : make_float4(0.f, 0.f, 0.f, 0.f);
+    }
+    const int vt = wave / FT, ft = wave % FT;
+    floatx4 acc_w[E];
+#pragma unroll
+    for (int c = 0; c < C; ++c) {
+    const int sub0 = sub00 + c * (64 * T);
+    const int m0 = m00 + c * (64 * T);
+    if (c > 0 && (bx0 + c) * (64 * T) >= m) break;
+    u32x4 va[2][3];
+#pragma unroll
+    for (int st = 0; st < 2; ++st) {
+        float x[8];
+#pragma unroll
+        for (int j = 0; j < 8; ++j) {
+            const int row = sub0 + 32 * st + 8 * q + j;
+            const float xv = values[(size_t)min(row, m - 1) * V + vt * 16 + i];
+            x[j] = (row < m) ? xv : 0.f;
+        }
+#pragma unroll
+        for (int j = 0; j < 4; ++j) {
+            unsigned int h0, m0_, l0, h1, m1_, l1;
+            ln_split3_bits(x[2 * j], h0, m0_, l0);
+            ln_split3_bits(x[2 * j + 1], h1, m1_, l1);
+            va[st][0][j] = ln_pack_hi(h0, h1);
+            va[st][1][j] = ln_pack_hi(m0_, m1_);
+            va[st][2][j] = ln_pack_hi(l0, l1);
+        }
+    }
+#ifndef LN_BWD_DEPTH
+#define LN_BWD_DEPTH 2
+#endif
+    constexpr int DEPTH = LN_BWD_DEPTH;
+    auto slot_of = [](int k) { return k == 0 ? E - 1 : k - 1; };
+    const int lr = lane >> 3, c8 = lane & 7;
+    int nb2[2][E];
+#pragma unroll
+    for (int j = 0; j < 2; ++j)
+#pragma unroll
+        for (int e = 0; e < E; ++e) {
+            const int id = nbr[(size_t)min(m0 + 8 * j + lr, m - 1) * E + (e < E - 1 ? (e ^ 1) : e)];
+            nb2[j][e] = (m0 + 8 * j + lr < m) ? id : -1;
+        }
+    floatx4 a[DEPTH + 1][2];
+    auto gather = [&](int e, floatx4 (&dst)[2]) {
+#pragma unroll
+        for (int j = 0; j < 2; ++j) dst[j] = *reinterpret_cast<const floatx4*>(grad_out + (size_t)(nb2[j][e] >= 0 ? nb2[j][e] : 0) * F + c8 * 4);
+    };
+#pragma unroll
+    for (int j = 0; j < 2; ++j)
+        a[0][j] = *reinterpret_cast<const floatx4*>(grad_out + (size_t)(m0 + 8 * j + lr < m ? m0 + 8 * j + lr : 0) * F + c8 * 4);
+#pragma unroll
+    for (int k = 1; k < DEPTH && k < E; ++k) gather(slot_of(k), a[k % (DEPTH + 1)]);
+    if (c == 0) {
+#pragma unroll
+    for (int s = 0; s < NST; ++s) {
+        const int x4 = tid + s * THREADS;
+        if (N4 % THREADS == 0 || x4 < N4) {
+            const int x = x4 * 4;
+            const int ev = x / F;
+            const int f0 = x - ev * F;
+            const int e = ev / V;
+            const int v = ev - e * V;
+            const float v4[4] = {wv[s].x, wv[s].y, wv[s].z, wv[s].w};
+            unsigned int h[4], md[4], lo[4];
+#pragma unroll
+            for (int j = 0; j < 4; ++j) ln_split3_bits(v4[j], h[j], md[j], lo[j]);
+            const int fr = (((e * NT + (v >> 4)) * 3) * 64 + (f0 >> 3) * 16 + ((v & 15) ^ (2 * (f0 >> 3)))) * 8 + (f0 & 7);
+            *reinterpret_cast<uint2*>(s_fh + fr) = make_uint2(ln_pack_hi(h[0], h[1]), ln_pack_hi(h[2], h[3]));
+            *reinterpret_cast<uint2*>(s_fh + fr + 64 * 8) = make_uint2(ln_pack_hi(md[0], md[1]), ln_pack_hi(md[2], md[3]));
+            *reinterpret_cast<uint2*>(s_fh + fr + 2 * 64 * 8) = make_uint2(ln_pack_hi(lo[0], lo[1]), ln_pack_hi(lo[2], lo[3]));
+        }
+    }
+    }
+    floatx4 acc_v[NT];
+#pragma unroll
+    for (int nt = 0; nt < NT; ++nt) acc_v[nt] = floatx4{0.f, 0.f, 0.f, 0.f};
+#pragma unroll
+    for (int k = 0; k < E; ++k) {
+        const int e = slot_of(k);
+        unsigned short* sg = s_stage + (size_t)sub * STAGE + ((c * E + k) & 1) * (3 * PART);
+        if (k + DEPTH < E) gather(slot_of(k + DEPTH), a[(k + DEPTH) % (DEPTH + 1)]);
+#pragma unroll
+        for (int j = 0; j < 2; ++j) {
+            const floatx4 x = a[k % (DEPTH + 1)][j];
+            const bool there = nb2[j][e] >= 0;
+            unsigned int h[4], md[4], lo[4];
+#pragma unroll
+            for (int cc = 0; cc < 4; ++cc) ln_split3_bits(there ? x[cc] : 0.f, h[cc], md[cc], lo[cc]);
+            const int row = wave * 16 + 8 * j + lr;
+            unsigned short* dst = sg + row * RS + (((c8 >> 1) ^ swz(row)) * 8 + (c8 & 1) * 4);
+            *reinterpret_cast<uint2*>(dst) = make_uint2(ln_pack_hi(h[0], h[1]), ln_pack_hi(h[2], h[3]));
+            *reinterpret_cast<uint2*>(dst + PART) = make_uint2(ln_pack_hi(md[0], md[1]), ln_pack_hi(md[2], md[3]));
+            *reinterpret_cast<uint2*>(dst + 2 * PART) = make_uint2(ln_pack_hi(lo[0], lo[1]), ln_pack_hi(lo[2], lo[3]));
+        }
+        __syncthreads();
+        u32x4 p1, p2, p3;
+        {
+            const unsigned short* src = sg + (wave * 16 + i) * RS + ((q ^ swz(wave * 16 + i)) * KQ);
+            p1 = *reinterpret_cast<const u32x4*>(src);
+            p2 = *reinterpret_cast<const u32x4*>(src + PART);
+            p3 = *reinterpret_cast<const u32x4*>(src + 2 * PART);
+        }
+        const bf16x8 a1 = __builtin_bit_cast(bf16x8, p1), a2 = __builtin_bit_cast(bf16x8, p2), a3 = __builtin_bit_cast(bf16x8, p3);
+#pragma unroll
+        for (int nt = 0; nt < NT; ++nt) {
+            const u32x4* pb = s_frag + ((e * NT + nt) * 3) * 64 + q * 16 + (i ^ (2 * q));
+            const bf16x8 b1 = __builtin_bit_cast(bf16x8, pb[0]), b2 = __builtin_bit_cast(bf16x8, pb[64]), b3 = __builtin_bit_cast(bf16x8, pb[128]);
+            acc_v[nt] = __builtin_amdgcn_mfma_f32_16x16x32_bf16(a3, b1, acc_v[nt], 0, 0, 0);
+            acc_v[nt] = __builtin_amdgcn_mfma_f32_16x16x32_bf16(a1, b3, acc_v[nt], 0, 0, 0);
+            acc_v[nt] = __builtin_amdgcn_mfma_f32_16x16x32_bf16(a2, b2, acc_v[nt], 0, 0, 0);
+            acc_v[nt] = __builtin_amdgcn_mfma_f32_16x16x32_bf16(a2, b1, acc_v[nt], 0, 0, 0);
+            acc_v[nt] = __builtin_amdgcn_mfma_f32_16x16x32_bf16(a1, b2, acc_v[nt], 0, 0, 0);
+            acc_v[nt] = __builtin_amdgcn_mfma_f32_16x16x32_bf16(a1, b1, acc_v[nt], 0, 0, 0);
+        }
+        floatx4 w0 = floatx4{0.f, 0.f, 0.f, 0.f}, w1 = floatx4{0.f, 0.f, 0.f, 0.f};
+#pragma unroll
+        for (int st = 0; st < 2; ++st) {
+            bf16x8 b[3];
+#pragma unroll
+            for (int part = 0; part < 3; ++part) {
+                const int r_lo = 32 * st + 8 * q + (i >> 2), r_hi = r_lo + 4;
+                const int piece = ft * 2 + ((i & 3) >> 1), inner = (i & 1) * 4;
+                const unsigned short* base = sg + part * PART + r_lo * RS + (piece ^ swz(r_lo)) * 8 + inner;
+                const unsigned short* base_hi = sg + part * PART + r_hi * RS + (piece ^ swz(r_hi)) * 8 + inner;
+                const short4v lo4 = __builtin_amdgcn_ds_read_tr16_b64_v4i16((short4v __attribute__((address_space(3)))*)(base));
+                const short4v hi4 = __builtin_amdgcn_ds_read_tr16_b64_v4i16((short4v __attribute__((address_space(3)))*)(base_hi));
+                u32x4 packed;
+                packed[0] = (unsigned int)(unsigned short)lo4[0] | ((unsigned int)(unsigned short)lo4[1] << 16);
+                packed[1] = (unsigned int)(unsigned short)lo4[2] | ((unsigned int)(unsigned short)lo4[3] << 16);
+                packed[2] = (unsigned int)(unsigned short)hi4[0] | ((unsigned int)(unsigned short)hi4[1] << 16);
+                packed[3] = (unsigned int)(unsigned short)hi4[2] | ((unsigned int)(unsigned short)hi4[3] << 16);
+                b[part] = __builtin_bit_cast(bf16x8, packed);
+            }
+            const bf16x8 v1 = __builtin_bit_cast(bf16x8, va[st][0]), v2 = __builtin_bit_cast(bf16x8, va[st][1]), v3 = __builtin_bit_cast(bf16x8, va[st][2]);
+            floatx4& acc = st ? w1 : w0;
+            acc = __builtin_amdgcn_mfma_f32_16x16x32_bf16(v3, b[0], acc, 0, 0, 0);
+            acc = __builtin_amdgcn_mfma_f32_16x16x32_bf16(v1, b[2], acc, 0, 0, 0);
+            acc = __builtin_amdgcn_mfma_f32_16x16x32_bf16(v2, b[1], acc, 0, 0, 0);
+            acc = __builtin_amdgcn_mfma_f32_16x16x32_bf16(v2, b[0], acc, 0, 0, 0);
+            acc = __builtin_amdgcn_mfma_f32_16x16x32_bf16(v1, b[1], acc, 0, 0, 0);
+            acc = __builtin_amdgcn_mfma_f32_16x16x32_bf16(v1, b[0], acc, 0, 0, 0);
+        }
+        if (c == 0) acc_w[e] = w0 + w1;
+        else acc_w[e] += w0 + w1;
+    }
+#pragma unroll
+    for (int nt = 0; nt < NT; ++nt) {
+#pragma unroll
+        for (int r = 0; r < 4; ++r) {
+            const int row = m0 + q * 4 + r;
+            if (row < m) grad_values[(size_t)row * V + nt * 16 + i] = acc_v[nt][r];
+        }
+    }
+    }
+    __syncthreads();
+    float* park_all = reinterpret_cast<float*>(s_raw);
+    const int colp = (ft * 16 + i) ^ ((q & 1) << 4);
+    if (sub > 0) {
+        float* park = park_all + (size_t)(sub - 1) * BANK;
+#pragma unroll
+        for (int e = 0; e < E; ++e)
+#pragma unroll
+            for (int r = 0; r < 4; ++r) park[(e * V + vt * 16 + q * 4 + r) * F + colp] = acc_w[e][r];
+    }
+    if constexpr (T > 1) __syncthreads();
+    if (sub == 0) {
+        float* dst = slabs + (size_t)blockIdx.x * BANK;
+#pragma unroll
+        for (int e = 0; e < E; ++e)
+#pragma unroll
+            for (int r = 0; r < 4; ++r) {
+                const int o = (e * V + vt * 16 + q * 4 + r) * F + ft * 16 + i;
+                float sum = acc_w[e][r];
+#pragma unroll
+                for (int k2 = 1; k2 < T; ++k2) sum += park_all[(k2 - 1) * BANK + (e * V + vt * 16 + q * 4 + r) * F + colp];
+                dst[o] = sum;
+            }
+    }
+}
+
 template <int T>
 static void ln_bwd_launch_fused(const LnBwdPlan& p, const int* nbr, const float* values, const float* grad_out, const float* filter, int m,
                                 float* grad_values, float* partial, const int* row_partition, hipStream_t st) {
     if constexpr (T <= LN_BWD_B3_MAX_T) {
         if (p.form == LN_BWD_FUSED_B3) {
+            if constexpr (T == LN_CONV_OVL_T) {
+                if (p.c > 1) {
+                    LN_LAUNCH("k_conv_backward_fused", (k_conv_backward_fused_b3_rows<T, LN_CONV_OVL_C>), dim3(p.grid), dim3(p.block), 0, st, nbr, values, grad_out,
+                              filter, m, grad_values, partial, row_partition);
+                    return;
+                }
+            }
             LN_LAUNCH("k_conv_backward_fused", (k_conv_backward_fused_b3<T>), dim3(p.grid), dim3(p.block), 0, st, nbr, values, grad_out, filter, m,
                       grad_values, partial, row_partition);
             return;
@@ -2069,14 +2430,15 @@
     return ln_conv_backward_query(mq, mn, filter_extent, val_dim, nr_filters, ln_conv_b3_enabled());
 }
 
-extern "C" int ln_conv_backward(const int* nbr_q, const int* nbr_n, const float* values_neigh, const float* grad_out, const float* filter, int mq,
-                                int mn, int filter_extent, int val_dim, int nr_filters, float* grad_values, float* grad_filter,
-                                void* workspace, size_t workspace_bytes, const int* row_partition, void* stream) {
+extern "C" int ln_conv_backward_flags(const int* nbr_q, const int* nbr_n, const float* values_neigh, const float* grad_out, const float* filter,
+                                      int mq, int mn, int filter_extent, int val_dim, int nr_filters, int flags, float* grad_values,
+                                      float* grad_filter, void* workspace, size_t workspace_bytes, const int* row_partition, void* stream) {
     hipStream_t st = (hipStream_t)stream;
+    LN_REQUIRE((flags & ~LN_CONV_OVERLAPPED) == 0, LN_ERR_ARG, "ln_conv_backward: unknown flags %d", flags);
     const LnBwdPlan p = ln_conv_backward_plan(LnBwdPlanIn{
         mq, mn, filter_extent, val_dim, nr_filters, nbr_q == nbr_n,
         nbr_q && nbr_n && values_neigh && grad_out && filter && grad_values && grad_filter, workspace ? workspace_bytes : 0,
-        ln_aligned16(values_neigh) && ln_aligned16(grad_out) && ln_aligned16(filter), ln_conv_b3_enabled()});
+        ln_aligned16(values_neigh) && ln_aligned16(grad_out) && ln_aligned16(filter), ln_conv_b3_enabled(), (flags & LN_CONV_OVERLAPPED) != 0});
     float* partial = static_cast<float*>(workspace);
     const int total = filter_extent * val_dim * nr_filters;
     if (p.form == LN_BWD_FUSED_B3 || p.form == LN_BWD_FUSED_F32) {
@@ -2105,6 +2467,13 @@
     rc = ln_conv_forward_riding(nbr_n, grad_out, filter, mn, filter_extent, nr_filters, val_dim, LN_CONV_FLIP_NEIGHBOURS | LN_CONV_TRANSPOSED_FILTER,
                                 grad_values, conv_ws, conv_ws ? workspace_bytes - gf_bytes : 0, row_partition, stream, sum);
     return rc ? rc : ln_check_launch("ln_conv_backward");
+}
+
+extern "C" int ln_conv_backward(const int* nbr_q, const int* nbr_n, const float* values_neigh, const float* grad_out, const float* filter, int mq,
+                                int mn, int filter_extent, int val_dim, int nr_filters, float* grad_values, float* grad_filter,
+                                void* workspace, size_t workspace_bytes, const int* row_partition, void* stream) {
+    return ln_conv_backward_flags(nbr_q, nbr_n, values_neigh, grad_out, filter, mq, mn, filter_extent, val_dim, nr_filters, 0, grad_values,
+                                  grad_filter, workspace, workspace_bytes, row_partition, stream);
 }
 
 extern "C" size_t ln_linear_backward_workspace_bytes(int rows, int cin, int cout) {
diff --git a/lattice_net_amd/csrc/ln_conv_plan.h b/lattice_net_amd/csrc/ln_conv_plan.h
--- a/lattice_net_amd/csrc/ln_conv_plan.h
+++ b/lattice_net_amd/csrc/ln_conv_plan.h
@@ -59,7 +59,14 @@
 constexpr bool ln_conv_small_filter(int E, int V, int F) { return E == 9 && (size_t)E * V * F * 4 <= 64 * 1024 && V <= 32; }
 constexpr bool ln_bwd_fused_shape(int E, int V, int F) { return E == 9 && V == 32 && F == 32; }
 
-constexpr int ln_bwd_subtiles(int m, bool b3_enabled) {
+constexpr int LN_CONV_OVL_T = 2;
+constexpr int LN_CONV_OVL_C = 2;
+constexpr int LN_CONV_OVL_MAX_ROWS = 2 * 64 * LN_BWD_B3_MAX_T * LN_BWD_CUS;
+constexpr bool ln_bwd_narrow(int m, bool b3_enabled, bool overlapped) {
+    return overlapped && b3_enabled && m >= LN_CONV_B3_MIN_ROWS && m <= LN_CONV_OVL_MAX_ROWS;
+}
+constexpr int ln_bwd_subtiles(int m, bool b3_enabled, bool overlapped = false) {
+    if (ln_bwd_narrow(m, b3_enabled, overlapped)) return LN_CONV_OVL_T;
     const int max_t = b3_enabled ? LN_BWD_B3_MAX_T : LN_BWD_MAX_SUBTILES;
     const int s = (m + 63) / 64;
     int best = 1, best_cost = 1 << 30;
@@ -73,7 +80,11 @@
     }
     return best;
 }
-constexpr int ln_bwd_workgroups(int m, bool b3_enabled) { return ln_cdiv(m, 64 * ln_bwd_subtiles(m, b3_enabled)); }
+constexpr int ln_bwd_chunks(int m, bool b3_enabled, bool overlapped = false) { return ln_bwd_narrow(m, b3_enabled, overlapped) ? LN_CONV_OVL_C : 1; }
+static_assert(LN_CONV_OVL_T * LN_CONV_OVL_C >= LN_BWD_B3_MAX_T, "the narrow form would write more slabs than the workspace queries report");
+constexpr int ln_bwd_workgroups(int m, bool b3_enabled, bool overlapped = false) {
+    return ln_cdiv(m, 64 * ln_bwd_subtiles(m, b3_enabled, overlapped) * ln_bwd_chunks(m, b3_enabled, overlapped));
+}
 
 constexpr size_t ln_conv_bank_bytes(int m, int E, int V, int F, bool b3_enabled) {
     if (V % 32 != 0 || F % 16 != 0 || m < LN_CONV_B3_MIN_ROWS || E > LN_CONV_LDS_E || !b3_enabled) return 0;
@@ -141,6 +152,7 @@
 struct LnConvLaunch {
     uint8_t kernel;
     uint8_t nt, t;
+    uint8_t c;
     bool carries_sum;
     int grid[3], block;
     int f_off, cols;
@@ -158,6 +170,7 @@
     size_t ws_bytes;
     bool bank_ready;
     int riding_total;
+    bool overlapped = false;
 };
 struct LnConvPlan {
     size_t bank_bytes, slab_bytes;
@@ -169,7 +182,7 @@
 
 inline LnConvLaunch* ln_plan_add(LnConvPlan& p, LnConvKernel k, int nt, int t, int gx, int gy, int gz, int block, int f_off, int cols) {
     LnConvLaunch& l = p.launch[p.n++];
-    l = LnConvLaunch{uint8_t(k), uint8_t(nt), uint8_t(t), false, {gx, gy, gz}, block, f_off, cols, 0, 0, 0};
+    l = LnConvLaunch{uint8_t(k), uint8_t(nt), uint8_t(t), 1, false, {gx, gy, gz}, block, f_off, cols, 0, 0, 0};
     return &l;
 }
 
@@ -181,8 +194,8 @@
     p.sum_left = in.riding_total > 0;
     if (E == 9 && in.filter_aligned) {
         if (!in.flip && !in.wt && V == 32 && F == 32 && m >= LN_CONV_B3_MIN_ROWS && in.b3_enabled && in.values_aligned) {
-            const int bt = ln_bwd_subtiles(m, true), t = bt < 3 ? bt : 3;
-            ln_plan_add(p, LN_K_FORWARD_B3, 2, t, ln_cdiv(m, 64 * t), 1, 1, 256 * t, 0, F);
+            const int bt = ln_bwd_subtiles(m, true, in.overlapped), t = bt < 3 ? bt : 3, c = ln_bwd_chunks(m, true, in.overlapped);
+            ln_plan_add(p, LN_K_FORWARD_B3, 2, t, ln_cdiv(m, 64 * t * c), 1, 1, 256 * t, 0, F)->c = uint8_t(c);
             return p;
         }
         if (ln_conv_full_shape(V, F)) {
@@ -286,7 +299,10 @@
 constexpr size_t ln_gf_query(int m, int E, int V, int F, bool b3_enabled) {
     if (!ln_gf_mfma_supported(V, F) || m <= 0) return 256;
     int chunks = ln_cdiv(m, LN_GF_ROWS);
-    if (ln_bwd_fused_shape(E, V, F) && ln_bwd_workgroups(m, b3_enabled) > chunks) chunks = ln_bwd_workgroups(m, b3_enabled);
+    if (ln_bwd_fused_shape(E, V, F)) {
+        if (ln_bwd_workgroups(m, b3_enabled, false) > chunks) chunks = ln_bwd_workgroups(m, b3_enabled, false);
+        if (ln_bwd_workgroups(m, b3_enabled, true) > chunks) chunks = ln_bwd_workgroups(m, b3_enabled, true);
+    }
     const int rows_b3 = ln_gfb_rows(m, E, V, F);
     if (rows_b3 > 0 && ln_cdiv(m, rows_b3) > chunks) chunks = ln_cdiv(m, rows_b3);
     return (size_t)chunks * E * V * F * sizeof(float) + 256;
@@ -355,22 +371,25 @@
     size_t ws_bytes;
     bool aligned;
     bool b3_enabled;
+    bool overlapped = false;
 };
 struct LnBwdPlan {
     uint8_t form;
     int t;
+    int c;
     int grid, block;
     int conv_blocks;
 };
 constexpr LnBwdPlan ln_conv_backward_plan(const LnBwdPlanIn& in) {
-    LnBwdPlan p = {LN_BWD_TWO_CALLS, 0, 0, 256, 0};
+    LnBwdPlan p = {LN_BWD_TWO_CALLS, 0, 1, 0, 256, 0};
     if (!(in.E == 9 && in.mq > 0 && in.mn > 0 && ln_gf_mfma_supported(in.val_dim, in.nr_filters) && in.buffers && in.ws_bytes > 0 &&
           in.ws_bytes >= ln_gf_query(in.mq, in.E, in.val_dim, in.nr_filters, in.b3_enabled) && in.aligned))
         return p;
     if (in.same_list && in.mq == in.mn && ln_bwd_fused_shape(in.E, in.val_dim, in.nr_filters)) {
-        p.t = ln_bwd_subtiles(in.mn, in.b3_enabled);
+        p.t = ln_bwd_subtiles(in.mn, in.b3_enabled, in.overlapped);
+        p.c = ln_bwd_chunks(in.mn, in.b3_enabled, in.overlapped);
         p.form = in.b3_enabled && p.t <= LN_BWD_B3_MAX_T ? LN_BWD_FUSED_B3 : LN_BWD_FUSED_F32;
-        p.grid = ln_cdiv(in.mn, 64 * p.t);
+        p.grid = ln_bwd_workgroups(in.mn, in.b3_enabled, in.overlapped);
         p.block = 256 * p.t;
     } else if (ln_conv_full_shape(in.nr_filters, in.val_dim)) {
         p.form = LN_BWD_FULL_SUM;
diff --git a/lattice_net_amd/lattice.py b/lattice_net_amd/lattice.py
--- a/lattice_net_amd/lattice.py
+++ b/lattice_net_amd/lattice.py
@@ -1090,6 +1090,8 @@
         out = torch.empty((m, nr_filters), dtype=vals.dtype, device=self._dev())
         flags = (_lib.LN_CONV_FLIP_NEIGHBOURS if flip_neighbours else 0) | (_lib.LN_CONV_TRANSPOSED_FILTER if filter_is_transposed else 0)
         lib = _lib.load()
+        if not half and _SCANS_IN_FLIGHT[0] > 1:
+            flags |= _lib.LN_CONV_OVERLAPPED
         if half:
             _lib.check(lib.ln_conv_forward_f16(_lib.ptr(nbr), _lib.ptr(vals), _lib.ptr(filter_bank), m, filter_extent, v, nr_filters, flags,
                                                _lib.ptr(out), self._stream()), "ln_conv_forward_f16")
@@ -1155,8 +1157,10 @@
                                                main), "ln_conv_forward_f16")
             return gvals, (gf if filter_grad_fp32 else gf.to(torch.float16))
         part = nb._row_partition() if q.m_hash_table._storage is nb.m_hash_table._storage else None
-        _lib.check(lib.ln_conv_backward(_lib.ptr(nbr_q), _lib.ptr(nbr_n), _lib.ptr(nb.values()), _lib.ptr(grad_out), _lib.ptr(filter_bank), mq,
-                                        mn, E, v, f, _lib.ptr(gvals), _lib.ptr(gf), _lib.ptr(ws), ws.numel(), part, main), "ln_conv_backward")
+        flags = _lib.LN_CONV_OVERLAPPED if _SCANS_IN_FLIGHT[0] > 1 else 0
+        _lib.check(lib.ln_conv_backward_flags(_lib.ptr(nbr_q), _lib.ptr(nbr_n), _lib.ptr(nb.values()), _lib.ptr(grad_out), _lib.ptr(filter_bank),
+                                              mq, mn, E, v, f, flags, _lib.ptr(gvals), _lib.ptr(gf), _lib.ptr(ws), ws.numel(), part, main),
+                   "ln_conv_backward")
         return gvals, gf
 
     def convolve_im2row_grad_filter(self, grad_out: torch.Tensor, dilation: int, lattice_neighbours: Optional["Lattice"],
```

Measured after the change: 1514, median of 6. 1.8% higher.
